# kfjahnke/envutil

Hardware: AMD Instinct MI355X
Metric: Mpix/s reprojected (16K lat/lon->cubemap, b-spline-3) (higher is better)
Workload: dtype f32

## Files before the change

envutil_amd/csrc/eu_api_render.hip:

```cpp

#include "eu_context.h"
#include "eu_setup_math.h"
#include "eu_encode.h"
#include "eu_rgbe_dev.h"

using namespace eu_host;

namespace {

int band_shift_of(int band_rows)
{
  int sh = 0;
  while ((1 << sh) < band_rows) sh++;
  return sh;
}

int build_inv_planar(const eu_target *t, eu_inv_planar *q)
{
  memset(q, 0, sizeof *q);
  const eu_facet *f = t->single;
  if (!f || !eu::has_2d_tf(*f)) return EU_OK;
  q->shear = f->shear_g != 0.0 || f->shear_t != 0.0;
  q->shift = f->h != 0.0 || f->v != 0.0;
  q->lcp = f->a != 0.0 || f->b != 0.0 || f->c != 0.0;
// ... 151 lines not shown
    if (k + 1 < EU_REJ_N) m = std::min(m, raw[k + 1]);
    tab[EU_REJ_HDR + k] = (float)(m * (1.0 - 2e-3));
  }
  const double W = std::max(std::max(std::fabs((double)d.wex0), std::fabs((double)d.wex1)),
                            std::max(std::fabs((double)d.wex2), std::fabs((double)d.wex3)));
  const double mg = 1e-3 * W;
  tab[0] = (float)u0; tab[1] = (float)(1.0 / du); tab[2] = 1.0f;
  {
    bool mono = true;
    double prev = -1.0;
    const double tmax = std::acos(std::max(-1.0, u0));
    for (int i = 0; i <= 4096 && mono; i++) {
      bool k2 = true;
      const double r = radius(tmax * i / 4096.0, k2);
      mono = k2 && r > prev;
      prev = r;
    }
    if (mono && analytic) {
      tab[2] = 2.0f;
      const double f = 1.0 - 2e-3;
      tab[10] = d.has_lcp ? 1.0f / d.lens_s : 0.0f;
      tab[11] = (float)(f * (d.has_lcp ? d.lens_d : 1.0)); tab[12] = d.has_lcp ? (float)(f * d.lens_c) : 0.0f;
      tab[13] = d.has_lcp ? (float)(f * d.lens_b) : 0.0f; tab[14] = d.has_lcp ? (float)(f * d.lens_a) : 0.0f;
    }
  }
  tab[4] = d.has_shift ? d.lens_h : 0.0f; tab[5] = d.has_shift ? d.lens_v : 0.0f;
  tab[6] = (float)(d.wex0 - mg); tab[7] = (float)(d.wex1 + mg); tab[8] = (float)(d.wex2 - mg); tab[9] = (float)(d.wex3 + mg);
  return true;
}

int build_multi(const eu_target *t, eu_source *const *srcs, int nsrc, float *out_dev,
                size_t row_stride_bytes, const eu_switches &sw, eu_multi_params *p, int *degree)
{
  { int rc0 = check_target(t); if (rc0) return rc0; }
  const eu_source *s0 = srcs[0];
  for (int f = 0; f < nsrc; f++) {
    if (!srcs[f]) return fail(EU_ERR_HANDLE, "null source");
    if (srcs[f]->degree != s0->degree) return fail(EU_ERR_ARGUMENT, "facets must share the spline degree");
  }
  const bool twine = t->ntaps > 0;
  std::vector<unsigned char> key = plan_key_of(t, srcs, nsrc, true);
  auto &mp = cur().mplan;
  HIPCHK(cur().tables.host_wait());
  if (key != mp.key) {
    eu::mat3 r_cam = eu::make_r3(t->roll, t->pitch, t->yaw, false);
    std::vector<float> rows;
    eu::stepper_tables tb;
    for (int f = 0; f < nsrc; f++) {
      eu::mat3 r_fct = eu::make_r3(srcs[f]->fct.roll, srcs[f]->fct.pitch, srcs[f]->fct.yaw, true);
      eu::mat3 basis = eu::rotate(r_cam, r_fct);
      if (!eu::build_stepper_tables(*t, basis, true, twine, tb))
        return fail(EU_ERR_UNSUPPORTED, "no stepper for this target projection");
      rows.insert(rows.end(), tb.row.begin(), tb.row.end());
    }
    { int rcu = upload_plan(mp, t, tb, rows, key); if (rcu) return rcu; }
  }
  std::vector<eu_src_dev> sd((size_t)nsrc);
  for (int f = 0; f < nsrc; f++) sd[f] = srcs[f]->sd;
  HIPCHK(mp.src.reserve((size_t)nsrc));
  HIPCHK(hipMemcpyAsync(mp.src.p, sd.data(), sizeof(eu_src_dev) * (size_t)nsrc, hipMemcpyHostToDevice, cur().stream));
  bool any_rej = false;
  std::vector<float> rej;
  if (sw.rej) {
    rej.resize((size_t)nsrc * EU_REJ_STRIDE);
    for (int f = 0; f < nsrc; f++) any_rej |= build_reject_table(sd[f], rej.data() + (size_t)f * EU_REJ_STRIDE, sw.rej == 2);
  }
  if (any_rej) {
    HIPCHK(mp.rej.reserve(rej.size()));
    HIPCHK(hipMemcpyAsync(mp.rej.p, rej.data(), rej.size() * sizeof(float), hipMemcpyHostToDevice, cur().stream));
  }
  std::vector<eu_generic> gv((size_t)nsrc);
  bool any_generic = false;
  for (int f = 0; f < nsrc; f++) {
    memset(&gv[f], 0, sizeof(eu_generic));
    if (!eu::has_translation(srcs[f]->fct) && !eu::generic_target(*t)) continue;
    if (!eu::make_generic(*t, srcs[f]->fct, gv[f]))
      return fail(EU_ERR_UNSUPPORTED, "generic stepper (translation, --single): no planar-to-ray functor for this target projection");
    any_generic = true;
  }
  if (any_generic) {
    HIPCHK(mp.gen.reserve((size_t)nsrc));
    HIPCHK(hipMemcpyAsync(mp.gen.p, gv.data(), sizeof(eu_generic) * (size_t)nsrc, hipMemcpyHostToDevice, cur().stream));
  }
  HIPCHK(hipStreamSynchronize(cur().stream));
  eu_inv_planar inv;
  { int rci = build_inv_planar(t, &inv); if (rci) return rci; }
  memset(p, 0, sizeof *p);
  p->gen = any_generic ? mp.gen.p : nullptr;
  p->rej = any_rej ? mp.rej.p : nullptr;
  p->inv = inv;
  fill_frame(t, p);
  p->form = mp.form; p->norm_mode = mp.norm; p->twine = twine; p->ntaps = t->ntaps;
  fill_synopsis(t, srcs, nsrc, p);
  p->col = mp.col.p; p->row = mp.row.p; p->taps = mp.taps.p; p->srcs = mp.src.p;
  p->out = out_dev; p->out_stride = (long long)(row_stride_bytes / sizeof(float));
  *degree = s0->degree;
  return EU_OK;
}

void refresh_seg_flags(const eu_render_params *p)
{
  eu_src_dev cmp = p->src;
  cmp.base = nullptr;
  if (cur().plan.seg_valid && !memcmp(&cmp, &cur().plan.seg_sd, sizeof cmp)) return;
  cur().plan.seg_sd = cmp;
  cur().plan.seg_valid = true;
  const int W = p->width, H = p->height;
  const int nseg = (H + EU_SEG_ROWS - 1) / EU_SEG_ROWS;
  cur().plan.seg_flags.assign((size_t)nseg, 0);
  const eu_src_dev &s = p->src;
  if (s.prj != EU_SPHERICAL || W < 64 || cur().plan.h_col.size() < (size_t)2 * W || cur().plan.h_row.size() < (size_t)H * EU_ROW_FLOATS)
    return;
  const double kx = (double)s.total_w / s.ext_w, ky = (double)s.total_h / s.ext_h;
  auto ray = [&](int x, int y, double *r) {
    const float *rt = &cur().plan.h_row[(size_t)y * EU_ROW_FLOATS];
    const float c0 = cur().plan.h_col[(size_t)x], c1 = cur().plan.h_col[(size_t)W + x];
    for (int i = 0; i < 3; i++)
      r[i] = p->form == EU_FORM_BCA ? (double)rt[3 + i] * c0 + (double)rt[6 + i] * c1 + rt[i]
                                    : (double)rt[3 + i] * c0 + rt[i];
  };
  for (int k = 0; k < nseg; k++) {
    const int yc = std::min(k * EU_SEG_ROWS + EU_SEG_ROWS / 2, H - 1);
    int across = 0;
    for (int j = 0; j < 16; j++) {
      const int xc = std::min((int)((j + 0.5) * W / 16), W - 2);
      double a[3], b[3];
      ray(xc, yc, a);
      ray(xc + 1, yc, b);
      const double lon0 = std::atan2(a[0], a[2]), lon1 = std::atan2(b[0], b[2]);
      const double lat0 = std::atan2(a[1], std::hypot(a[0], a[2])), lat1 = std::atan2(b[1], std::hypot(b[0], b[2]));
      double dlon = std::fabs(lon1 - lon0);
      if (dlon > M_PI) dlon = 2.0 * M_PI - dlon;
      if (std::fabs(lat1 - lat0) * ky > 0.5 * dlon * kx) across++;
    }
    cur().plan.seg_flags[(size_t)k] = across > 8;
  }
}

int launch_staged(const eu_render_params *p, const eu_switches &sw, hipStream_t st, int *launches)
{
  const unsigned long long ntiles = eu_staged_tiles(p->width, p->row_begin, p->row_end);
  if (ntiles > EU4_WL_MAX_TILES) return -2;
  const size_t need = eu_render4_worklist_ints((size_t)ntiles);
  if (cur().staged.wl.cap < need) {
    if (cur().staged.wl_pair.host_wait() != hipSuccess || cur().staged.wl.reserve(need) != hipSuccess) return -1;
    if (hipMemsetAsync(cur().staged.wl.p, 0, eu_render4_worklist_header_ints() * sizeof(int), st) != hipSuccess) {
      cur().staged.wl.cap = 0;
      return -1;
    }
  }
  eu_render_params q = *p;
  q.wl = cur().staged.wl.p;
  if (cur().staged.wl_pair.order_after(st) != hipSuccess) return -1;
  const int rc = eu_launch_render4(&q, &sw, cur().plan.h_row.data(), cur().plan.h_row.size(), cur().plan.plan_gen, st, launches);
  if (rc || !*launches) return rc;
  return cur().staged.wl_pair.note(st) != hipSuccess ? -1 : 0;
}

int launch_packed_runs(const eu_render_params *p, const eu_switches &sw, hipStream_t st, int *launches)
{
  refresh_seg_flags(p);
  const std::vector<eu_run> runs = eu_split_runs(cur().plan.seg_flags.data(), (int)cur().plan.seg_flags.size(), *p, sw.hybrid == 2);
  if (runs.empty()) { *launches = 1; return eu_launch_render2(p, &sw, st); }
  for (const eu_run &r : runs) {
    eu_render_params q = *p;
    q.row_begin = r.row_begin; q.row_end = r.row_end;
    q.out = p->out + (long long)(r.row_begin - p->row_begin) * p->out_stride;
    q.layout = r.layout;
    ++*launches;
    const int rc = eu_launch_render2(&q, &sw, st);
    if (rc) return rc;
  }
  return 0;
}

int launch_render(const eu_render_params *p, const eu_switches &sw, hipStream_t st)
{
  eu_path path = eu_select_path(*p, sw);
  int rc = 0, n = 0;
  if (path == EU_PATH_STAGED) {
    rc = launch_staged(p, sw, st, &n);
    if (!rc && !n) path = eu_select_path(*p, sw, false);
  }
  switch (path) {
    case EU_PATH_STAGED: break;
    case EU_PATH_PACKED_RUNS: rc = launch_packed_runs(p, sw, st, &n); break;
    case EU_PATH_PACKED: n = 1; rc = eu_launch_render2(p, &sw, st); break;
    case EU_PATH_GENERAL: n = 1; rc = eu_launch_render(p, st); break;
    case EU_PATH_GENERAL_DIRECT: {
      eu_render_params q = *p;
      q.direct = 1;
      n = 1;
      rc = eu_launch_render(&q, st);
    }
  }
  cur().launches += n;
  return rc;
}

int order_encoders(hipStream_t st)
{
  if (st == cur().stream) cur().enc.own = true;
  else if (cur().enc.own) { HIPCHK(hipStreamSynchronize(cur().stream)); cur().enc.own = false; }
  HIPCHK(cur().tables.order_after(st));
  HIPCHK(cur().enc.readers.order_after(st));
  return EU_OK;
}

}

namespace eu_host __attribute__((visibility("hidden"))) {

int render_on_device(const eu_target *trg, eu_source *const *srcs, int nsrc, float *out_dev, size_t stride_bytes,
                     const eu_switches &sw, hipStream_t st, const eu_encode *enc, bool rgbe)
{
  int rc;
  const bool multi = nsrc > 1;
  const bool screen = trg->out_format == EU_OUT_SRGBA8;
  eu_target tf = *trg;
  float *fout = out_dev;
  size_t fstride = stride_bytes;
  const size_t rows = (size_t)(trg->row_end - trg->row_begin);
  if (screen || enc || rgbe) {
    if (screen && !cur().lut) return fail(EU_ERR_NO_DEVICE, "sRGB table missing: library not initialised");
    if (screen && (rc = order_encoders(st))) return rc;
    tf.out_format = EU_OUT_FLOAT;
    fstride = (size_t)frame_w(trg) * trg->nchannels * sizeof(float);
    if (cur().out.scr.cap < rows * frame_w(trg) * trg->nchannels) HIPCHK(cur().tables.host_wait());
    HIPCHK(cur().out.scr.reserve(rows * frame_w(trg) * trg->nchannels));
    fout = cur().out.scr.p;
  }
  if (multi) {
    eu_multi_params mp;
    int mdeg = 0;
    if ((rc = build_multi(&tf, srcs, nsrc, fout, fstride, sw, &mp, &mdeg))) return rc;
    if (eu_launch_render_multi(&mp, mdeg, st)) return fail(EU_ERR_NO_DEVICE, "kernel launch failed");
  } else {
    eu_render_params p;
    if ((rc = build_params(&tf, srcs, nsrc, fout, fstride, sw, &p))) return rc;
    if (launch_render(&p, sw, st)) return fail(EU_ERR_NO_DEVICE, "kernel launch failed");
  }
  if (screen &&
      eu_launch_to_screen(fout, (long long)(fstride / sizeof(float)), (unsigned *)out_dev,
                          (long long)(stride_bytes / sizeof(unsigned)), frame_w(trg), (int)rows,
                          trg->nchannels, cur().lut, st))
    return fail(EU_ERR_NO_DEVICE, "kernel launch failed");
  if (enc && rows) {
    eu_encode_params ep {};
    ep.src = fout; ep.src_stride_bytes = fstride;
    ep.dst = out_dev; ep.dst_stride_bytes = stride_bytes;
    ep.tables = cur().enc.steps.dev.p;
    ep.w = frame_w(trg); ep.h = (int)rows; ep.nch = trg->nchannels;
    ep.bits = enc->bits; ep.big_endian = enc->big_endian;
    if (eu_launch_encode(&ep, st)) return fail(EU_ERR_NO_DEVICE, "kernel launch failed");
  }
  if (rgbe && rows) {
    eu_rgbe_encode_params ep {};
    ep.src = fout; ep.src_stride_bytes = fstride;
    ep.dst = reinterpret_cast<uint32_t *>(out_dev); ep.dst_stride_bytes = stride_bytes;
    ep.w = frame_w(trg); ep.h = (int)rows;
    if (eu_launch_rgbe_encode(&ep, st)) return fail(EU_ERR_NO_DEVICE, "kernel launch failed");
  }
  return EU_OK;
}

}

extern "C" {

static int check_steps(const float *s, int bits, const char *who, const char *which)
{
  const int n = 1 << bits;
  const std::string head = std::string(who) + ": " + which + " steps: ";
  if (std::isnan(s[1])) return fail(EU_ERR_ARGUMENT, head + "entry 1 is NaN, a table has at least one code above 0");
  int m = 1;
  for (; m + 1 < n && !std::isnan(s[m + 1]); m++)
    if (s[m + 1] < s[m]) return fail(EU_ERR_ARGUMENT, head + "entry " + std::to_string(m + 1) + " is smaller than the one before it");
  for (int k = m + 1; k < n; k++)
    if (!std::isnan(s[k]))
      return fail(EU_ERR_ARGUMENT, head + "entry " + std::to_string(k) + " is a number behind the NaN at entry " + std::to_string(m + 1));
  return EU_OK;
}

static int check_encode(const char *who, const eu_encode *enc, int width, int nch, const void *out, size_t out_row_stride_bytes)
{
  const std::string head = std::string(who) + ": ";
  if (!enc || !out) return fail(EU_ERR_ARGUMENT, head + "null argument");
  if (enc->bits != 8 && enc->bits != 16) return fail(EU_ERR_ARGUMENT, head + "bits must be 8 or 16");
  if (!enc->colour_steps) return fail(EU_ERR_ARGUMENT, head + "null colour steps");
  if (nch < 1 || nch > 4) return fail(EU_ERR_ARGUMENT, head + "channels must be 1..4");
  if (width < 0 || (size_t)width * nch > (size_t(1) << 28)) return fail(EU_ERR_ARGUMENT, head + "rows of 0 .. 2^28 samples");
  if (out_row_stride_bytes < (size_t)width * nch * (enc->bits / 8)) return fail(EU_ERR_ARGUMENT, head + "row stride smaller than a row");
  if (enc->bits == 16 && (reinterpret_cast<uintptr_t>(out) % 2 || out_row_stride_bytes % 2))
    return fail(EU_ERR_ARGUMENT, head + "16-bit samples lie at even addresses: out and its row stride are multiples of 2");
  int rc;
  if ((rc = check_steps(enc->colour_steps, enc->bits, who, "colour"))) return rc;
  if (enc->alpha_steps && (rc = check_steps(enc->alpha_steps, enc->bits, who, "alpha"))) return rc;
  return EU_OK;
}

static int upload_steps(const eu_encode *enc, hipStream_t st)
{
  { int rc = order_encoders(st); if (rc) return rc; }
  const size_t n = size_t(1) << enc->bits;
  const float *alpha = enc->alpha_steps ? enc->alpha_steps : enc->colour_steps;
  held_table &steps = cur().enc.steps;
  if (steps.holds(enc->colour_steps, n, alpha, n)) return EU_OK;
// ... 285 lines not shown
```

envutil_amd/csrc/eu_launch.h:

```cpp
#ifndef EU_LAUNCH_H
#define EU_LAUNCH_H
#include <hip/hip_runtime.h>
#include <cstddef>
#include "eu_device.h"
#include "eu_select.h"
#include "eu_worklist.h"

#define EU_REJ_N 1024
#define EU_REJ_HDR 16
#define EU_REJ_STRIDE (EU_REJ_HDR + EU_REJ_N)

struct eu_multi_params {
  int width, height, row_begin, row_end;
  int form, norm_mode, twine, ntaps, nch, nfct, plus;
  const float *col;
  const float *row;
  const float *taps;
  const eu_src_dev *srcs;
  float *out;
  long long out_stride;
  int tiles_x, tiles_y;
  int band_shift, band_count, band_index;
  int hdr, hdr_low, hdr_high;
  const eu_generic *gen;
  eu_inv_planar inv;
  const float *rej;
};

struct eu_alpha_params;

template <class T> struct eu_dev_buf {
  T *p = nullptr;
  size_t cap = 0;
  hipError_t reserve(size_t n)
  {
    if (cap >= n) return hipSuccess;
    if (p) (void)hipFree(p);
    p = nullptr; cap = 0;
    const hipError_t e = hipMalloc((void **)&p, n * sizeof(T));
    if (e == hipSuccess) cap = n; else p = nullptr;
    return e;
  }
};

struct eu_readers {
  hipEvent_t ev = nullptr;
  bool recorded = false;
  hipError_t note(hipStream_t st)
  {
    hipError_t e = ev ? order_after(st) : hipEventCreateWithFlags(&ev, hipEventDisableTiming);
    if (e == hipSuccess) e = hipEventRecord(ev, st);
    if (e == hipSuccess) recorded = true;
    return e;
  }
  hipError_t host_wait() const { return recorded ? hipEventSynchronize(ev) : hipSuccess; }
  hipError_t order_after(hipStream_t st) const { return recorded ? hipStreamWaitEvent(st, ev, 0) : hipSuccess; }
};

extern "C" {
int eu_launch_render(const eu_render_params *p, void *stream);
int eu_launch_render2(const eu_render_params *p, const eu_switches *sw, void *stream);
int eu_launch_render4(const eu_render_params *p, const eu_switches *sw, const float *h_row, size_t h_row_floats,
                      unsigned long long plan_gen, void *stream, int *launches);
int eu_launch_render_rays(const eu_rays_params *p, int path, void *stream);
int eu_launch_view_tables(const eu_view_dev *views, int nviews, int prj, int width, int height, int twine, float *col,
                          float *row, void *stream);
int eu_launch_render_views(const eu_render_params *p, const eu_view_strides *vs, int nviews, int path,
                           const eu_switches *sw, void *stream);
int eu_launch_render_layers(const eu_render_params *p, const eu_layers_params *lp, int path, const eu_switches *sw,
                            void *stream);
int eu_launch_render_multi(const eu_multi_params *p, int degree, void *stream);
int eu_launch_render_multi_nch1(const eu_multi_params *p, int degree, void *stream);
int eu_launch_render_multi_nch2(const eu_multi_params *p, int degree, void *stream);
int eu_launch_render_multi_nch3(const eu_multi_params *p, int degree, void *stream);
int eu_launch_render_multi_nch4(const eu_multi_params *p, int degree, void *stream);
int eu_launch_render_views_multi(const eu_multi_params *p, const eu_view_strides *vs, int nviews, int degree, void *stream);
int eu_launch_render_views_multi_nch1(const eu_multi_params *p, const eu_view_strides *vs, int nviews, int degree, void *stream);
int eu_launch_render_views_multi_nch2(const eu_multi_params *p, const eu_view_strides *vs, int nviews, int degree, void *stream);
int eu_launch_render_views_multi_nch3(const eu_multi_params *p, const eu_view_strides *vs, int nviews, int degree, void *stream);
int eu_launch_render_views_multi_nch4(const eu_multi_params *p, const eu_view_strides *vs, int nviews, int degree, void *stream);
int eu_launch_to_screen(const float *in, long long in_stride, unsigned *out, long long out_stride, int w, int rows,
                        int nch, const float *lut, void *stream);
int eu_launch_prefilter(float *container, const eu_container *g, int nch, int bc0, int bc1, int prefilter_degree,
                        int spherical, int iir_stream, void *stream);
int eu_launch_cubemap_build(const float *faces_dev, float *ir_dev, int nch, long face_px, long section_px,
                            long left_frame, long right_frame, double refc_md, double model_to_px,
                            int prefilter_degree, int iir_stream, void *stream);
int eu_launch_facet_alpha(const eu_alpha_params *p, void *stream);
int eu_launch_diag(const eu_render_params *p, unsigned long long *stamps_dev, void *stream);
int eu_launch_diag_coords(const eu_src_dev *s, const float *rays_dev, long n, int variant, float *out_dev,
                          void *stream);
int eu_launch_selftest(unsigned long long seed, int blocks, int iters, unsigned long long *bad_dev, void *stream);
int eu_verify_const_div(float c, float limit, void *stream);
int eu_current_slot(void);
}

#endif
```

envutil_amd/csrc/eu_render4.hip:

```cpp
#include <cstdio>
#include <cstring>
#include <vector>
#include <algorithm>
#include "eu_packed_dev.h"
#include "eu_launch.h"

#define EU4_TW 16
#define EU4_TH 8
#define EU4_WAVES 4
#ifndef EU4_WAVES0
#define EU4_WAVES0 1
#define EU4_TEXELS 384
#define EU4_OCC0 4
#endif
#define EU4_UNIT_ROWS 4
#define EU4_COL_FLOATS 8
#define EU4_MAX_PLANS 16

__device__ __forceinline__ void eu4_box_reduce(int &mn0, int &mn1, int &mx0, int &mx1)
{
#define EU4_RED(ctrl)                                        \
  "v_min_i32_dpp %0, %0, %0 " ctrl "\n\t"                    \
  "v_min_i32_dpp %1, %1, %1 " ctrl "\n\t"                    \
  "v_max_i32_dpp %2, %2, %2 " ctrl "\n\t"                    \
  "v_max_i32_dpp %3, %3, %3 " ctrl "\n\t"
  asm("s_nop 1\n\t"
      EU4_RED("row_shr:1 row_mask:0xf bank_mask:0xf")
      EU4_RED("row_shr:2 row_mask:0xf bank_mask:0xf")
      EU4_RED("row_shr:4 row_mask:0xf bank_mask:0xf")
      EU4_RED("row_shr:8 row_mask:0xf bank_mask:0xf")
      EU4_RED("row_bcast:15 row_mask:0xa bank_mask:0xf")
      EU4_RED("row_bcast:31 row_mask:0xc bank_mask:0xf")
      "s_nop 0"
      : "+v"(mn0), "+v"(mn1), "+v"(mx0), "+v"(mx1));
#undef EU4_RED
  mn0 = __builtin_amdgcn_readlane(mn0, 63); mn1 = __builtin_amdgcn_readlane(mn1, 63);
  mx0 = __builtin_amdgcn_readlane(mx0, 63); mx1 = __builtin_amdgcn_readlane(mx1, 63);
}

typedef __attribute__((address_space(3))) void *eu4_lds_void;
typedef const __attribute__((address_space(1))) void *eu4_gbl_void;

typedef float eu4_f4 __attribute__((ext_vector_type(4)));

__device__ __forceinline__ void eu4_dma_row(unsigned dst, unsigned voff, const char *sb)
{
  unsigned keep;
  asm volatile("s_mov_b32 %0, m0\n\t"
               "s_mov_b32 m0, %1\n\t"
               "s_nop 0\n\t"
               "global_load_lds_dwordx4 %2, %3\n\t"
               "s_mov_b32 m0, %0"
               : "=&s"(keep) : "s"(dst), "v"(voff), "s"(sb) : "memory");
}

struct eu4_plan {
  const float *atab_g;
  const int *tileplan;
  const float *coltab;
  int tiles16;
  const int *l2_rows;
  int l2_off[9];
  int l2_half;
  unsigned long long l2_magic;
  const int *l1_ent;
  int l1_off[9];
  int l1_ecols;
  unsigned long long l1_magic;
  const int *xtab;
  const int *boxtab;
#ifdef EU5_STAMPS
  unsigned long long *stamps;
#endif
};

#ifdef EU5_STAMPS
#define EU5_STAMP(k) do { asm volatile("" ::: "memory"); st_[k] = __builtin_amdgcn_s_memtime(); asm volatile("" ::: "memory"); } while (0)
#define EU5_STAMP32(k) do { asm volatile("" ::: "memory"); st_[k] = (unsigned)__builtin_amdgcn_s_memtime(); asm volatile("" ::: "memory"); } while (0)
#else
#define EU5_STAMP(k) do { } while (0)
#define EU5_STAMP32(k) do { } while (0)
#endif

template <int NCH, int DEG, int PRJ>
__device__ __forceinline__ void eu4_tile(const eu_render_params &p, const eu4_plan &w, const float *atab,
                                         float *wtile, int tile_y, int x0, int lane)
{
  constexpr int TEX = 4;
  constexpr int order = DEG + 1;
  const eu_src_dev &s = p.src;
  const int lx = lane & 7, ly = lane >> 3;
  const int y = p.row_begin + tile_y * EU4_TH + ly;
  const bool yin = y < p.row_end;
  const int yc = yin ? y : p.row_end - 1;
  const float *rt = p.row + (long long)eu_frame_row(yc, p.band_shift, p.band_count, p.band_index) * EU_ROW_FLOATS;
  const int xa = x0 + 2 * lx, xb = xa + 1;
  const bool va = yin && xa < p.width, vb = yin && xb < p.width;
  const int xac = xa < p.width ? xa : p.width - 1, xbc = xb < p.width ? xb : p.width - 1;

  eu_f2 tx, ty, gy;
  eu_i2 hit, ok = { -1, -1 };
  int ixa, ixb;
  float wxa[order], wxb[order];
  eu_ray2 r;
  {
    const float A0 = rt[0], A1 = rt[1], A2 = rt[2], B0 = rt[3], B1 = rt[4], B2 = rt[5];
    const eu_f2 c0 = { p.col[xac], p.col[xbc] };
    if (p.form == EU_FORM_BCA) {
      const float C0 = rt[6], C1 = rt[7], C2 = rt[8];
      const float *colB = p.col + p.width;
      const eu_f2 c1 = { colB[xac], colB[xbc] };
      r.x = B0 * c0 + C0 * c1 + A0;
      r.y = B1 * c0 + C1 * c1 + A1;
      r.z = B2 * c0 + C2 * c1 + A2;
    } else {
      r.x = B0 * c0 + A0;
      r.y = B1 * c0 + A1;
      r.z = B2 * c0 + A2;
    }
    if (p.norm_mode == EU_NORM_DIV) {
      eu_f2 sqn = r.x * r.x; sqn = sqn + r.y * r.y; sqn = sqn + r.z * r.z;
      const eu_f2 n = { sqrtf(sqn.x), sqrtf(sqn.y) };
      r.x = r.x / n; r.y = r.y / n; r.z = r.z / n;
    }
  }
  asm volatile("s_waitcnt vmcnt(0)" ::: "memory");
  eu_f2 sx, sy;
  hit = eu_coord2_ok<PRJ>(s, r, sx, sy, atab, ok);
  const eu_f2 gx = eu_gate2_ok(sx, s.gate0, s.lower0, s.upper0, ok);
  gy = eu_gate2_ok(sy, s.gate1, s.lower1, s.upper1, ok);
  eu_f2 fx;
  if constexpr (DEG & 1) fx = (eu_f2){ floorf(gx.x), floorf(gx.y) };
  else fx = (eu_f2){ roundf(gx.x), roundf(gx.y) };
  tx = gx - fx;
  ixa = (int)fx.x; ixb = (int)fx.y;
  hit = hit & (eu_i2){ va ? -1 : 0, vb ? -1 : 0 };
  eu_f2 fy;
  if constexpr (DEG & 1) fy = (eu_f2){ floorf(gy.x), floorf(gy.y) };
  else fy = (eu_f2){ roundf(gy.x), roundf(gy.y) };
  ty = gy - fy;
  const int iya = (int)fy.x, iyb = (int)fy.y;

  int mnx = INT_MAX, mny = INT_MAX, mxx = INT_MIN, mxy = INT_MIN;
  if (hit.x) { mnx = ixa; mxx = ixa; mny = iya; mxy = iya; }
  if (hit.y) { mnx = min(mnx, ixb); mxx = max(mxx, ixb); mny = min(mny, iyb); mxy = max(mxy, iyb); }
  eu4_box_reduce(mnx, mny, mxx, mxy);
  const bool any = mnx != INT_MAX;
  const long long bw = (long long)mxx - mnx + order, bh = (long long)mxy - mny + order;
  const bool fits = bw <= 64 && bh <= EU4_TEXELS && bw * bh <= EU4_TEXELS;
  const bool clean = __ballot((hit.x && !ok.x) || (hit.y && !ok.y)) == 0ull;
  float *const orow = p.out + (long long)(yc - p.row_begin) * p.out_stride;
  if (any && !(fits && clean)) {
    if (lane == 0) {
      const int id = tile_y * w.tiles16 + x0 / EU4_TW;
      const int sh = eu4_shard_of(id);
      const int slot = atomicAdd(p.wl + EU4_WL_SHARD(sh), 1);
      p.wl[EU4_WL_ENTRIES + (size_t)slot * EU4_SHARDS + sh] = id;
    }
    return;
  }
  float qa[NCH], qb[NCH];
  if (any) {
    const int ibw = (int)bw, ibh = (int)bh;
    const unsigned lds_tile = (unsigned)(unsigned long long)(eu4_lds_void)wtile;
    if (lane < ibw) {
      const int bx0 = mnx - DEG / 2, by0 = mny - DEG / 2;
      const unsigned voff = (unsigned)(lane * NCH) * 4u;
      const char *sb = (const char *)(s.base + ((long long)by0 * s.es1 + (long long)bx0 * NCH));
      const long long step = s.es1 * 4;
      unsigned dst = lds_tile;
      const unsigned dstep = (unsigned)ibw * (TEX * 4u);
#pragma unroll 1
      for (int it = 0; it < ibh; it++) { eu4_dma_row(dst, voff, sb); sb += step; dst += dstep; }
    }
    eu_f2 wx[order], wy[order];
    float wya[order], wyb[order];
    if constexpr (DEG >= 2) {
      eu_weights2<DEG>(s.wm, ty, wy);
      eu_weights2<DEG>(s.wm, tx, wx);
    }
#pragma unroll
    for (int i = 0; i < order; i++) {
      if constexpr (DEG >= 2) {
        wya[i] = wy[i].x; wyb[i] = wy[i].y;
        wxa[i] = wx[i].x; wxb[i] = wx[i].y;
      } else {
        wya[i] = wyb[i] = 0.0f;
        wxa[i] = wxb[i] = 0.0f;
      }
    }
    const int oa = hit.x ? ((iya - mny) * ibw + (ixa - mnx)) * TEX : 0;
    const int ob = hit.y ? ((iyb - mny) * ibw + (ixb - mnx)) * TEX : 0;
    asm volatile("s_waitcnt vmcnt(0)" ::: "memory");
    eu_lptr lt = (eu_lptr)wtile;
    eu_accumulate1<NCH, DEG, TEX, int, eu_lptr>(lt + oa, ibw * TEX, wxa, wya, tx.x, ty.x, qa);
    eu_accumulate1<NCH, DEG, TEX, int, eu_lptr>(lt + ob, ibw * TEX, wxb, wyb, tx.y, ty.y, qb);
  } else {
#pragma unroll
    for (int c = 0; c < NCH; c++) { qa[c] = 0.0f; qb[c] = 0.0f; }
  }
  constexpr int ncol = (NCH == 2 || NCH == 4) ? NCH - 1 : NCH;
  const bool bright = s.brighten != 1.0f;
#pragma unroll
  for (int c = 0; c < NCH; c++) {
    float a = qa[c], bb = qb[c];
    if (bright && c < ncol) { a = a * s.brighten; bb = bb * s.brighten; }
    qa[c] = hit.x ? a : 0.0f;
    qb[c] = hit.y ? bb : 0.0f;
  }
  if (va) eu_put<NCH>(orow, xa, qa);
  if (vb) eu_put<NCH>(orow, xb, qb);
}

template <int NCH, int DEG, int PRJ>
__global__ __launch_bounds__(64 * EU4_WAVES0, EU4_OCC0) void eu_render4s_kernel(const eu_render_params p, const eu4_plan w)
{
  __shared__ __attribute__((aligned(16))) float tile_all[EU4_WAVES0 * EU4_TEXELS * 4];
  __shared__ __attribute__((aligned(16))) float atab[768];
  const int lane = threadIdx.x & 63;
  const int wave = __builtin_amdgcn_readfirstlane(threadIdx.x >> 6);
  float *const tile = tile_all + wave * (EU4_TEXELS * 4);
  if (PRJ != EU_CUBEMAP && wave == 0) {
    static_assert(EU_ATAN_TAB_FLOATS * 4 <= 3 * 1024, "three pieces");
#pragma unroll
    for (int i = 0; i < 3; i++)
      __builtin_amdgcn_global_load_lds((eu4_gbl_void)(w.atab_g + i * 256 + lane * 4),
                                       (eu4_lds_void)(atab + i * 256), 16, 0, 0);
  }
  const int tile_x = (int)(blockIdx.x >> 3) * EU4_WAVES0 + wave;
  const int tile_y = ((int)blockIdx.z * 8 + (int)(blockIdx.x & 7)) * EU4_UNIT_ROWS + (int)blockIdx.y;
  if (tile_y >= p.tiles_y) return;
  if constexpr (EU4_WAVES0 > 1) {
    asm volatile("s_waitcnt vmcnt(0)" ::: "memory");
    __syncthreads();
  }
  if (tile_x >= w.tiles16) return;
  eu4_tile<NCH, DEG, PRJ>(p, w, atab, tile, tile_y, tile_x * EU4_TW, lane);
}

template <int NCH, int DEG, int PRJ>
__device__ __forceinline__ void eu4_direct_tile(const eu_render_params &p, const float *atab, int tile_y, int x0, int lane)
{
  const eu_src_dev &s = p.src;
  const int lx = lane & 7, ly = lane >> 3;
  const int y = p.row_begin + tile_y * EU4_TH + ly;
  const bool yin = y < p.row_end;
  const int yc = yin ? y : p.row_end - 1;
  const float *rt = p.row + (long long)eu_frame_row(yc, p.band_shift, p.band_count, p.band_index) * EU_ROW_FLOATS;
  const int xa = x0 + 2 * lx, xb = xa + 1;
  const bool va = yin && xa < p.width, vb = yin && xb < p.width;
  const int xac = xa < p.width ? xa : p.width - 1, xbc = xb < p.width ? xb : p.width - 1;
  eu_ray2 ry;
  {
    const float A0 = rt[0], A1 = rt[1], A2 = rt[2], B0 = rt[3], B1 = rt[4], B2 = rt[5];
    const eu_f2 c0 = { p.col[xac], p.col[xbc] };
    if (p.form == EU_FORM_BCA) {
      const float C0 = rt[6], C1 = rt[7], C2 = rt[8];
      const float *colB = p.col + p.width;
      const eu_f2 c1 = { colB[xac], colB[xbc] };
      ry.x = B0 * c0 + C0 * c1 + A0;
      ry.y = B1 * c0 + C1 * c1 + A1;
      ry.z = B2 * c0 + C2 * c1 + A2;
    } else {
      ry.x = B0 * c0 + A0;
      ry.y = B1 * c0 + A1;
      ry.z = B2 * c0 + A2;
    }
    if (p.norm_mode == EU_NORM_DIV) {
      eu_f2 sqn = ry.x * ry.x; sqn = sqn + ry.y * ry.y; sqn = sqn + ry.z * ry.z;
      const eu_f2 n = { sqrtf(sqn.x), sqrtf(sqn.y) };
      ry.x = ry.x / n; ry.y = ry.y / n; ry.z = ry.z / n;
    }
  }
  eu_f2 sx, sy;
  eu_i2 hit = eu_coord2<PRJ>(s, ry, sx, sy, atab);
  hit = hit & (eu_i2){ va ? -1 : 0, vb ? -1 : 0 };
  float pxa[NCH], pxb[NCH];
  eu_eval2<NCH, DEG>(s, sx, sy, hit, pxa, pxb);
  float *const orow = p.out + (long long)(yc - p.row_begin) * p.out_stride;
  if (va) eu_put<NCH>(orow, xa, pxa);
  if (vb) eu_put<NCH>(orow, xb, pxb);
}

#include "eu_share_groups.h"
#include "eu_render5.h"

template <int DEG>
__global__ __launch_bounds__(256) void eu_colplan_kernel(const eu_render_params p, float *ct,
                                                         float A0, float A2, float B0, float B2)
{
  __shared__ __attribute__((aligned(16))) float atab[EU_ATAN_TAB_FLOATS];
  if (threadIdx.x < EU_ATAN_TAB_ENTRIES) eu_atan_tab_entry(threadIdx.x, atab + 8 * threadIdx.x);
  __syncthreads();
  constexpr int order = DEG + 1;
  const eu_src_dev &s = p.src;
  const int xa = 2 * (blockIdx.x * 256 + threadIdx.x), xb = xa + 1;
  if (xa >= p.width) return;
  const int xbc = xb < p.width ? xb : p.width - 1;
  const eu_f2 c0 = { p.col[xa], p.col[xbc] };
  const eu_f2 rx = B0 * c0 + A0, rz = B2 * c0 + A2;
  eu_i2 ok = { -1, -1 };
  const eu_f2 q2 = rx * rx + rz * rz;
  const eu_f2 qs = eu_sqrt2_ok(q2, ok);
  const eu_f2 lon = eu_atan2f_2_tab_ok(rx, rz, atab, 0, ok);
  eu_f2 i0 = { (float)((double)lon.x - s.tex_x0), (float)((double)lon.y - s.tex_x0) };
  if (s.cdiv_ok) i0 = eu_div2_const(i0, s.ext_w, s.rcp_ext_w);
  else i0 = i0 / s.ext_w;
  i0 = i0 * s.total_w; i0 = i0 - .5f;
  const eu_f2 sx = i0 - s.win_x_off;
  const eu_f2 gx = eu_gate2_ok(sx, s.gate0, s.lower0, s.upper0, ok);
  eu_f2 fx;
  if constexpr (DEG & 1) fx = (eu_f2){ floorf(gx.x), floorf(gx.y) };
  else fx = (eu_f2){ roundf(gx.x), roundf(gx.y) };
  const eu_f2 tx = gx - fx;
  eu_f2 wx[4];
#pragma unroll
  for (int i = 0; i < 4; i++) wx[i] = (eu_f2){ 0.0f, 0.0f };
  if constexpr (DEG >= 2) eu_weights2<DEG>(s.wm, tx, wx);
  float e[2][EU4_COL_FLOATS];
  e[0][0] = __int_as_float(ok.x ? (int)fx.x : INT_MIN);
  e[1][0] = __int_as_float(ok.y ? (int)fx.y : INT_MIN);
  e[0][1] = tx.x; e[1][1] = tx.y;
#pragma unroll
  for (int i = 0; i < 4; i++) { e[0][2 + i] = i < order ? wx[i].x : 0.0f; e[1][2 + i] = i < order ? wx[i].y : 0.0f; }
  e[0][6] = qs.x; e[1][6] = qs.y;
  e[0][7] = lon.x; e[1][7] = lon.y;
  float *o = ct + (size_t)xa * EU4_COL_FLOATS;
#pragma unroll
  for (int i = 0; i < EU4_COL_FLOATS; i++) o[i] = e[0][i];
  if (xb < p.width) {
#pragma unroll
    for (int i = 0; i < EU4_COL_FLOATS; i++) o[EU4_COL_FLOATS + i] = e[1][i];
  }
}

template <int NCH, int DEG, int PRJ>
__global__ __launch_bounds__(256, 4) void eu_render4d_kernel(const eu_render_params p, const eu4_plan w)
{
  __shared__ __attribute__((aligned(16))) float atab[EU_ATAN_TAB_FLOATS];
  if constexpr (PRJ != EU_CUBEMAP) {
    if (threadIdx.x < EU_ATAN_TAB_ENTRIES) eu_atan_tab_entry(threadIdx.x, atab + 8 * threadIdx.x);
  }
  const int lane = threadIdx.x & 63;
  const int wave = __builtin_amdgcn_readfirstlane(threadIdx.x >> 6);
  const int gid = blockIdx.x * EU4_WAVES + wave;
  const int sh = gid & (EU4_SHARDS - 1);
  const int nwork = __builtin_amdgcn_readfirstlane(
    __hip_atomic_load(p.wl + EU4_WL_SHARD(sh), __ATOMIC_RELAXED, __HIP_MEMORY_SCOPE_AGENT));
  __syncthreads();
#pragma unroll 1
  for (int k = gid / EU4_SHARDS; k < nwork; k += (int)(gridDim.x * EU4_WAVES / EU4_SHARDS)) {
    const int id = __builtin_amdgcn_readfirstlane(p.wl[EU4_WL_ENTRIES + (size_t)k * EU4_SHARDS + sh]);
    const int tile_y = id / w.tiles16;
    const int x0 = (id - tile_y * w.tiles16) * EU4_TW;
    eu4_direct_tile<NCH, DEG, PRJ>(p, atab, tile_y, x0, lane);
  }
  __shared__ int last, listed;
  __syncthreads();
  if (threadIdx.x == 0) { listed = 0; last = atomicAdd(p.wl + EU4_WL_DONE1, 1) == (int)gridDim.x - 1; }
  __syncthreads();
  if (last) {
    int mine = 0;
    for (int i = threadIdx.x; i < EU4_SHARDS; i += 256)
      mine += __hip_atomic_load(p.wl + EU4_WL_SHARD(i), __ATOMIC_RELAXED, __HIP_MEMORY_SCOPE_AGENT);
    atomicAdd(&listed, mine);
    for (int i = threadIdx.x; i <= EU4_SHARDS + 8; i += 256)
      __hip_atomic_store(p.wl + 16 * i, 0, __ATOMIC_RELAXED, __HIP_MEMORY_SCOPE_AGENT);
    __syncthreads();
    if (threadIdx.x == 0) __hip_atomic_store(p.wl + EU4_WL_LISTED, listed, __ATOMIC_RELAXED, __HIP_MEMORY_SCOPE_AGENT);
  }
}

static long long eu4_followers_plan = 0, eu4_followers_last = 0;
extern "C" unsigned long long eu_hip_share_follower_tiles(void) { return (unsigned long long)eu4_followers_last; }
static int eu4_boxtab_last = 0;
static long long eu4_boxtab_tiles_last = 0;
extern "C" int eu_hip_boxtab_used(void) { return eu4_boxtab_last; }
extern "C" unsigned long long eu_hip_boxtab_tiles(void) { return (unsigned long long)eu4_boxtab_tiles_last; }

#ifndef EU4_DIRECT_WGS
#define EU4_DIRECT_WGS 2048
#endif

template <int NCH, int DEG, int PRJ>
static int launch4_ndp(const eu_render_params &p, const eu4_plan &w, hipStream_t st)
{
  if constexpr (PRJ == EU_SPHERICAL) {
    static const int cus = [] {
      int dev = 0, n = 0;
      if (hipGetDevice(&dev) != hipSuccess) return 0;
      if (hipDeviceGetAttribute(&n, hipDeviceAttributeMultiprocessorCount, dev) != hipSuccess) return 0;
      return n;
    }();
    const bool fast = eu_staged_fast_profile(p);
    const bool bt = fast && w.boxtab != nullptr && p.out_stride < (1ll << 25);
    int per_cu = 0;
    if (bt) {
      static const int occ = [] { int n = 0; return hipOccupancyMaxActiveBlocksPerMultiprocessor(&n, eu_render5_kernel<NCH, DEG, PRJ, true, true>, 64 * EU5_WAVES, 0) == hipSuccess ? n : 0; }();
      per_cu = occ;
    } else if (fast) {
      static const int occ = [] { int n = 0; return hipOccupancyMaxActiveBlocksPerMultiprocessor(&n, eu_render5_kernel<NCH, DEG, PRJ, true>, 64 * EU5_WAVES, 0) == hipSuccess ? n : 0; }();
      per_cu = occ;
    } else {
      static const int occ = [] { int n = 0; return hipOccupancyMaxActiveBlocksPerMultiprocessor(&n, eu_render5_kernel<NCH, DEG, PRJ, false>, 64 * EU5_WAVES, 0) == hipSuccess ? n : 0; }();
      per_cu = occ;
    }
    const int wgs = (cus / 8) * 8 * per_cu;
    if (wgs <= 0) return -1;
    if (fast) eu4_followers_last = eu4_followers_plan;
    eu4_boxtab_last = bt;
    if (bt) hipLaunchKernelGGL((eu_render5_kernel<NCH, DEG, PRJ, true, true>), dim3((unsigned)wgs), dim3(64 * EU5_WAVES), 0, st, p, w);
    else if (fast) hipLaunchKernelGGL((eu_render5_kernel<NCH, DEG, PRJ, true>), dim3((unsigned)wgs), dim3(64 * EU5_WAVES), 0, st, p, w);
    else hipLaunchKernelGGL((eu_render5_kernel<NCH, DEG, PRJ, false>), dim3((unsigned)wgs), dim3(64 * EU5_WAVES), 0, st, p, w);
  } else {
    const int units = (p.tiles_y + EU4_UNIT_ROWS - 1) / EU4_UNIT_ROWS;
    dim3 grid((unsigned)(8 * ((w.tiles16 + EU4_WAVES0 - 1) / EU4_WAVES0)), (unsigned)EU4_UNIT_ROWS, (unsigned)((units + 7) / 8));
    hipLaunchKernelGGL((eu_render4s_kernel<NCH, DEG, PRJ>), grid, dim3(64 * EU4_WAVES0), 0, st, p, w);
  }
  if (hipGetLastError() != hipSuccess) return -1;
  hipLaunchKernelGGL((eu_render4d_kernel<NCH, DEG, PRJ>), dim3(EU4_DIRECT_WGS), dim3(256), 0, st, p, w);
  if (hipGetLastError() != hipSuccess) {
    (void)hipMemsetAsync(p.wl, 0, EU4_WL_ENTRIES * sizeof(int), st);
    return -1;
  }
  return 0;
}

template <int NCH, int DEG>
static int launch4_nd(const eu_render_params &p, const eu4_plan &w, hipStream_t st)
{
  switch (p.src.prj) {
    case EU_SPHERICAL: return launch4_ndp<NCH, DEG, EU_SPHERICAL>(p, w, st);
    case EU_CUBEMAP: return launch4_ndp<NCH, DEG, EU_CUBEMAP>(p, w, st);
    case EU_BIATAN6: return launch4_ndp<NCH, DEG, EU_BIATAN6>(p, w, st);
  }
  return -2;
}

template <int NCH>
static int launch4_n(const eu_render_params &p, const eu4_plan &w, hipStream_t st)
{
  switch (p.src.degree) {
    case 1: return launch4_nd<NCH, 1>(p, w, st);
    case 2: return launch4_nd<NCH, 2>(p, w, st);
    case 3: return launch4_nd<NCH, 3>(p, w, st);
  }
  return -2;
}

static_assert(EU_STAGED_TILE_ROWS == EU4_TH && EU_STAGED_MAX_TILES_Y == 65535 * 8 * EU4_UNIT_ROWS, "eu_select.h: eu_staged_covers");
namespace {
struct plan_cache {
  std::vector<unsigned char> key;
  eu_dev_buf<int> tileplan, l2_rows, l1_ent, xtab, boxtab;
  bool has_boxtab = false;
  long long boxtab_tiles = 0;
  eu_dev_buf<float> coltab;
  float *atab = nullptr;
  int planned_rows = 0;
  int l2_off[9] = {};
  int l1_off[9] = {};
  int l1_ecols = 1;
  long long follower_tiles = 0;
} g4s[EU_MAX_SLOTS];
#define g4 (g4s[eu_current_slot()])

bool ensure_atab()
{
  if (g4.atab) return true;
  std::vector<float> tab(768, 0.0f);
  for (int i = 0; i < EU_ATAN_TAB_ENTRIES; i++) eu_atan_tab_entry(i, tab.data() + 8 * i);
  if (hipMalloc((void **)&g4.atab, tab.size() * sizeof(float)) != hipSuccess) return false;
  return hipMemcpy(g4.atab, tab.data(), tab.size() * sizeof(float), hipMemcpyHostToDevice) == hipSuccess;
}

template <int DEG>
void launch_colplan(const eu_render_params &p, float *ct, const float *k, hipStream_t st)
{
  hipLaunchKernelGGL((eu_colplan_kernel<DEG>), dim3((unsigned)((p.width + 511) / 512)), dim3(256), 0, st, p, ct,
                     k[0], k[1], k[2], k[3]);
}

std::vector<unsigned char> eu4_plan_key(const eu_render_params &p, unsigned long long plan_gen, const eu_switches &sw)
{
  std::vector<unsigned char> key(sizeof(unsigned long long) + sizeof(eu_src_dev) + 11 * sizeof(int));
  unsigned char *q = key.data();
  memcpy(q, &plan_gen, sizeof plan_gen); q += sizeof plan_gen;
  eu_src_dev sd = p.src; sd.base = nullptr;
  memcpy(q, &sd, sizeof sd); q += sizeof sd;
  const int v[11] = { p.width, p.row_begin, p.row_end, p.band_shift, p.band_count, p.band_index, p.form, p.norm_mode, sw.share,
                      sw.boxtab, sw.boxtab_max_kb };
  memcpy(q, v, sizeof v);
  return key;
}

bool upload(eu_dev_buf<int> &buf, const std::vector<int> &v, size_t spare)
{
  if (buf.reserve(v.size() + spare) != hipSuccess) return false;
  return v.empty() || hipMemcpy(buf.p, v.data(), v.size() * sizeof(int), hipMemcpyHostToDevice) == hipSuccess;
}

template <int DEG>
void launch_boxplan(const eu_render_params &p, const float *atab_g, const int *l2_rows, int tiles16, int ntiles, int *tab, hipStream_t st)
{
  hipLaunchKernelGGL((eu5_boxplan_kernel<DEG>), dim3((unsigned)((ntiles + 3) / 4)), dim3(256), 0, st, p, atab_g, l2_rows, tiles16,
                     ntiles, tab);
}

int eu4_build_plans(const eu_render_params &p, int tiles16, const eu_switches &sw, const float *h_row,
                    size_t h_row_floats, hipStream_t st)
{
  std::vector<int> tp((size_t)p.tiles_y, -1);
  std::vector<float> plans;
  const bool can = p.form == EU_FORM_BA && p.norm_mode == EU_NORM_NONE && h_row;
  if (can && sw.colplan) {
    for (int ty = 0; ty < p.tiles_y; ty++) {
      float k[4] = { 0, 0, 0, 0 };
      bool same = true;
      for (int ly = 0; ly < EU4_TH && same; ly++) {
        const int y = std::min(p.row_begin + ty * EU4_TH + ly, p.row_end - 1);
        const size_t fr = (size_t)eu_frame_row(y, p.band_shift, p.band_count, p.band_index) * EU_ROW_FLOATS;
        if (fr + 6 > h_row_floats) { same = false; break; }
        const float c[4] = { h_row[fr + 0], h_row[fr + 2], h_row[fr + 3], h_row[fr + 5] };
        if (ly == 0) memcpy(k, c, sizeof k);
        else same = memcmp(k, c, sizeof k) == 0;
      }
      if (!same) continue;
      int id = -1;
      for (size_t j = 0; j < plans.size() / 4 && id < 0; j++)
        if (memcmp(&plans[4 * j], k, sizeof k) == 0) id = (int)j;
      if (id < 0 && plans.size() / 4 < EU4_MAX_PLANS) {
        id = (int)(plans.size() / 4);
        plans.insert(plans.end(), k, k + 4);
      }
      tp[(size_t)ty] = id;
    }
  }
  const int nplans = (int)(plans.size() / 4);
  if (hipStreamSynchronize(st) != hipSuccess) return -1;
  if (g4.tileplan.reserve(tp.size()) != hipSuccess) return -1;
  if (g4.coltab.reserve(std::max<size_t>(1, nplans) * (size_t)p.width * EU4_COL_FLOATS) != hipSuccess) return -1;
  if (hipMemcpy(g4.tileplan.p, tp.data(), tp.size() * sizeof(int), hipMemcpyHostToDevice) != hipSuccess) return -1;
  g4.planned_rows = 0;
  for (int v : tp) g4.planned_rows += v >= 0;
  auto paired = [&](int m) { return 2 * m + 1 < p.tiles_y && tp[(size_t)2 * m] >= 0 && tp[(size_t)2 * m] == tp[(size_t)2 * m + 1]; };
  {
    std::vector<int> rows[8], all;
    for (int r = 0; r < p.tiles_y; r++)
      if (!paired(r >> 1)) rows[(r / EU5_UNIT_ROWS) & 7].push_back(r);
    for (int x = 0; x < 8; x++) { g4.l2_off[x] = (int)all.size(); all.insert(all.end(), rows[x].begin(), rows[x].end()); }
    g4.l2_off[8] = (int)all.size();
    if (!upload(g4.l2_rows, all, 1)) return -1;
  }
  g4.has_boxtab = false; g4.boxtab_tiles = 0;
  if (sw.boxtab && eu_staged_fast_profile(p)) {
    const long long ntiles = (long long)g4.l2_off[8] * tiles16;
    const long long bytes = ntiles * (EU5_BT_RECS * 16);
    if (bytes <= (long long)sw.boxtab_max_kb * 1024) {
      if (g4.boxtab.reserve((size_t)std::max<long long>(1, ntiles) * (EU5_BT_RECS * 4)) != hipSuccess) return -1;
      if (ntiles > 0) {
        switch (p.src.degree) {
          case 1: launch_boxplan<1>(p, g4.atab, g4.l2_rows.p, tiles16, (int)ntiles, g4.boxtab.p, st); break;
          case 2: launch_boxplan<2>(p, g4.atab, g4.l2_rows.p, tiles16, (int)ntiles, g4.boxtab.p, st); break;
          default: launch_boxplan<3>(p, g4.atab, g4.l2_rows.p, tiles16, (int)ntiles, g4.boxtab.p, st); break;
        }
        if (hipGetLastError() != hipSuccess) return -1;
      }
      g4.has_boxtab = true; g4.boxtab_tiles = ntiles;
    }
  }
  for (int j = 0; j < nplans; j++) {
    float *ct = g4.coltab.p + j * (size_t)p.width * EU4_COL_FLOATS;
    switch (p.src.degree) {
      case 1: launch_colplan<1>(p, ct, &plans[4 * j], st); break;
      case 2: launch_colplan<2>(p, ct, &plans[4 * j], st); break;
      default: launch_colplan<3>(p, ct, &plans[4 * j], st); break;
    }
    if (hipGetLastError() != hipSuccess) return -1;
  }
  std::vector<float> h_ct((size_t)nplans * p.width * EU4_COL_FLOATS);
  if (nplans) {
    if (hipStreamSynchronize(st) != hipSuccess) return -1;
    if (hipMemcpy(h_ct.data(), g4.coltab.p, h_ct.size() * sizeof(float), hipMemcpyDeviceToHost) != hipSuccess) return -1;
  }
  std::vector<int> cm, cp;
  for (int m = 0; 2 * m + 1 < p.tiles_y; m++)
    if (paired(m)) { cm.push_back(m); cp.push_back(tp[(size_t)2 * m]); }
  eu_share_input in;
  in.width = p.width; in.tiles16 = tiles16; in.row_begin = p.row_begin; in.row_end = p.row_end;
  in.band_mode = p.band_count > 1;
  in.ncand = (int)cm.size(); in.cand_m = cm.data(); in.cand_plan = cp.data();
  in.h_row = h_row; in.h_row_floats = h_row_floats; in.row_floats = EU_ROW_FLOATS;
  in.coltab = nplans ? h_ct.data() : nullptr; in.col_floats = EU4_COL_FLOATS; in.nplans = nplans;
  in.mode = sw.share; in.unit_drows = EU5_UNIT_ROWS / 2;
  eu_share_result gr;
  eu_share_build(in, gr);
  if (!upload(g4.l1_ent, gr.entries, 2)) return -1;
  if (g4.xtab.reserve(gr.xtab.size()) != hipSuccess) return -1;
  if (hipMemcpy(g4.xtab.p, gr.xtab.data(), gr.xtab.size() * sizeof(int), hipMemcpyHostToDevice) != hipSuccess) return -1;
  for (int x = 0; x < 9; x++) g4.l1_off[x] = gr.off[x];
  g4.l1_ecols = gr.ecols;
  g4.follower_tiles = gr.follower_tiles;
  return 0;
}

void eu4_fill_plan(eu4_plan &w)
{
  w.tileplan = g4.tileplan.p;
  w.coltab = g4.coltab.p;
  w.l2_rows = g4.l2_rows.p;
  for (int x = 0; x < 9; x++) w.l2_off[x] = g4.l2_off[x];
  w.l2_half = (w.tiles16 + 1) / 2;
  w.l2_magic = (1ull << 40) / (unsigned long long)w.l2_half + 1;
  w.l1_ent = g4.l1_ent.p;
  for (int x = 0; x < 9; x++) w.l1_off[x] = g4.l1_off[x];
  w.l1_ecols = g4.l1_ecols;
  w.l1_magic = (1ull << 40) / (unsigned long long)w.l1_ecols + 1;
  w.xtab = g4.xtab.p;
  w.boxtab = g4.has_boxtab ? g4.boxtab.p : nullptr;
}

int launch4(const eu_render_params &p, const eu4_plan &w, hipStream_t st)
{
  switch (p.nch) {
    case 3: return launch4_n<3>(p, w, st);
    case 4: return launch4_n<4>(p, w, st);
  }
  return -2;
}

#ifdef EU5_STAMPS
int launch4_stamped(const eu_render_params &p, eu4_plan &w, hipStream_t st)
{
  static unsigned long long *d_st = nullptr; static size_t st_cap = 0; static int dumps = 0;
  const size_t ntile_st = (size_t)w.tiles16 * p.tiles_y * 8;
  const size_t nst = ntile_st + 8192 * 4;
  if (st_cap < nst) { if (d_st) (void)hipFree(d_st); if (hipMalloc((void **)&d_st, nst * 8) != hipSuccess) return -1; st_cap = nst; }
  (void)hipMemsetAsync(d_st, 0, nst * 8, st);
  w.stamps = d_st;
  const int rc_ = launch4(p, w, st);
  if (rc_ == 0 && dumps < 2 && nst >= 8 * 4096) {
    dumps++;
    std::vector<unsigned long long> h(nst);
    (void)hipStreamSynchronize(st);
    (void)hipMemcpy(h.data(), d_st, nst * 8, hipMemcpyDeviceToHost);
    double acc[32][8] = {}; size_t cnt[32] = {};
    for (size_t t = 0; t < ntile_st / 8; t++) {
      const unsigned long long *q = &h[t * 8];
      if (!q[0] || !q[7]) continue;
      const int cls = (int)(q[1] & 31);
      cnt[cls]++;
      acc[cls][0] += (double)(q[2] - q[0]); acc[cls][1] += (double)(q[3] - q[2]);
      if (q[4]) { acc[cls][2] += (double)(q[4] - q[3]); acc[cls][3] += (double)(q[5] - q[4]); acc[cls][4] += (double)(q[6] - q[5]); }
      acc[cls][5] += (double)(q[7] - q[6]); acc[cls][6] += (double)(q[7] - q[0]);
    }
    {
      double mn = 1e30, mx = 0, sum = 0, l1 = 0, first = 1e30, last = 0; size_t nw = 0;
      for (size_t k = 0; k < 8192; k++) {
        const unsigned long long *q = &h[ntile_st + k * 4];
        if (!q[3]) continue;
        const double d = (double)(q[2] - q[0]);
        mn = std::min(mn, d); mx = std::max(mx, d); sum += d; l1 += (double)(q[1] - q[0]); nw++;
        first = std::min(first, (double)q[0]); last = std::max(last, (double)q[2]);
      }
      if (nw) fprintf(stderr, "eu5 waves: %zu, cycles per wave min %.0f avg %.0f max %.0f, first loop avg %.0f, first start .. last end %.0f\n",
                      nw, mn, sum / nw, mx, l1 / nw, last - first);
    }
    for (int c = 0; c < 32; c++) if (cnt[c])
      fprintf(stderr, "eu5 stamps: hoist %d npass %2d tiles %8zu | coords %7.0f box %6.0f dma-issue+weights %6.0f dma-wait %6.0f taps(all passes) %6.0f store %5.0f | tile %7.0f (100 MHz ticks? s_memtime)\n",
              c >> 4, (c & 15) - 1, cnt[c], acc[c][0] / cnt[c], acc[c][1] / cnt[c], acc[c][2] / cnt[c], acc[c][3] / cnt[c], acc[c][4] / cnt[c], acc[c][5] / cnt[c], acc[c][6] / cnt[c]);
  }
  return rc_;
}
#endif
}

extern "C" int eu_launch_render4(const eu_render_params *pp, const eu_switches *sw, const float *h_row, size_t h_row_floats,
                                 unsigned long long plan_gen, void *stream, int *launches)
{
  eu_render_params p = *pp;
  eu4_followers_last = 0;
  eu4_boxtab_last = 0; eu4_boxtab_tiles_last = 0;
  *launches = 2;
  if (!eu_staged_covers(p) || !p.wl) return -2;
  p.tiles_y = (p.row_end - p.row_begin + EU4_TH - 1) / EU4_TH;
  eu4_plan w;
  w.tiles16 = (p.width + EU4_TW - 1) / EU4_TW;
  if (w.tiles16 <= 0 || p.tiles_y <= 0) return 0;
  hipStream_t st = (hipStream_t)stream;
  if (!ensure_atab()) return -1;
  w.atab_g = g4.atab;
  if (p.src.prj == EU_SPHERICAL) {
    std::vector<unsigned char> key = eu4_plan_key(p, plan_gen, *sw);
    if (key != g4.key) {
      if (eu4_build_plans(p, w.tiles16, *sw, h_row, h_row_floats, st)) return -1;
      g4.key.swap(key);
    }
    if (sw->r4 != 1 && !eu_staged_worth(p.src.degree, g4.planned_rows, p.tiles_y)) { *launches = 0; return 0; }
  }
  eu4_fill_plan(w);
  eu4_followers_plan = g4.follower_tiles;
  eu4_boxtab_tiles_last = w.boxtab ? g4.boxtab_tiles : 0;
#ifdef EU5_STAMPS
  return launch4_stamped(p, w, st);
#else
  return launch4(p, w, st);
#endif
}
```

envutil_amd/csrc/eu_render5.h:

```cpp
#define EU5_WAVES 4
#ifndef EU5_TEXELS
#define EU5_TEXELS 576
#endif
#ifndef EU5_OCC
#define EU5_OCC 4
#endif
#ifndef EU5_UNIT_ROWS
#define EU5_UNIT_ROWS 4
#endif

typedef const __attribute__((address_space(3))) eu4_f4 *eu5_l4ptr;

template <int NCH, int DEG>
__device__ __forceinline__ void eu5_taps(eu_lptr lt, int a, int b, int pitch, const eu_f2 *wx, const eu_f2 *wy,
                                         eu_f2 tx, eu_f2 ty, eu_f2 &rga, eu_f2 &bxa, eu_f2 &rgb, eu_f2 &bxb)
{
  constexpr int order = DEG + 1;
  if constexpr (DEG == 1) {
    const eu_f2 wl0 = 1.0f - tx, wr0 = tx, wl1 = 1.0f - ty, wr1 = ty;
    const eu4_f4 a00 = *(eu5_l4ptr)(lt + a), a01 = *(eu5_l4ptr)(lt + a + 4);
    const eu4_f4 a10 = *(eu5_l4ptr)(lt + a + pitch), a11 = *(eu5_l4ptr)(lt + a + pitch + 4);
    const eu4_f4 b00 = *(eu5_l4ptr)(lt + b), b01 = *(eu5_l4ptr)(lt + b + 4);
    const eu4_f4 b10 = *(eu5_l4ptr)(lt + b + pitch), b11 = *(eu5_l4ptr)(lt + b + pitch + 4);
    {
      const eu_f2 l0 = { wl0.x, wl0.x }, r0 = { wr0.x, wr0.x }, l1 = { wl1.x, wl1.x }, r1 = { wr1.x, wr1.x };
      eu_f2 s = a00.xy * l0; s = s + a01.xy * r0; s = s * l1;
      eu_f2 u = a10.xy * l0; u = u + a11.xy * r0; rga = s + u * r1;
      s = a00.zw * l0; s = s + a01.zw * r0; s = s * l1;
      u = a10.zw * l0; u = u + a11.zw * r0; bxa = s + u * r1;
    }
    {
      const eu_f2 l0 = { wl0.y, wl0.y }, r0 = { wr0.y, wr0.y }, l1 = { wl1.y, wl1.y }, r1 = { wr1.y, wr1.y };
      eu_f2 s = b00.xy * l0; s = s + b01.xy * r0; s = s * l1;
      eu_f2 u = b10.xy * l0; u = u + b11.xy * r0; rgb = s + u * r1;
      s = b00.zw * l0; s = s + b01.zw * r0; s = s * l1;
      u = b10.zw * l0; u = u + b11.zw * r0; bxb = s + u * r1;
    }
  } else {
#pragma unroll
    for (int j = 0; j < order; j++) {
      eu4_f4 ta[order], tb[order];
#pragma unroll
      for (int i = 0; i < order; i++) {
        ta[i] = *(eu5_l4ptr)(lt + a + j * pitch + 4 * i);
        tb[i] = *(eu5_l4ptr)(lt + b + j * pitch + 4 * i);
      }
      const eu_f2 w0a = { wx[0].x, wx[0].x }, w0b = { wx[0].y, wx[0].y };
      eu_f2 ra = ta[0].xy * w0a, qa = ta[0].zw * w0a, rb = tb[0].xy * w0b, qb = tb[0].zw * w0b;
#pragma unroll
      for (int i = 1; i < order; i++) {
        const eu_f2 wa = { wx[i].x, wx[i].x }, wb = { wx[i].y, wx[i].y };
        ra = EU_MAD2(wa, ta[i].xy, ra); qa = EU_MAD2(wa, ta[i].zw, qa);
        rb = EU_MAD2(wb, tb[i].xy, rb); qb = EU_MAD2(wb, tb[i].zw, qb);
      }
      const eu_f2 ya = { wy[j].x, wy[j].x }, yb = { wy[j].y, wy[j].y };
      if (j == 0) { rga = ra * ya; bxa = qa * ya; rgb = rb * yb; bxb = qb * yb; }
      else { rga = EU_MAD2(ra, ya, rga); bxa = EU_MAD2(qa, ya, bxa); rgb = EU_MAD2(rb, yb, rgb); bxb = EU_MAD2(qb, yb, bxb); }
    }
  }
}

__device__ __forceinline__ void eu5_box_reduce(int &q0, int &q1, int &q2, int &q3, int &h0, int &h1, int &h2, int &h3)
{
#define EU5_RED(ctrl)                                        \
  "v_min_i32_dpp %0, %0, %0 " ctrl "\n\t"                    \
  "v_min_i32_dpp %1, %1, %1 " ctrl "\n\t"                    \
  "v_max_i32_dpp %2, %2, %2 " ctrl "\n\t"                    \
  "v_max_i32_dpp %3, %3, %3 " ctrl "\n\t"
  asm("s_nop 1\n\t"
      EU5_RED("row_shr:1 row_mask:0xf bank_mask:0xf")
      EU5_RED("row_shr:2 row_mask:0xf bank_mask:0xf")
      EU5_RED("row_shr:4 row_mask:0xf bank_mask:0xf")
      EU5_RED("row_shr:8 row_mask:0xf bank_mask:0xf")
      "v_mov_b32 %4, %0\n\tv_mov_b32 %5, %1\n\tv_mov_b32 %6, %2\n\tv_mov_b32 %7, %3\n\t"
      "v_min_i32_dpp %4, %0, %4 row_bcast:15 row_mask:0xa bank_mask:0xf\n\t"
      "v_min_i32_dpp %5, %1, %5 row_bcast:15 row_mask:0xa bank_mask:0xf\n\t"
      "v_max_i32_dpp %6, %2, %6 row_bcast:15 row_mask:0xa bank_mask:0xf\n\t"
      "v_max_i32_dpp %7, %3, %7 row_bcast:15 row_mask:0xa bank_mask:0xf\n\t"
      "s_nop 0"
      : "+v"(q0), "+v"(q1), "+v"(q2), "+v"(q3), "=&v"(h0), "=&v"(h1), "=&v"(h2), "=&v"(h3));
#undef EU5_RED
}

struct eu5_box { int mnx, mny, mxx, mxy; };

struct eu5_divtab_t { unsigned v[65]; };
static constexpr eu5_divtab_t eu5_make_divtab()
{
  eu5_divtab_t t = {};
  t.v[0] = 0;
  for (unsigned w = 1; w <= 64; w++) t.v[w] = ((65536u + w - 1) / w) | ((64u / w) << 24);
  return t;
}
__constant__ const eu5_divtab_t eu5_divtab = eu5_make_divtab();

__device__ __forceinline__ eu5_box eu5_box_at(int a, int b, int c, int d, int lane)
{
  eu5_box r;
  r.mnx = __builtin_amdgcn_readlane(a, lane); r.mny = __builtin_amdgcn_readlane(b, lane);
  r.mxx = __builtin_amdgcn_readlane(c, lane); r.mxy = __builtin_amdgcn_readlane(d, lane);
  return r;
}
__device__ __forceinline__ eu5_box eu5_box_join(const eu5_box &a, const eu5_box &b)
{
  eu5_box r = { min(a.mnx, b.mnx), min(a.mny, b.mny), max(a.mxx, b.mxx), max(a.mxy, b.mxy) };
  return r;
}
template <int ORDER>
__device__ __forceinline__ int eu5_box_fits(const eu5_box &b)
{
  if (b.mnx == INT_MAX) return -1;
  const unsigned bw = (unsigned)b.mxx - (unsigned)b.mnx + ORDER, bh = (unsigned)b.mxy - (unsigned)b.mny + ORDER;
  return bw <= 64u && bh <= (unsigned)EU5_TEXELS && bw * bh <= (unsigned)EU5_TEXELS;
}

__device__ __forceinline__ eu_f2 eu5_gate2(eu_f2 c, int kind, float lower, float upper)
{
  if (kind == 0) {
    eu_f2 r = c;
    r = eu_sel2(c < lower, (eu_f2){ lower, lower }, r);
    r = eu_sel2(c > upper, (eu_f2){ upper, upper }, r);
    return r;
  }
  eu_f2 cc = c - lower;
  if (kind == 1) cc = eu_abs2(cc);
  return cc + lower;
}

__device__ __forceinline__ int eu5_out_of_range3(float a, float b, float c)
{
  const float hi = __builtin_fmaxf(__builtin_fmaxf(__builtin_fabsf(a), __builtin_fabsf(b)), __builtin_fabsf(c));
  const float lo = __builtin_fminf(__builtin_fminf(__builtin_fabsf(a), __builtin_fabsf(b)), __builtin_fabsf(c));
  return (hi <= 0x1p40f && lo >= 0x1p-40f) ? 0 : -1;
}

struct eu5_tab8 { eu_f2 c0; float A0, A1, A2, B0, B1, B2; };

template <bool FAST>
__device__ __forceinline__ void eu5_load8(const eu_render_params &p, int tile_y, int x0, int lane, eu5_tab8 &T)
{
  const int pr = lane & 3, rw = (lane >> 2) & 7, hf = lane >> 5;
  const int y = p.row_begin + tile_y * EU4_TH + rw;
  const int yc = y < p.row_end ? y : p.row_end - 1;
  const float *rt = p.row + (long long)(FAST ? yc : eu_frame_row(yc, p.band_shift, p.band_count, p.band_index)) * EU_ROW_FLOATS;
  const int xa = x0 + 8 * hf + 2 * pr, xb = xa + 1;
  const int xac = xa < p.width ? xa : p.width - 1, xbc = xb < p.width ? xb : p.width - 1;
  T.A0 = rt[0]; T.A1 = rt[1]; T.A2 = rt[2]; T.B0 = rt[3]; T.B1 = rt[4]; T.B2 = rt[5];
  T.c0 = (eu_f2){ p.col[xac], p.col[xbc] };
}

struct eu5_co8 {
  eu_f2 tx, ty;
  int ixa, ixb, iya, iyb;
  eu_i2 ok;
};

template <int DEG>
__device__ __forceinline__ void eu5_coords8(const eu_src_dev &s, const float *atab, const eu5_tab8 &T, eu5_co8 &c)
{
  eu_i2 big0 = { 0, 0 }, big1 = { 0, 0 };
  const eu_f2 c0 = T.c0;
  const eu_f2 rx = T.B0 * c0 + T.A0, ry = T.B1 * c0 + T.A1, rz = T.B2 * c0 + T.A2;
  const eu_i2 ok = { ~eu5_out_of_range3(rx.x, ry.x, rz.x), ~eu5_out_of_range3(rx.y, ry.y, rz.y) };
  const eu_f2 q2 = rx * rx + rz * rz;
  const eu_f2 qs = eu_sqrt2_safe(q2);
  const eu_f2 lat = eu_atan2f_2_lean(ry, qs, atab, 1, big0);
  const eu_f2 lon = eu_atan2f_2_lean(rx, rz, atab, 0, big1);
  c.ok = ok & ~(big0 | big1);
  eu_f2 i0 = { (float)((double)lon.x - s.tex_x0), (float)((double)lon.y - s.tex_x0) };
  if (s.cdiv_ok) i0 = eu_div2_const(i0, s.ext_w, s.rcp_ext_w);
  else i0 = eu_div2_rr(i0, s.ext_w, eu_rcp_refined(s.ext_w));
  i0 = i0 * s.total_w; i0 = i0 - .5f;
  const eu_f2 sx = i0 - s.win_x_off;
  const eu_f2 gx = eu5_gate2(sx, s.gate0, s.lower0, s.upper0);
  eu_f2 fx;
  if constexpr (DEG & 1) fx = (eu_f2){ floorf(gx.x), floorf(gx.y) };
  else fx = (eu_f2){ roundf(gx.x), roundf(gx.y) };
  c.tx = gx - fx;
  c.ixa = (int)fx.x; c.ixb = (int)fx.y;
  eu_f2 i1 = { (float)((double)lat.x - s.tex_y0), (float)((double)lat.y - s.tex_y0) };
  if (s.cdiv_ok) i1 = eu_div2_const(i1, s.ext_h, s.rcp_ext_h);
  else i1 = eu_div2_rr(i1, s.ext_h, eu_rcp_refined(s.ext_h));
  i1 = i1 * s.total_h; i1 = i1 - .5f;
  const eu_f2 sy = i1 - s.win_y_off;
  c.ty = eu5_gate2(sy, s.gate1, s.lower1, s.upper1);
}

template <int DEG>
__device__ __forceinline__ void eu5_split_y(eu5_co8 &c)
{
  const eu_f2 gy = c.ty;
  eu_f2 fy;
  if constexpr (DEG & 1) fy = (eu_f2){ floorf(gy.x), floorf(gy.y) };
  else fy = (eu_f2){ roundf(gy.x), roundf(gy.y) };
  c.ty = gy - fy;
  c.iya = (int)fy.x; c.iyb = (int)fy.y;
}

struct eu5_boxes {
  int q0, q1, q2, q3, h0, h1, h2, h3;
  eu5_box full;
  int npass;
  bool clean;
};

template <int DEG, bool GATES>
__device__ __forceinline__ void eu5_box_stage(int gate0, int gate1, float upper0, float upper1, eu_i2 hit, eu_i2 ok,
                                              int ixa, int ixb, int iya, int iyb, eu5_boxes &b)
{
  constexpr int order = DEG + 1;
  int q0 = INT_MAX, q1 = INT_MAX, q2 = INT_MIN, q3 = INT_MIN, h0, h1, h2, h3;
  if (hit.x) { q0 = ixa; q2 = ixa; q1 = iya; q3 = iya; }
  if (hit.y) { q0 = min(q0, ixb); q2 = max(q2, ixb); q1 = min(q1, iyb); q3 = max(q3, iyb); }
  eu5_box_reduce(q0, q1, q2, q3, h0, h1, h2, h3);
  const eu5_box full = eu5_box_join(eu5_box_at(h0, h1, h2, h3, 31), eu5_box_at(h0, h1, h2, h3, 63));
  bool clean = __ballot((hit.x && !ok.x) || (hit.y && !ok.y)) == 0ull;
  if constexpr (GATES) {
    const int cw = (int)(upper0 + 0.5f), ch = (int)(upper1 + 0.5f);
    if (full.mnx != INT_MAX) {
      if (gate0 == 2 && full.mnx < 0) clean = false;
      if (gate0 != 0 && full.mxx >= cw - 1) clean = false;
      if (gate1 == 2 && full.mny < 0) clean = false;
      if (gate1 != 0 && full.mxy >= ch - 1) clean = false;
    }
  }
  int npass = 1;
  const int f = eu5_box_fits<order>(full);
  if (f < 0) npass = 0;
  else if (f == 0) {
    npass = 2;
    if (eu5_box_fits<order>(eu5_box_at(h0, h1, h2, h3, 31)) == 0 || eu5_box_fits<order>(eu5_box_at(h0, h1, h2, h3, 63)) == 0) {
      npass = 4;
      if (eu5_box_fits<order>(eu5_box_at(q0, q1, q2, q3, 15)) == 0 || eu5_box_fits<order>(eu5_box_at(q0, q1, q2, q3, 31)) == 0 ||
          eu5_box_fits<order>(eu5_box_at(q0, q1, q2, q3, 47)) == 0 || eu5_box_fits<order>(eu5_box_at(q0, q1, q2, q3, 63)) == 0)
        npass = -1;
    }
  }
  b.q0 = q0; b.q1 = q1; b.q2 = q2; b.q3 = q3; b.h0 = h0; b.h1 = h1; b.h2 = h2; b.h3 = h3;
  b.full = full; b.npass = npass; b.clean = clean;
}

template <int NCH, int DEG, int PRJ, bool HOIST, bool FAST, bool PRE = false>
__device__ __forceinline__ void eu5_tile(const eu_render_params &p, const eu4_plan &w, const float *atab,
                                         float *wtile, const float *ct, int tile_y, int x0, int lane,
                                         const eu5_tab8 *T = nullptr, bool have_n = false, int ty_n = 0, int x0_n = 0,
                                         eu5_tab8 *Tn = nullptr)
{
  static_assert(!PRE || (!HOIST && FAST), "the prefetching form exists for plain FAST tiles");
  constexpr int TEX = 4;
  constexpr int order = DEG + 1;
  const eu_src_dev &s = p.src;
#ifdef EU5_STAMPS
  unsigned long long st_[8] = { 0, 0, 0, 0, 0, 0, 0, 0 };
#endif
  EU5_STAMP(0);
  const int pr = lane & 3, rw = (lane >> 2) & 7, hf = lane >> 5;
  const int y = p.row_begin + tile_y * EU4_TH + rw;
  const bool yin = y < p.row_end;
  const int yc = yin ? y : p.row_end - 1;
  const float *rt = p.row + (long long)(FAST ? yc : eu_frame_row(yc, p.band_shift, p.band_count, p.band_index)) * EU_ROW_FLOATS;
  const int xa = x0 + 8 * hf + 2 * pr, xb = xa + 1;
  const bool va = yin && xa < p.width, vb = yin && xb < p.width;
  const int xac = xa < p.width ? xa : p.width - 1, xbc = xb < p.width ? xb : p.width - 1;

  eu_f2 tx, ty, gy;
  eu_i2 hit, ok = { -1, -1 };
  int ixa, ixb;
  eu_f2 wx[order], wy[order];
  constexpr bool LEAN = FAST && PRJ == EU_SPHERICAL;
  if constexpr (LEAN) {
    hit = (eu_i2){ -1, -1 };
    eu_i2 big0 = { 0, 0 }, big1 = { 0, 0 };
    eu_f2 lat;
    if constexpr (HOIST) {
      const float4 *ea = (const float4 *)(ct + (size_t)xac * EU4_COL_FLOATS);
      const float4 *eb = (const float4 *)(ct + (size_t)xbc * EU4_COL_FLOATS);
      const float4 a0 = ea[0], a1 = ea[1], b0 = eb[0], b1 = eb[1];
      const float A1 = rt[1], B1 = rt[4];
      const eu_f2 c0 = { p.col[xac], p.col[xbc] };
      const eu_f2 ryy = B1 * c0 + A1;
      ixa = __float_as_int(a0.x); ixb = __float_as_int(b0.x);
      tx = (eu_f2){ a0.y, b0.y };
      if constexpr (DEG >= 2) {
        wx[0] = (eu_f2){ a0.z, b0.z }; wx[1] = (eu_f2){ a0.w, b0.w }; wx[2] = (eu_f2){ a1.x, b1.x };
        if constexpr (DEG == 3) wx[3] = (eu_f2){ a1.y, b1.y };
      }
      const eu_f2 qs = { a1.z, b1.z };
      ok = (eu_i2){ (ixa != INT_MIN ? -1 : 0) & ~eu5_out_of_range3(ryy.x, qs.x, qs.x),
                    (ixb != INT_MIN ? -1 : 0) & ~eu5_out_of_range3(ryy.y, qs.y, qs.y) };
      lat = eu_atan2f_2_lean(ryy, qs, atab, 1, big0);
    } else {
      float A0, A1, A2, B0, B1, B2;
      eu_f2 c0;
      if constexpr (PRE) { A0 = T->A0; A1 = T->A1; A2 = T->A2; B0 = T->B0; B1 = T->B1; B2 = T->B2; c0 = T->c0; }
      else {
        A0 = rt[0]; A1 = rt[1]; A2 = rt[2]; B0 = rt[3]; B1 = rt[4]; B2 = rt[5];
        c0 = (eu_f2){ p.col[xac], p.col[xbc] };
      }
      const eu_f2 rx = B0 * c0 + A0, ry = B1 * c0 + A1, rz = B2 * c0 + A2;
      ok = (eu_i2){ ~eu5_out_of_range3(rx.x, ry.x, rz.x), ~eu5_out_of_range3(rx.y, ry.y, rz.y) };
      const eu_f2 q2 = rx * rx + rz * rz;
      const eu_f2 qs = eu_sqrt2_safe(q2);
      lat = eu_atan2f_2_lean(ry, qs, atab, 1, big0);
      const eu_f2 lon = eu_atan2f_2_lean(rx, rz, atab, 0, big1);
      eu_f2 i0 = { (float)((double)lon.x - s.tex_x0), (float)((double)lon.y - s.tex_x0) };
      if (s.cdiv_ok) i0 = eu_div2_const(i0, s.ext_w, s.rcp_ext_w);
      else i0 = eu_div2_rr(i0, s.ext_w, eu_rcp_refined(s.ext_w));
      i0 = i0 * s.total_w; i0 = i0 - .5f;
      const eu_f2 sx = i0 - s.win_x_off;
      const eu_f2 gx = eu5_gate2(sx, s.gate0, s.lower0, s.upper0);
      eu_f2 fx;
      if constexpr (DEG & 1) fx = (eu_f2){ floorf(gx.x), floorf(gx.y) };
      else fx = (eu_f2){ roundf(gx.x), roundf(gx.y) };
      tx = gx - fx;
      ixa = (int)fx.x; ixb = (int)fx.y;
    }
    ok = ok & ~(big0 | big1);
    eu_f2 i1 = { (float)((double)lat.x - s.tex_y0), (float)((double)lat.y - s.tex_y0) };
    if (s.cdiv_ok) i1 = eu_div2_const(i1, s.ext_h, s.rcp_ext_h);
    else i1 = eu_div2_rr(i1, s.ext_h, eu_rcp_refined(s.ext_h));
    i1 = i1 * s.total_h; i1 = i1 - .5f;
    const eu_f2 sy = i1 - s.win_y_off;
    gy = eu5_gate2(sy, s.gate1, s.lower1, s.upper1);
  } else if constexpr (HOIST) {
    const float4 *ea = (const float4 *)(ct + (size_t)xac * EU4_COL_FLOATS);
    const float4 *eb = (const float4 *)(ct + (size_t)xbc * EU4_COL_FLOATS);
    const float4 a0 = ea[0], a1 = ea[1], b0 = eb[0], b1 = eb[1];
    const float A1 = rt[1], B1 = rt[4];
    const eu_f2 c0 = { p.col[xac], p.col[xbc] };
    const eu_f2 ryy = B1 * c0 + A1;
    ixa = __float_as_int(a0.x); ixb = __float_as_int(b0.x);
    ok = ok & (eu_i2){ ixa != INT_MIN ? -1 : 0, ixb != INT_MIN ? -1 : 0 };
    tx = (eu_f2){ a0.y, b0.y };
    if constexpr (DEG >= 2) {
      wx[0] = (eu_f2){ a0.z, b0.z }; wx[1] = (eu_f2){ a0.w, b0.w }; wx[2] = (eu_f2){ a1.x, b1.x };
      if constexpr (DEG == 3) wx[3] = (eu_f2){ a1.y, b1.y };
    }
    const eu_f2 qs = { a1.z, b1.z };
// ... 65 lines not shown
  const eu5_box full = eu5_box_join(eu5_box_at(h0, h1, h2, h3, 31), eu5_box_at(h0, h1, h2, h3, 63));
  bool clean = __ballot((hit.x && !ok.x) || (hit.y && !ok.y)) == 0ull;
  if constexpr (LEAN) {
    const int cw = (int)(s.upper0 + 0.5f), ch = (int)(s.upper1 + 0.5f);
    if (full.mnx != INT_MAX) {
      if (s.gate0 == 2 && full.mnx < 0) clean = false;
      if (s.gate0 != 0 && full.mxx >= cw - 1) clean = false;
      if (s.gate1 == 2 && full.mny < 0) clean = false;
      if (s.gate1 != 0 && full.mxy >= ch - 1) clean = false;
    }
  }
  int npass = 1;
  const int f = eu5_box_fits<order>(full);
  if (f < 0) npass = 0;
  else if (f == 0) {
    npass = 2;
    if (eu5_box_fits<order>(eu5_box_at(h0, h1, h2, h3, 31)) == 0 || eu5_box_fits<order>(eu5_box_at(h0, h1, h2, h3, 63)) == 0) {
      npass = 4;
      if (eu5_box_fits<order>(eu5_box_at(q0, q1, q2, q3, 15)) == 0 || eu5_box_fits<order>(eu5_box_at(q0, q1, q2, q3, 31)) == 0 ||
          eu5_box_fits<order>(eu5_box_at(q0, q1, q2, q3, 47)) == 0 || eu5_box_fits<order>(eu5_box_at(q0, q1, q2, q3, 63)) == 0)
        npass = -1;
    }
  }
  EU5_STAMP(3);
  float *const orow = p.out + (long long)(yc - p.row_begin) * p.out_stride;
  if (npass < 0 || (npass > 0 && !clean)) {
    if (lane == 0) {
      const int id = tile_y * w.tiles16 + x0 / EU4_TW;
      const int sh = eu4_shard_of(id);
      const int slot = atomicAdd(p.wl + EU4_WL_SHARD(sh), 1);
      p.wl[EU4_WL_ENTRIES + (size_t)slot * EU4_SHARDS + sh] = id;
    }
    if constexpr (PRE) { if (have_n) eu5_load8<FAST>(p, ty_n, x0_n, lane, *Tn); }
    return;
  }
  eu_f2 rga = { 0.0f, 0.0f }, bxa = { 0.0f, 0.0f }, rgb = { 0.0f, 0.0f }, bxb = { 0.0f, 0.0f };
  if (npass > 0) {
    const unsigned lds_tile = (unsigned)(unsigned long long)(eu4_lds_void)wtile;
    const int grp = npass == 1 ? 0 : npass == 2 ? hf : (lane >> 4);
#pragma unroll 1
    for (int pi = 0; pi < npass; pi++) {
      eu5_box bx = full;
      if (npass > 1) {
        const int ln = npass == 2 ? 31 + 32 * pi : 15 + 16 * pi;
        const eu5_box bh = eu5_box_at(h0, h1, h2, h3, ln), bq = eu5_box_at(q0, q1, q2, q3, ln);
        bx = npass == 2 ? bh : bq;
      }
      if (bx.mnx == INT_MAX) continue;
      const int ibw = bx.mxx - bx.mnx + order, ibh = bx.mxy - bx.mny + order;
      {
        const unsigned tv = eu5_divtab.v[ibw];
        const int k = (int)(tv >> 24);
        const unsigned r = ((unsigned)lane * (tv & 0x1ffffu)) >> 16, c = (unsigned)lane - r * (unsigned)ibw;
        const int bx0 = bx.mnx - DEG / 2, by0 = bx.mny - DEG / 2;
        const unsigned pitchb = (unsigned)(s.es1 * 4);
        const unsigned voff = r * pitchb + c * (NCH * 4u);
        const char *sb = (const char *)(s.base + ((long long)by0 * s.es1 + (long long)bx0 * NCH));
        const unsigned long long step = (unsigned long long)k * pitchb;
        unsigned dst = lds_tile;
        const unsigned dstep = (unsigned)(k * ibw) * (TEX * 4u);
        int left = ibh;
        if ((int)r < k) {
#pragma unroll 1
          for (; left >= k; left -= k) { eu4_dma_row(dst, voff, sb); sb += step; dst += dstep; }
        }
        left = ibh % k;
        if ((int)r < left) {
          const int full = ibh / k;
          eu4_dma_row(lds_tile + (unsigned)full * dstep, voff,
                      (const char *)(s.base + ((long long)by0 * s.es1 + (long long)bx0 * NCH)) + (unsigned long long)full * step);
        }
      }
      if (pi == 0) {
        if constexpr (DEG >= 2) {
          eu_weights2<DEG>(s.wm, ty, wy);
          if constexpr (!HOIST) eu_weights2<DEG>(s.wm, tx, wx);
        }
      }
      const bool mine = grp == pi;
      const int oa = (mine && hit.x) ? ((iya - bx.mny) * ibw + (ixa - bx.mnx)) * TEX : 0;
      const int ob = (mine && hit.y) ? ((iyb - bx.mny) * ibw + (ixb - bx.mnx)) * TEX : 0;
      if (pi == 0) EU5_STAMP(4);
      asm volatile("s_waitcnt vmcnt(0)" ::: "memory");
      if (pi == 0) EU5_STAMP(5);
      if (mine) eu5_taps<NCH, DEG>((eu_lptr)wtile, oa, ob, ibw * TEX, wx, wy, tx, ty, rga, bxa, rgb, bxb);
    }
  }
#ifdef EU5_STAMPS
  asm volatile("" : : "v"(rga), "v"(bxa), "v"(rgb), "v"(bxb));
#endif
  EU5_STAMP(6);
  float qa[4] = { rga.x, rga.y, bxa.x, bxa.y }, qb[4] = { rgb.x, rgb.y, bxb.x, bxb.y };
  constexpr int ncol = (NCH == 2 || NCH == 4) ? NCH - 1 : NCH;
  const bool bright = !FAST && s.brighten != 1.0f;
#pragma unroll
  for (int c = 0; c < NCH; c++) {
    float a = qa[c], bb = qb[c];
    if (bright && c < ncol) { a = a * s.brighten; bb = bb * s.brighten; }
    qa[c] = hit.x ? a : 0.0f;
    qb[c] = hit.y ? bb : 0.0f;
  }
  if constexpr (PRE) {
    if (have_n) eu5_load8<FAST>(p, ty_n, x0_n, lane, *Tn);
    __builtin_amdgcn_sched_barrier(0);
  }
  if (va) eu_put<NCH>(orow, xa, qa);
  if (vb) eu_put<NCH>(orow, xb, qb);
  EU5_STAMP(7);
#ifdef EU5_STAMPS
  if (lane == 0 && w.stamps) {
    unsigned long long *o = w.stamps + ((size_t)tile_y * w.tiles16 + x0 / EU4_TW) * 8;
    st_[1] = (unsigned long long)(npass + 1) | (HOIST ? 16ull : 0ull);
#pragma unroll
    for (int k = 0; k < 8; k++) o[k] = st_[k];
  }
#endif
}



template <int NCH, int DEG>
__device__ __forceinline__ void eu5_stage(const eu_src_dev &s, const eu5_box &bx, unsigned lds_tile, int lane)
{
  constexpr int order = DEG + 1;
  const int ibw = bx.mxx - bx.mnx + order, ibh = bx.mxy - bx.mny + order;
  const unsigned tv = eu5_divtab.v[ibw];
  const int k = (int)(tv >> 24);
  const unsigned r = ((unsigned)lane * (tv & 0x1ffffu)) >> 16, c = (unsigned)lane - r * (unsigned)ibw;
  const int bx0 = bx.mnx - DEG / 2, by0 = bx.mny - DEG / 2;
  const unsigned pitchb = (unsigned)(s.es1 * 4);
  const unsigned voff = r * pitchb + c * (NCH * 4u);
  const char *const sb0 = (const char *)(s.base + ((long long)by0 * s.es1 + (long long)bx0 * NCH));
  const unsigned long long step = (unsigned long long)k * pitchb;
  const unsigned dstep = (unsigned)(k * ibw) * 16u;
  if ((int)r < k) {
    const char *sb = sb0;
    unsigned dst = lds_tile;
#pragma unroll 1
    for (int left = ibh; left >= k; left -= k) { eu4_dma_row(dst, voff, sb); sb += step; dst += dstep; }
  }
  if ((int)r < ibh % k) {
    const int full = ibh / k;
    eu4_dma_row(lds_tile + (unsigned)full * dstep, voff, sb0 + (unsigned long long)full * step);
  }
}

#define EU5_BT_RECS 4
#define EU5_BT_WORK 8
#define EU5_WAIT_VM0 0x0F70
typedef unsigned eu5_u3 __attribute__((ext_vector_type(3)));
typedef unsigned eu5_u4 __attribute__((ext_vector_type(4)));
typedef int eu5_i4 __attribute__((ext_vector_type(4)));
typedef const __attribute__((address_space(4))) eu5_i4 *eu5_crec;

__device__ __forceinline__ int eu5_bt_pack(const eu5_box &b, int w3, int c)
{
  if (c == 2) return b.mnx == INT_MAX ? -1 : (int)(((unsigned)b.mxx - (unsigned)b.mnx) | (((unsigned)b.mxy - (unsigned)b.mny) << 16));
  return c == 0 ? b.mnx : c == 1 ? b.mny : w3;
}

template <int DEG>
__global__ __launch_bounds__(256) void eu5_boxplan_kernel(const eu_render_params p, const float *atab_g, const int *l2_rows,
                                                          int tiles16, int ntiles, int *tab)
{
  __shared__ __attribute__((aligned(16))) float atab[768];
  const int lane = threadIdx.x & 63;
  const int wave = __builtin_amdgcn_readfirstlane(threadIdx.x >> 6);
  if (wave == 0) {
#pragma unroll
    for (int i = 0; i < 3; i++)
      __builtin_amdgcn_global_load_lds((eu4_gbl_void)(atab_g + i * 256 + lane * 4), (eu4_lds_void)(atab + i * 256), 16, 0, 0);
    asm volatile("s_waitcnt vmcnt(0)" ::: "memory");
  }
  __syncthreads();
  const int g = (int)blockIdx.x * 4 + wave;
  if (g >= ntiles) return;
  const int slot = g / tiles16, tcol = g - slot * tiles16;
  const int tile_y = __builtin_amdgcn_readfirstlane(l2_rows[slot]);
  const int x0 = tcol * EU4_TW;
  const eu_src_dev &s = p.src;
  const int pr = lane & 3, rw = (lane >> 2) & 7, hf = lane >> 5;
  const int y = p.row_begin + tile_y * EU4_TH + rw;
  const bool yin = y < p.row_end;
  const int xa = x0 + 8 * hf + 2 * pr, xb = xa + 1;
  const bool va = yin && xa < p.width, vb = yin && xb < p.width;
  eu5_tab8 T;
  eu5_load8<true>(p, tile_y, x0, lane, T);
  eu5_co8 c;
  eu5_coords8<DEG>(s, atab, T, c);
  eu5_split_y<DEG>(c);
  const eu_i2 hit = { va ? -1 : 0, vb ? -1 : 0 };
  eu5_boxes B;
  eu5_box_stage<DEG, true>(s.gate0, s.gate1, s.upper0, s.upper1, hit, c.ok, c.ixa, c.ixb, c.iya, c.iyb, B);
  const int cls = (B.npass < 0 || (B.npass > 0 && !B.clean)) ? EU5_BT_WORK : B.npass;
  eu5_box r[EU5_BT_RECS] = { B.full, B.full, B.full, B.full };
  if (B.npass == 2) { r[0] = eu5_box_at(B.h0, B.h1, B.h2, B.h3, 31); r[1] = eu5_box_at(B.h0, B.h1, B.h2, B.h3, 63); }
  if (B.npass == 4) {
#pragma unroll
    for (int k = 0; k < 4; k++) r[k] = eu5_box_at(B.q0, B.q1, B.q2, B.q3, 15 + 16 * k);
  }
  int v = 0;
#pragma unroll
  for (int k = 0; k < EU5_BT_RECS; k++) {
#pragma unroll
    for (int i = 0; i < 4; i++)
      if (lane == 4 * k + i) v = eu5_bt_pack(r[k], k == 0 ? cls : 0, i);
  }
  if (lane < 4 * EU5_BT_RECS) tab[(size_t)g * (4 * EU5_BT_RECS) + lane] = v;
}

template <int NCH, int DEG>
__device__ __forceinline__ void eu5_tile_bt(const eu_render_params &p, const eu4_plan &w, const float *atab, float *wtile,
                                            int tile_y, int x0, int lane, const eu5_tab8 &T, eu5_i4 R, eu5_crec rec,
                                            bool have_n, int ty_n, int x0_n, eu5_tab8 &Tn)
{
  constexpr int order = DEG + 1;
  const eu_src_dev &s = p.src;
#ifdef EU5_STAMPS
  unsigned long long st_[8] = { 0, 0, 0, 0, 0, 0, 0, 0 };
#endif
  EU5_STAMP(0);
  const int cls = R.w;
  if (cls & EU5_BT_WORK) {
    if (lane == 0) {
      const int id = tile_y * w.tiles16 + x0 / EU4_TW;
      const int sh = eu4_shard_of(id);
      const int slot = atomicAdd(p.wl + EU4_WL_SHARD(sh), 1);
      p.wl[EU4_WL_ENTRIES + (size_t)slot * EU4_SHARDS + sh] = id;
    }
    if (have_n) eu5_load8<true>(p, ty_n, x0_n, lane, Tn);
    __builtin_amdgcn_s_waitcnt(EU5_WAIT_VM0);
    return;
  }
  const int npass = cls & 7;
  const unsigned lds_tile = (unsigned)(unsigned long long)(eu4_lds_void)wtile;
  eu5_tab8 Tl = T;
  asm volatile("" : "+v"(Tl.c0), "+v"(Tl.A0), "+v"(Tl.A1), "+v"(Tl.A2), "+v"(Tl.B0), "+v"(Tl.B1), "+v"(Tl.B2));
  eu5_box bx = { R.x, R.y, R.x + (R.z & 0xffff), R.y + (R.z >> 16) };
  bool some = npass > 0 && R.z >= 0;
  if (some) eu5_stage<NCH, DEG>(s, bx, lds_tile, lane);
  const int pr = lane & 3, rw = (lane >> 2) & 7, hf = lane >> 5;
  const int y = p.row_begin + tile_y * EU4_TH + rw;
  const bool yin = y < p.row_end;
  const int xa = x0 + 8 * hf + 2 * pr, xb = xa + 1;
  const bool va = yin && xa < p.width, vb = yin && xb < p.width;
  eu_f2 rga = { 0.0f, 0.0f }, bxa = { 0.0f, 0.0f }, rgb = { 0.0f, 0.0f }, bxb = { 0.0f, 0.0f };
  if (npass > 0) {
    eu5_co8 c;
    eu5_coords8<DEG>(s, atab, Tl, c);
    eu5_split_y<DEG>(c);
#ifdef EU5_STAMPS
    asm volatile("" : : "v"(c.iya), "v"(c.iyb), "v"(c.ixa), "v"(c.ixb));
#endif
    EU5_STAMP(2);
#ifdef EU5_STAMPS
    st_[3] = st_[2];
#endif
    eu_f2 wx[order], wy[order];
    if constexpr (DEG >= 2) {
      eu_weights2<DEG>(s.wm, c.ty, wy);
      eu_weights2<DEG>(s.wm, c.tx, wx);
    }
    const int grp = npass == 1 ? 0 : npass == 2 ? hf : (lane >> 4);
#pragma unroll 1
    for (int pi = 0; pi < npass; pi++) {
      eu5_i4 Rn = { 0, 0, -1, 0 };
      if (pi + 1 < npass) Rn = rec[pi + 1];
      if (some) {
        if (pi > 0) eu5_stage<NCH, DEG>(s, bx, lds_tile, lane);
        const int ibw = bx.mxx - bx.mnx + order;
        const bool mine = grp == pi;
        const int oa = (mine && va) ? ((c.iya - bx.mny) * ibw + (c.ixa - bx.mnx)) * 4 : 0;
        const int ob = (mine && vb) ? ((c.iyb - bx.mny) * ibw + (c.ixb - bx.mnx)) * 4 : 0;
        if (pi == 0) EU5_STAMP(4);
        asm volatile("s_waitcnt vmcnt(0)" ::: "memory");
        if (pi == 0) EU5_STAMP(5);
        if (mine) eu5_taps<NCH, DEG>((eu_lptr)wtile, oa, ob, ibw * 4, wx, wy, c.tx, c.ty, rga, bxa, rgb, bxb);
      }
      bx = (eu5_box){ Rn.x, Rn.y, Rn.x + (Rn.z & 0xffff), Rn.y + (Rn.z >> 16) };
      some = Rn.z >= 0;
    }
  }
#ifdef EU5_STAMPS
  asm volatile("" : : "v"(rga), "v"(bxa), "v"(rgb), "v"(bxb));
#endif
  EU5_STAMP(6);
  float qa[4] = { rga.x, rga.y, bxa.x, bxa.y }, qb[4] = { rgb.x, rgb.y, bxb.x, bxb.y };
  if (have_n) eu5_load8<true>(p, ty_n, x0_n, lane, Tn);
  __builtin_amdgcn_sched_barrier(0);
  {
    float *const base = p.out + (long long)(tile_y * EU4_TH) * p.out_stride + (long long)x0 * NCH;
    const __amdgpu_buffer_rsrc_t rs = __builtin_amdgcn_make_buffer_rsrc(base, 0, 0x80000000u, 0x00027000);
    const unsigned off = ((unsigned)rw * (unsigned)p.out_stride + (unsigned)((8 * hf + 2 * pr) * NCH)) * 4u;
    const unsigned oa = va ? off : 0xfffff000u, ob = vb ? oa + NCH * 4u : 0xfffff000u;
    if constexpr (NCH == 3) {
      __builtin_amdgcn_raw_buffer_store_b96((eu5_u3){ __float_as_uint(qa[0]), __float_as_uint(qa[1]), __float_as_uint(qa[2]) }, rs, (int)oa, 0, 0);
      __builtin_amdgcn_raw_buffer_store_b96((eu5_u3){ __float_as_uint(qb[0]), __float_as_uint(qb[1]), __float_as_uint(qb[2]) }, rs, (int)ob, 0, 0);
    } else {
      __builtin_amdgcn_raw_buffer_store_b128((eu5_u4){ __float_as_uint(qa[0]), __float_as_uint(qa[1]), __float_as_uint(qa[2]), __float_as_uint(qa[3]) }, rs, (int)oa, 0, 0);
      __builtin_amdgcn_raw_buffer_store_b128((eu5_u4){ __float_as_uint(qb[0]), __float_as_uint(qb[1]), __float_as_uint(qb[2]), __float_as_uint(qb[3]) }, rs, (int)ob, 0, 0);
    }
  }
  EU5_STAMP(7);
#ifdef EU5_STAMPS
  if (lane == 0 && w.stamps) {
    unsigned long long *o = w.stamps + ((size_t)tile_y * w.tiles16 + x0 / EU4_TW) * 8;
    st_[1] = (unsigned long long)(npass + 1);
#pragma unroll
    for (int k = 0; k < 8; k++) o[k] = st_[k];
  }
#endif
}

struct eu5_tab16 {
  eu4_f4 a0, a1, b0, b1;
  eu_f2 c0;
  float A1A, B1A, A1B, B1B;
};

__device__ __forceinline__ void eu5_load16(const eu_render_params &p, const float *ct, int tile_y, int x0, int lane, eu5_tab16 &T)
{
  const int pr = lane & 3, rw = (lane >> 2) & 7, hf = lane >> 5;
  const int yA = p.row_begin + tile_y * EU4_TH + rw, yB = yA + EU4_TH;
  const int ycA = yA < p.row_end ? yA : p.row_end - 1, ycB = yB < p.row_end ? yB : p.row_end - 1;
  const float *rtA = p.row + (long long)ycA * EU_ROW_FLOATS, *rtB = p.row + (long long)ycB * EU_ROW_FLOATS;
  const int xa = x0 + 8 * hf + 2 * pr, xb = xa + 1;
  const int xac = xa < p.width ? xa : p.width - 1, xbc = xb < p.width ? xb : p.width - 1;
  const eu4_f4 *ea = (const eu4_f4 *)(ct + (size_t)xac * EU4_COL_FLOATS);
  const eu4_f4 *eb = (const eu4_f4 *)(ct + (size_t)xbc * EU4_COL_FLOATS);
  T.a0 = ea[0]; T.a1 = ea[1]; T.b0 = eb[0]; T.b1 = eb[1];
  T.A1A = rtA[1]; T.B1A = rtA[4]; T.A1B = rtB[1]; T.B1B = rtB[4];
  T.c0 = (eu_f2){ p.col[xac], p.col[xbc] };
}

typedef const __attribute__((address_space(4))) int *eu5_cint;

__device__ __forceinline__ void eu5_load_cols(const float *ct, int xa, int xb, eu5_tab16 &T)
{
  const eu4_f4 *ea = (const eu4_f4 *)(ct + (size_t)xa * EU4_COL_FLOATS);
  const eu4_f4 *eb = (const eu4_f4 *)(ct + (size_t)xb * EU4_COL_FLOATS);
  T.a0 = ea[0]; T.a1 = ea[1]; T.b0 = eb[0]; T.b1 = eb[1];
}

__device__ __forceinline__ void eu5_y_reduce(int &mn, int &mx)
{
#define EU5_RED2(ctrl)                                       \
  "v_min_i32_dpp %0, %0, %0 " ctrl "\n\t"                    \
  "v_max_i32_dpp %1, %1, %1 " ctrl "\n\t"                    \
  "s_nop 1\n\t"
  asm("s_nop 1\n\t"
      EU5_RED2("row_shr:1 row_mask:0xf bank_mask:0xf")
      EU5_RED2("row_shr:2 row_mask:0xf bank_mask:0xf")
      EU5_RED2("row_shr:4 row_mask:0xf bank_mask:0xf")
      EU5_RED2("row_shr:8 row_mask:0xf bank_mask:0xf")
      EU5_RED2("row_bcast:15 row_mask:0xa bank_mask:0xf")
      EU5_RED2("row_bcast:31 row_mask:0xc bank_mask:0xf")
      : "+v"(mn), "+v"(mx));
#undef EU5_RED2
  mn = __builtin_amdgcn_readlane(mn, 63); mx = __builtin_amdgcn_readlane(mx, 63);
}

template <int NCH, int DEG>
__device__ __forceinline__ void eu5_group16(const eu_render_params &p, const eu4_plan &w, const float *atab, float *wtile,
                                            eu5_tab16 &T, eu5_cint ent, int n, int m0, int plan0, int tcol, int lane0,
                                            bool have_n, int m_n, int plan_n, int tcol_n)
{
  constexpr int order = DEG + 1;
  const eu_src_dev &s = p.src;
#ifdef EU5_STAMPS
  unsigned st_[8] = { 0, 0, 0, 0, 0, 0, 0, 0 };
#endif
  EU5_STAMP32(0);
  const eu5_cint xt = (eu5_cint)w.xtab;
  int xmn = xt[2 * (plan0 * w.tiles16 + tcol)], xmx = xt[2 * (plan0 * w.tiles16 + tcol) + 1];
  int iyAa, iyAb, iyBa, iyBb, bad, mny = INT_MAX, mxy = INT_MIN;
  eu_f2 tyA, tyB;
  bool off;
  {
    int lane = lane0;
    asm volatile("" : "+v"(lane));
    const int pr = lane & 3, rw = (lane >> 2) & 7, hf = lane >> 5;
    const int yA = p.row_begin + 2 * m0 * EU4_TH + rw, yB = yA + EU4_TH;
    const bool yinA = yA < p.row_end, yinB = yB < p.row_end;
    const int xa = tcol * EU4_TW + 8 * hf + 2 * pr, xb = xa + 1;
    const bool vxa = xa < p.width, vxb = xb < p.width;
    const eu_f2 c0 = T.c0;
    const eu_f2 ryA = T.B1A * c0 + T.A1A, ryB = T.B1B * c0 + T.A1B;
    const eu_f2 qs = { T.a1.z, T.b1.z };
    eu_i2 bigA = { 0, 0 }, bigB = { 0, 0 };
    bad = eu5_out_of_range3(ryA.x, qs.x, ryB.x) | eu5_out_of_range3(ryA.y, qs.y, ryB.y);
    const eu_f2 latA = eu_atan2f_2_lean(ryA, qs, atab, 1, bigA);
    const eu_f2 latB = eu_atan2f_2_lean(ryB, qs, atab, 1, bigB);
    bad |= bigA.x | bigA.y | bigB.x | bigB.y;
    const float rr = s.cdiv_ok ? 0.0f : __int_as_float(__builtin_amdgcn_readfirstlane(__float_as_int(eu_rcp_refined(s.ext_h))));
    eu_f2 iA = { (float)((double)latA.x - s.tex_y0), (float)((double)latA.y - s.tex_y0) };
    eu_f2 iB = { (float)((double)latB.x - s.tex_y0), (float)((double)latB.y - s.tex_y0) };
    if (s.cdiv_ok) { iA = eu_div2_const(iA, s.ext_h, s.rcp_ext_h); iB = eu_div2_const(iB, s.ext_h, s.rcp_ext_h); }
    else { iA = eu_div2_rr(iA, s.ext_h, rr); iB = eu_div2_rr(iB, s.ext_h, rr); }
    iA = iA * s.total_h; iA = iA - .5f; iB = iB * s.total_h; iB = iB - .5f;
    const eu_f2 gyA = eu5_gate2(iA - s.win_y_off, s.gate1, s.lower1, s.upper1);
    const eu_f2 gyB = eu5_gate2(iB - s.win_y_off, s.gate1, s.lower1, s.upper1);
    eu_f2 fyA, fyB;
    if constexpr (DEG & 1) { fyA = (eu_f2){ floorf(gyA.x), floorf(gyA.y) }; fyB = (eu_f2){ floorf(gyB.x), floorf(gyB.y) }; }
    else { fyA = (eu_f2){ roundf(gyA.x), roundf(gyA.y) }; fyB = (eu_f2){ roundf(gyB.x), roundf(gyB.y) }; }
    tyA = gyA - fyA; tyB = gyB - fyB;
    iyAa = (int)fyA.x; iyAb = (int)fyA.y; iyBa = (int)fyB.x; iyBb = (int)fyB.y;
#ifdef EU5_STAMPS
    asm volatile("" : : "v"(iyAa), "v"(iyAb), "v"(iyBa), "v"(iyBb));
#endif
    EU5_STAMP32(2);
    const bool hAa = yinA && vxa, hAb = yinA && vxb, hBa = yinB && vxa, hBb = yinB && vxb;
    int q1 = INT_MAX, q3 = INT_MIN;
    if (hAa) { q1 = iyAa; q3 = iyAa; }
    if (hAb) { q1 = min(q1, iyAb); q3 = max(q3, iyAb); }
    if (hBa) { q1 = min(q1, iyBa); q3 = max(q3, iyBa); }
    if (hBb) { q1 = min(q1, iyBb); q3 = max(q3, iyBb); }
    eu5_y_reduce(q1, q3);
    mny = q1; mxy = q3;
    off = __ballot(bad != 0 && (hAa || hAb || hBa || hBb)) != 0ull;
  }
  EU5_STAMP32(3);
  int mk = m0, pk = plan0;
#pragma unroll 1
  for (int k = 0; k < n; k++) {
    int lane = lane0;
    asm volatile("" : "+v"(lane));
    const int pr = lane & 3, rw = (lane >> 2) & 7, hf = lane >> 5;
    const bool mir = (pk & EU_SHARE_MIRROR) != 0;
    const int tc = mir ? w.tiles16 - 1 - tcol : tcol;
    int mk_n = 0, pk_n = 0;
    if (k + 1 < n) { mk_n = ent[2 * k + 4]; pk_n = ent[2 * k + 5]; }
#ifdef EU5_STAMPS
    if (k > 0) { EU5_STAMP32(0); st_[2] = st_[0]; st_[3] = st_[0]; }
#endif
    eu5_box bx = { xmn, mny, xmx, mxy };
    bool fast = !off && xmn != INT_MAX && mny != INT_MAX;
    if (fast) {
      const int cw = __builtin_amdgcn_readfirstlane((int)(s.upper0 + 0.5f)), ch = __builtin_amdgcn_readfirstlane((int)(s.upper1 + 0.5f));
      if (s.gate0 == 2 && bx.mnx < 0) fast = false;
      if (s.gate0 != 0 && bx.mxx >= cw - 1) fast = false;
      if (s.gate1 == 2 && bx.mny < 0) fast = false;
      if (s.gate1 != 0 && bx.mxy >= ch - 1) fast = false;
      if (eu5_box_fits<order>(bx) != 1) fast = false;
    }
    const int xl = 8 * hf + 2 * pr;
    const int xa = mir ? p.width - 1 - (tcol * EU4_TW + xl) : tc * EU4_TW + xl, xb = mir ? xa - 1 : xa + 1;
    const int yA = p.row_begin + 2 * mk * EU4_TH + rw, yB = yA + EU4_TH;
    const bool yinA = yA < p.row_end, yinB = yB < p.row_end;
    const int ycA = yinA ? yA : p.row_end - 1, ycB = yinB ? yB : p.row_end - 1;
    const bool vxa = xa < p.width, vxb = xb < p.width;
    const bool hAa = yinA && vxa, hAb = yinA && vxb, hBa = yinB && vxa, hBb = yinB && vxb;
    eu_f2 rga = { 0.0f, 0.0f }, bxa = { 0.0f, 0.0f }, rgb = { 0.0f, 0.0f }, bxb = { 0.0f, 0.0f };
    if (fast) eu5_stage<NCH, DEG>(s, bx, (unsigned)(unsigned long long)(eu4_lds_void)wtile, lane);
    const bool mir_n = (pk_n & EU_SHARE_MIRROR) != 0;
    const int plan_k = pk_n & (EU_SHARE_MIRROR - 1);
    const int tc_k = mir_n ? w.tiles16 - 1 - tcol : tcol;
    int xmn_n = INT_MAX, xmx_n = INT_MIN;
    if (k + 1 < n) { xmn_n = xt[2 * (plan_k * w.tiles16 + tc_k)]; xmx_n = xt[2 * (plan_k * w.tiles16 + tc_k) + 1]; }
    if (fast) {
      eu_f2 wx[order], wyA[order], wyB[order];
      const int ixa = __float_as_int(T.a0.x), ixb = __float_as_int(T.b0.x);
      const eu_f2 tx = { T.a0.y, T.b0.y };
      if constexpr (DEG >= 2) {
        wx[0] = (eu_f2){ T.a0.z, T.b0.z }; wx[1] = (eu_f2){ T.a0.w, T.b0.w }; wx[2] = (eu_f2){ T.a1.x, T.b1.x };
        if constexpr (DEG == 3) wx[3] = (eu_f2){ T.a1.y, T.b1.y };
        eu_weights2<DEG>(s.wm, tyA, wyA); eu_weights2<DEG>(s.wm, tyB, wyB);
      }
      const int ibw = bx.mxx - bx.mnx + order;
      const int oAa = hAa ? ((iyAa - bx.mny) * ibw + (ixa - bx.mnx)) * 4 : 0, oAb = hAb ? ((iyAb - bx.mny) * ibw + (ixb - bx.mnx)) * 4 : 0;
      const int oBa = hBa ? ((iyBa - bx.mny) * ibw + (ixa - bx.mnx)) * 4 : 0, oBb = hBb ? ((iyBb - bx.mny) * ibw + (ixb - bx.mnx)) * 4 : 0;
      asm volatile("s_waitcnt vmcnt(0)" ::: "memory");
      __builtin_amdgcn_sched_barrier(0);
      eu5_taps<NCH, DEG>((eu_lptr)wtile, oAa, oAb, ibw * 4, wx, wyA, tx, tyA, rga, bxa, rgb, bxb);
      asm volatile("" : "+v"(rga), "+v"(bxa), "+v"(rgb), "+v"(bxb));
      {
        float qa[4] = { rga.x, rga.y, bxa.x, bxa.y }, qb[4] = { rgb.x, rgb.y, bxb.x, bxb.y };
        float *const orow = p.out + (long long)(ycA - p.row_begin) * p.out_stride;
        if (hAa) eu_put<NCH>(orow, xa, qa);
        if (hAb) eu_put<NCH>(orow, xb, qb);
      }
      __builtin_amdgcn_sched_barrier(0);
      eu5_taps<NCH, DEG>((eu_lptr)wtile, oBa, oBb, ibw * 4, wx, wyB, tx, tyB, rga, bxa, rgb, bxb);
      asm volatile("" : "+v"(rga), "+v"(bxa), "+v"(rgb), "+v"(bxb));
    } else if (mny != INT_MAX) {
      if (lane < 2) {
        const int id = (2 * mk + lane) * w.tiles16 + tc;
        const int sh = eu4_shard_of(id);
        const int slot = atomicAdd(p.wl + EU4_WL_SHARD(sh), 1);
        p.wl[EU4_WL_ENTRIES + (size_t)slot * EU4_SHARDS + sh] = id;
      }
    }
    if (k + 1 < n) {
      const int xa_n = mir_n ? p.width - 1 - (tcol * EU4_TW + xl) : tcol * EU4_TW + xl, xb_n = mir_n ? xa_n - 1 : xa_n + 1;
      const int xac = xa_n < p.width ? xa_n : p.width - 1, xbc = xb_n < p.width ? xb_n : p.width - 1;
      eu5_load_cols(w.coltab + (size_t)plan_k * p.width * EU4_COL_FLOATS, xac, xbc, T);
    } else if (have_n) {
      eu5_load16(p, w.coltab + (size_t)plan_n * p.width * EU4_COL_FLOATS, 2 * m_n, tcol_n * EU4_TW, lane, T);
    }
    __builtin_amdgcn_sched_barrier(0);
    if (fast) {
      float qa[4] = { rga.x, rga.y, bxa.x, bxa.y }, qb[4] = { rgb.x, rgb.y, bxb.x, bxb.y };
      float *const orow = p.out + (long long)(ycB - p.row_begin) * p.out_stride;
      if (hBa) eu_put<NCH>(orow, xa, qa);
      if (hBb) eu_put<NCH>(orow, xb, qb);
    }
    EU5_STAMP32(7);
#ifdef EU5_STAMPS
    if (fast && lane == 0 && w.stamps) {
      unsigned long long *o = w.stamps + ((size_t)(2 * mk) * w.tiles16 + tc) * 8;
      st_[1] = (k == 0 ? 6ull : 7ull) | 16ull;
#pragma unroll
      for (int q = 0; q < 8; q++) o[q] = q == 1 ? st_[1] : (q == 4 || q == 5) ? 0ull : (unsigned long long)st_[q == 6 ? 7 : q] | (1ull << 32);
    }
#endif
    mk = mk_n; pk = pk_n; xmn = xmn_n; xmx = xmx_n;
  }
}

template <int UNIT>
struct eu5_iter {
  int ul, ry, rx;
  int du, dy, dx;
  int xcd, units, tiles16;
  __device__ __forceinline__ void start(int t0, int K)
  {
    const int per_unit = UNIT * tiles16;
    ul = t0 / per_unit;
    ry = (t0 - ul * per_unit) / tiles16;
    rx = t0 - ul * per_unit - ry * tiles16;
    du = K / per_unit; dy = (K - du * per_unit) / tiles16; dx = K - du * per_unit - dy * tiles16;
  }
  __device__ __forceinline__ void step()
  {
    rx += dx; ry += dy; ul += du;
    if (rx >= tiles16) { rx -= tiles16; ry++; }
    if (ry >= UNIT) { ry -= UNIT; ul++; }
  }
  __device__ __forceinline__ bool done() const { return ul * 8 + xcd >= units; }
  __device__ __forceinline__ int row() const { return (ul * 8 + xcd) * UNIT + ry; }
  __device__ __forceinline__ int col() const
  {
    const unsigned h = ((unsigned)row() * 0x9E3779B1u) >> 16;
    int c = rx + (int)((h * (unsigned)tiles16) >> 16);
    if (c >= tiles16) c -= tiles16;
    return c;
  }
};

__device__ __forceinline__ int eu5_pair_plan(const int *tileplan, int tiles_y, int m)
{
  if (2 * m + 1 >= tiles_y) return -1;
  const eu5_cint tp = (eu5_cint)tileplan;
  const int a = tp[2 * m], b = tp[2 * m + 1];
  return a == b ? a : -1;
}

template <int NCH, int DEG, int PRJ, bool FAST, bool BOXTAB = false>
__global__ __launch_bounds__(64 * EU5_WAVES, EU5_OCC) void eu_render5_kernel(const eu_render_params p, const eu4_plan w)
{
  __shared__ __attribute__((aligned(16))) float tile_all[EU5_WAVES * EU5_TEXELS * 4];
  __shared__ __attribute__((aligned(16))) float atab[768];
  const int lane0 = threadIdx.x & 63;
  const int wave = __builtin_amdgcn_readfirstlane(threadIdx.x >> 6);
  float *const tile = tile_all + wave * (EU5_TEXELS * 4);
  if (PRJ != EU_CUBEMAP && wave == 0) {
#pragma unroll
    for (int i = 0; i < 3; i++)
      __builtin_amdgcn_global_load_lds((eu4_gbl_void)(w.atab_g + i * 256 + lane0 * 4),
                                       (eu4_lds_void)(atab + i * 256), 16, 0, 0);
    asm volatile("s_waitcnt vmcnt(0)" ::: "memory");
  }
  __syncthreads();
#ifdef EU5_STAMPS
  const unsigned long long ws0 = __builtin_amdgcn_s_memtime();
  unsigned long long ws1 = ws0;
#endif
  const int xcd = (int)(blockIdx.x & 7);
  const int K = (int)(gridDim.x >> 3) * EU5_WAVES;
  const int t0 = (int)(blockIdx.x >> 3) * EU5_WAVES + wave;
  constexpr bool PAIRS = FAST && PRJ == EU_SPHERICAL;
  if constexpr (PAIRS) {
    const int n1 = (w.l1_off[xcd + 1] - w.l1_off[xcd]) * w.l1_ecols;
    const eu5_cint ents = (eu5_cint)w.l1_ent + EU_SHARE_ENTRY_INTS * w.l1_off[xcd];
    int pos1 = t0;
    auto seek = [&](eu5_cint &e, int &n, int &m, int &plan, int &tcol) -> bool {
      if (pos1 >= n1) return false;
      const int r = (int)(((unsigned long long)(unsigned)pos1 * w.l1_magic) >> 40);
      e = ents + EU_SHARE_ENTRY_INTS * r;
      n = e[0]; m = e[2]; plan = e[3];
      const unsigned h = ((unsigned)m * 0x9E3779B1u) >> 16;
      int c = pos1 - r * w.l1_ecols + (int)((h * (unsigned)w.l1_ecols) >> 16);
      if (c >= w.l1_ecols) c -= w.l1_ecols;
      tcol = e[1] + c;
      pos1 += K;
      return true;
    };
    eu5_cint e_a = ents, e_n = ents;
    int n_a = 0, m_a = 0, col_a = 0, plan_a = 0, n_n = 0, m_n = 0, col_n = 0, plan_n = 0;
    bool have_a = seek(e_a, n_a, m_a, plan_a, col_a);
    eu5_tab16 T;
    if (have_a) eu5_load16(p, w.coltab + (size_t)plan_a * p.width * EU4_COL_FLOATS, 2 * m_a, col_a * EU4_TW, lane0, T);
#pragma unroll 1
    while (have_a) {
      const bool have_n = seek(e_n, n_n, m_n, plan_n, col_n);
      eu5_group16<NCH, DEG>(p, w, atab, tile, T, e_a, n_a, m_a, plan_a, col_a, lane0, have_n, m_n, have_n ? plan_n : 0, col_n);
      e_a = e_n; n_a = n_n; m_a = m_n; plan_a = plan_n; col_a = col_n; have_a = have_n;
    }
  }
#ifdef EU5_STAMPS
  ws1 = __builtin_amdgcn_s_memtime();
#endif
  eu5_iter<EU5_UNIT_ROWS> it;
  it.xcd = xcd; it.tiles16 = w.tiles16;
  it.units = (p.tiles_y + EU5_UNIT_ROWS - 1) / EU5_UNIT_ROWS;
  it.start(t0, K);
  if constexpr (PAIRS) {
    int *const queue = p.wl + EU4_WL_DYN(xcd);
    const int nbatch = (w.l2_off[xcd + 1] - w.l2_off[xcd]) * w.l2_half;
    const eu5_cint rows2 = (eu5_cint)w.l2_rows + w.l2_off[xcd];
    auto take = [&]() -> int {
      int v = 0;
      if (lane0 == 0) v = atomicAdd(queue, 1);
      return v;
    };
    if constexpr (BOXTAB) {
      static_assert(FAST && PRJ == EU_SPHERICAL, "the box table is that of the FAST lat/lon second loop");
      const eu5_crec bt = (eu5_crec)w.boxtab;
      auto decode = [&](int j, int &ty, int &tcol, int &ti) -> bool {
        if (j >= nbatch) return false;
        const int r = (int)(((unsigned long long)(unsigned)j * w.l2_magic) >> 40);
        ty = rows2[r]; tcol = 2 * (j - r * w.l2_half);
        ti = ((w.l2_off[xcd] + r) * w.tiles16 + tcol) * EU5_BT_RECS;
        return true;
      };
      int ty_a = 0, col_a = 0, ti_a = 0, ty_n = 0, col_n = 0, ti_n = 0;
      bool have = decode(__builtin_amdgcn_readfirstlane(take()), ty_a, col_a, ti_a);
      eu5_tab8 Ta, Tb;
      eu5_i4 Ra = { 0, 0, -1, 0 }, Rb = { 0, 0, -1, 0 };
      if (have) { Ra = bt[ti_a]; eu5_load8<FAST>(p, ty_a, col_a * EU4_TW, lane0, Ta); }
      __builtin_amdgcn_s_waitcnt(EU5_WAIT_VM0);
#pragma unroll 1
      while (have) {
        const int jn_lane = take();
        const bool second = col_a + 1 < w.tiles16;
        if (second) Rb = bt[ti_a + EU5_BT_RECS];
        {
          int lane = lane0;
          asm volatile("" : "+v"(lane));
          eu5_tile_bt<NCH, DEG>(p, w, atab, tile, ty_a, col_a * EU4_TW, lane, Ta, Ra, bt + ti_a, second, ty_a,
                                (col_a + 1) * EU4_TW, Tb);
        }
        const bool have_n = decode(__builtin_amdgcn_readfirstlane(jn_lane), ty_n, col_n, ti_n);
        if (have_n) Ra = bt[ti_n];
        if (second) {
          int lane = lane0;
          asm volatile("" : "+v"(lane));
          eu5_tile_bt<NCH, DEG>(p, w, atab, tile, ty_a, (col_a + 1) * EU4_TW, lane, Tb, Rb, bt + ti_a + EU5_BT_RECS, have_n,
                                ty_n, col_n * EU4_TW, Ta);
        } else if (have_n) {
          eu5_load8<FAST>(p, ty_n, col_n * EU4_TW, lane0, Ta);
          __builtin_amdgcn_s_waitcnt(EU5_WAIT_VM0);
        }
        ty_a = ty_n; col_a = col_n; ti_a = ti_n; have = have_n;
      }
    } else {
      auto decode = [&](int j, int &ty, int &tcol) -> bool {
        if (j >= nbatch) return false;
        const int r = (int)(((unsigned long long)(unsigned)j * w.l2_magic) >> 40);
        ty = rows2[r]; tcol = 2 * (j - r * w.l2_half);
        return true;
      };
      int ty_a = 0, col_a = 0, ty_n = 0, col_n = 0;
      bool have = decode(__builtin_amdgcn_readfirstlane(take()), ty_a, col_a);
      eu5_tab8 Ta, Tb;
      if (have) eu5_load8<FAST>(p, ty_a, col_a * EU4_TW, lane0, Ta);
  #pragma unroll 1
      while (have) {
        const int jn_lane = take();
        const bool second = col_a + 1 < w.tiles16;
        {
          int lane = lane0;
          asm volatile("" : "+v"(lane));
          eu5_tile<NCH, DEG, PRJ, false, FAST, true>(p, w, atab, tile, nullptr, ty_a, col_a * EU4_TW, lane, &Ta, second, ty_a,
                                                     (col_a + 1) * EU4_TW, &Tb);
        }
        const bool have_n = decode(__builtin_amdgcn_readfirstlane(jn_lane), ty_n, col_n);
        if (second) {
          int lane = lane0;
          asm volatile("" : "+v"(lane));
          eu5_tile<NCH, DEG, PRJ, false, FAST, true>(p, w, atab, tile, nullptr, ty_a, (col_a + 1) * EU4_TW, lane, &Tb, have_n, ty_n,
                                                     col_n * EU4_TW, &Ta);
        } else if (have_n) eu5_load8<FAST>(p, ty_n, col_n * EU4_TW, lane0, Ta);
        ty_a = ty_n; col_a = col_n; have = have_n;
      }
    }
  } else {
    int plan_n = (it.done() || it.row() >= p.tiles_y) ? -2 : (PRJ == EU_SPHERICAL ? ((eu5_cint)w.tileplan)[it.row()] : -1);
#pragma unroll 1
    while (!it.done()) {
      const int tile_y = it.row(), tcol = it.col(), plan = plan_n;
      it.step();
      plan_n = (it.done() || it.row() >= p.tiles_y) ? -2 : (PRJ == EU_SPHERICAL ? ((eu5_cint)w.tileplan)[it.row()] : -1);
      if (plan == -2) continue;
      int lane = lane0;
      asm volatile("" : "+v"(lane));
      if (plan >= 0)
        eu5_tile<NCH, DEG, PRJ, PRJ == EU_SPHERICAL, FAST>(p, w, atab, tile, w.coltab + (size_t)plan * p.width * EU4_COL_FLOATS,
                                                            tile_y, tcol * EU4_TW, lane);
      else
        eu5_tile<NCH, DEG, PRJ, false, FAST>(p, w, atab, tile, nullptr, tile_y, tcol * EU4_TW, lane);
    }
  }
#ifdef EU5_STAMPS
  if (lane0 == 0 && w.stamps) {
    unsigned long long *o = w.stamps + (size_t)w.tiles16 * p.tiles_y * 8 + ((size_t)blockIdx.x * EU5_WAVES + wave) * 4;
    o[0] = ws0; o[1] = ws1; o[2] = __builtin_amdgcn_s_memtime(); o[3] = 1;
  }
#endif
}
```

envutil_amd/csrc/eu_select.h:

```cpp
#ifndef EU_SELECT_H
#define EU_SELECT_H
#include <algorithm>
#include <climits>
#include <cstdlib>
#include <vector>
#include "eu_device.h"
#include "eu_share_groups.h"
#include "eu_worklist.h"

struct eu_switches {
  int force_general;
  int hybrid;
  int r4;
  int colmajor;
  int rej;
  int colplan;
  int share;
  int direct;
  int iir_stream;
  int boxtab;
  int boxtab_max_kb;
  int views_max_kb;
  int layers_max;
};

#define EU_BOXTAB_MAX_KB 65536
#define EU_VIEWS_MAX_KB 65536
#define EU_LAYERS_MAX 4

inline eu_switches eu_read_switches()
{
  auto first = [](const char *name) { const char *e = getenv(name); return e ? e[0] : '\0'; };
  eu_switches s;
  s.force_general = first("EU_HIP_KERNEL") == '1';
  const char hy = first("EU_HIP_HYBRID");
  s.hybrid = hy == '0' ? 0 : hy == '2' ? 2 : 1;
  const char *r4 = getenv("EU_HIP_R4");
  s.r4 = r4 ? atoi(r4) : -1;
  const char *cm = getenv("EU_HIP_COLMAJOR");
  s.colmajor = cm && cm[0] ? atoi(cm) : -1;
  const char rj = first("EU_HIP_REJ");
  s.rej = rj == '1' ? 1 : rj == '2' ? 2 : 0;
  s.colplan = first("EU_HIP_COLPLAN") != '0';
  const char sh = first("EU_HIP_SHARE");
  s.share = sh == '0' ? 0 : sh == 'm' ? EU_SHARE_MIRRORS : sh == 'f' ? EU_SHARE_FACES : EU_SHARE_FACES | EU_SHARE_MIRRORS;
  s.direct = first("EU_HIP_DIRECT") == '1';
  const char *iir = getenv("EU_HIP_IIR_STREAM");
  s.iir_stream = iir ? atoi(iir) : 7;
  s.boxtab = first("EU_HIP_BOXTAB") != '0';
  const char *bm = getenv("EU_HIP_BOXTAB_MAX_KB");
  s.boxtab_max_kb = bm && bm[0] ? std::max(0, std::min(atoi(bm), 16 * 1024 * 1024)) : EU_BOXTAB_MAX_KB;
  const char *vm = getenv("EU_HIP_VIEWS_MAX_KB");
  s.views_max_kb = vm && vm[0] ? std::max(0, std::min(atoi(vm), 16 * 1024 * 1024)) : EU_VIEWS_MAX_KB;
  const char *lm = getenv("EU_HIP_LAYERS_MAX");
  s.layers_max = lm && lm[0] ? std::max(0, atoi(lm)) : EU_LAYERS_MAX;
  return s;
}

inline bool eu_cube_source(int prj) { return prj == EU_CUBEMAP || prj == EU_BIATAN6; }

inline bool eu_packed_covers_source(const eu_src_dev &s, int nch, int nch_out)
{
  if (s.has_lcp || nch_out != nch) return false;
  if (s.prj != EU_SPHERICAL && !eu_cube_source(s.prj)) return false;
  if (s.degree < 1 || s.degree > 3 || s.es0 != nch) return false;
  return nch >= 1 && nch <= 4;
}
inline bool eu_packed_covers(const eu_render_params &p)
{
  if (p.stage != 0 || p.form >= EU_FORM_FISH) return false;
  return eu_packed_covers_source(p.src, p.nch, p.nch_out);
}

#define EU_STAGED_TILE_ROWS 8
#define EU_STAGED_TILE_COLS 16
#define EU_STAGED_MAX_TILES_Y (65535 * 8 * 4)
inline unsigned long long eu_staged_tiles(int width, int row_begin, int row_end)
{
  const long long tx = ((long long)width + EU_STAGED_TILE_COLS - 1) / EU_STAGED_TILE_COLS;
  const long long ty = ((long long)row_end - row_begin + EU_STAGED_TILE_ROWS - 1) / EU_STAGED_TILE_ROWS;
  return tx > 0 && ty > 0 ? (unsigned long long)tx * (unsigned long long)ty : 0ull;
}
inline bool eu_staged_covers(const eu_render_params &p)
{
  if (!eu_packed_covers(p) || p.twine) return false;
  if (p.norm_mode != EU_NORM_NONE && p.norm_mode != EU_NORM_DIV) return false;
  if (p.nch != 3 && p.nch != 4) return false;
  if (p.src.es1 * 4 >= (1ll << 31)) return false;
  if ((p.row_end - p.row_begin + EU_STAGED_TILE_ROWS - 1) / EU_STAGED_TILE_ROWS > EU_STAGED_MAX_TILES_Y) return false;
  return eu_staged_tiles(p.width, p.row_begin, p.row_end) <= EU4_WL_MAX_TILES;
}

inline bool eu_plain_ba(const eu_render_params &p)
{
  return p.form == EU_FORM_BA && p.norm_mode == EU_NORM_NONE && p.band_count <= 1 && p.src.brighten == 1.0f &&
         p.src.always_hit;
}

inline bool eu_staged_default(const eu_render_params &p)
{
  return p.src.prj == EU_SPHERICAL && p.src.degree >= 2 && !p.twine && eu_plain_ba(p);
}

inline bool eu_staged_fast_profile(const eu_render_params &p)
{
  auto mag_ok = [](double v) { const double a = v < 0 ? -v : v; return a == 0.0 || (a >= 0x1p-20 && a <= 0x1p20); };
  return eu_plain_ba(p) && mag_ok(p.src.tex_x0) && mag_ok(p.src.tex_y0) && p.src.ext_w >= 0x1p-20f &&
         p.src.ext_w <= 0x1p20f && p.src.ext_h >= 0x1p-20f && p.src.ext_h <= 0x1p20f && p.tab_finite;
}

inline bool eu_staged_worth(int degree, int planned_rows, int tiles_y)
{
  return degree >= 2 && planned_rows * 2 >= tiles_y;
}

enum eu_path { EU_PATH_GENERAL, EU_PATH_GENERAL_DIRECT, EU_PATH_PACKED, EU_PATH_PACKED_RUNS, EU_PATH_STAGED };

inline eu_path eu_select_path(const eu_render_params &p, const eu_switches &sw, bool staged_allowed = true)
{
  if (p.src.mask_paint) return EU_PATH_GENERAL_DIRECT;
  if (sw.force_general) return EU_PATH_GENERAL;
  const bool want_staged = sw.r4 == 1 || (sw.r4 != 0 && p.src.degree >= 2 && (eu_cube_source(p.src.prj) || eu_staged_default(p)));
  if (staged_allowed && want_staged && eu_staged_covers(p)) return EU_PATH_STAGED;
  if (!eu_packed_covers(p)) return EU_PATH_GENERAL;
  const bool worth = sw.hybrid == 2 || p.src.degree >= 2;
  if (sw.hybrid && worth && !p.twine && p.norm_mode == EU_NORM_NONE && p.src.prj == EU_SPHERICAL) return EU_PATH_PACKED_RUNS;
  return EU_PATH_PACKED;
}

enum eu_ray_path { EU_RAYS_GENERAL, EU_RAYS_PACKED };

inline eu_ray_path eu_select_ray_path(const eu_rays_params &p, const eu_switches &sw)
{
  if (p.src.mask_paint || sw.force_general) return EU_RAYS_GENERAL;
  return eu_packed_covers_source(p.src, p.nch, p.nch_out) ? EU_RAYS_PACKED : EU_RAYS_GENERAL;
}

enum eu_view_path { EU_VIEWS_GENERAL, EU_VIEWS_PACKED };

inline eu_view_path eu_select_view_path(const eu_render_params &p, const eu_switches &sw)
{
  if (p.src.mask_paint || sw.force_general) return EU_VIEWS_GENERAL;
  return eu_packed_covers(p) ? EU_VIEWS_PACKED : EU_VIEWS_GENERAL;
}

#define EU_VIEWS_MAX_GRID_Y 65535
inline int eu_views_per_chunk(int width, int height, int max_kb, int nfct = 1)
{
  const unsigned long long nf = (unsigned long long)std::max(nfct, 1);
  const unsigned long long per = nf * ((unsigned long long)6 * width + (unsigned long long)EU_ROW_FLOATS * height) * sizeof(float);
  const unsigned long long n = per ? (unsigned long long)max_kb * 1024ull / per : EU_VIEWS_MAX_GRID_Y;
  return (int)std::max<unsigned long long>(1, std::min<unsigned long long>(n, EU_VIEWS_MAX_GRID_Y / nf));
}

enum eu_layer_path { EU_LAYERS_GENERAL, EU_LAYERS_PACKED };

inline eu_layer_path eu_select_layer_path(const eu_render_params &p, const eu_switches &sw)
{
  if (p.src.mask_paint || sw.force_general) return EU_LAYERS_GENERAL;
  return eu_packed_covers(p) ? EU_LAYERS_PACKED : EU_LAYERS_GENERAL;
}

#ifndef EU_LAYERS_GROUP
#define EU_LAYERS_GROUP 1
#endif

constexpr int eu_layers_per_launch(int nlayers, int layers_max)
{
  return layers_max > 0 && layers_max < nlayers ? layers_max : nlayers;
}
constexpr int eu_layers_launches(int nlayers, int layers_max)
{
  return eu_layers_per_launch(nlayers, layers_max) > 0
             ? (nlayers + eu_layers_per_launch(nlayers, layers_max) - 1) / eu_layers_per_launch(nlayers, layers_max) : 0;
}
constexpr int eu_layers_groups(int n, int group = EU_LAYERS_GROUP) { return n > 0 ? (n + group - 1) / group : 0; }
constexpr int eu_layers_in_group(int n, int g, int group = EU_LAYERS_GROUP)
{
  return n - g * group <= 0 ? 0 : n - g * group < group ? n - g * group : group;
}

#define EU_SEG_ROWS 512

struct eu_run { int row_begin, row_end, layout; };

inline std::vector<eu_run> eu_split_runs(const unsigned char *flags, int nflags, const eu_render_params &p, bool any)
{
  std::vector<eu_run> runs;
  bool mixed = false;
  for (int k = 0; k < nflags; k++) mixed = mixed || flags[k];
  if (!mixed) return runs;
  auto flag_of = [&](int r) {
    const int fy = eu_frame_row(std::min(r, p.row_end - 1), p.band_shift, p.band_count, p.band_index);
    return (int)flags[std::min(fy / EU_SEG_ROWS, nflags - 1)];
  };
  auto run_end = [&](int a, int fl) {
    int b = std::min((a / 64 + 1) * 64, p.row_end);
    while (b < p.row_end && flag_of(b) == fl) b = std::min(b + 64, p.row_end);
// ... 17 lines not shown
```

envutil_amd/csrc/eu_share_groups.h:

```cpp
#ifndef EU_SHARE_GROUPS_H
#define EU_SHARE_GROUPS_H
#include <climits>
#include <cstddef>
#include <cstring>
#include <vector>

#define EU_SHARE_MAX_MEMBERS 8
#define EU_SHARE_ENTRY_INTS (2 + 2 * EU_SHARE_MAX_MEMBERS)
#define EU_SHARE_MIRROR (1 << 30)
#define EU_SHARE_FACES 1
#define EU_SHARE_MIRRORS 2

struct eu_share_input {
  int width, tiles16;
  int row_begin, row_end;
  int band_mode;
  int ncand;
  const int *cand_m, *cand_plan;
  const float *h_row;
  size_t h_row_floats;
  int row_floats;
  const float *coltab;
  int col_floats, nplans;
  int mode;
  int unit_drows;
};

struct eu_share_result {
  std::vector<int> entries;
  int off[9];
  int ecols;
  long long follower_tiles;
  std::vector<int> xtab;
};

namespace eu_share_detail {
inline bool is_zero_bits(float v) { unsigned u; memcpy(&u, &v, 4); return (u & 0x7fffffffu) == 0; }
inline int ix_of(const eu_share_input &in, int plan, int x)
{
  int v; memcpy(&v, in.coltab + ((size_t)plan * in.width + x) * in.col_floats, 4); return v;
}
inline unsigned qs_of(const eu_share_input &in, int plan, int x)
{
  unsigned v; memcpy(&v, in.coltab + ((size_t)plan * in.width + x) * in.col_floats + 6, 4); return v;
}
}

inline void eu_share_build(const eu_share_input &in, eu_share_result &out)
{
  using namespace eu_share_detail;
  const int W = in.width, T = in.tiles16, np = in.nplans;
  out.xtab.assign((size_t)(np > 0 ? np : 1) * T * 2, 0);
  std::vector<char> plan_clean((size_t)(np > 0 ? np : 1), 1);
  for (int pl = 0; pl < np; pl++)
    for (int t = 0; t < T; t++) {
      int mn = INT_MAX, mx = INT_MIN;
      bool okc = true;
      for (int x = 16 * t; x < 16 * t + 16 && x < W; x++) {
        const int ix = ix_of(in, pl, x);
        if (ix == INT_MIN) okc = false;
        mn = ix < mn ? ix : mn; mx = ix > mx ? ix : mx;
      }
      if (!okc) { mn = INT_MAX; mx = INT_MIN; plan_clean[(size_t)pl] = 0; }
      out.xtab[((size_t)pl * T + t) * 2] = mn; out.xtab[((size_t)pl * T + t) * 2 + 1] = mx;
    }
  const bool share_ok = in.mode != 0 && !in.band_mode && in.h_row && in.coltab;
  const bool half = share_ok && (in.mode & EU_SHARE_MIRRORS) && W % 16 == 0 && T % 2 == 0;
  out.ecols = half ? T / 2 : T;
  out.follower_tiles = 0;
  const int n = in.ncand;
  std::vector<char> can((size_t)n, 0), done((size_t)n, 0);
  std::vector<float> a1((size_t)n * 16, 0.0f);
  for (int i = 0; share_ok && i < n; i++) {
    const int y0 = in.row_begin + 16 * in.cand_m[i];
    const int pl = in.cand_plan[i];
    if (y0 + 16 > in.row_end || pl < 0 || pl >= np || !plan_clean[(size_t)pl]) continue;
    bool ok = true;
    for (int r = 0; r < 16 && ok; r++) {
      const size_t fr = (size_t)(y0 + r) * in.row_floats;
      if (fr + 6 > in.h_row_floats) { ok = false; break; }
      const float A1 = in.h_row[fr + 1], B1 = in.h_row[fr + 4];
      ok = is_zero_bits(B1) && !is_zero_bits(A1);
      a1[(size_t)i * 16 + r] = A1;
    }
    can[(size_t)i] = ok;
  }
  std::vector<char> memo((size_t)(np > 0 ? np : 1) * (np > 0 ? np : 1) * 2, 0);
  auto qs_eq = [&](int pa, int pb, int mirror) -> bool {
    char &m = memo[((size_t)pa * np + pb) * 2 + mirror];
    if (!m) {
      m = 1;
      for (int x = 0; x < W; x++)
        if (qs_of(in, pa, x) != qs_of(in, pb, mirror ? W - 1 - x : x)) { m = 2; break; }
    }
    return m == 1;
  };
  std::vector<int> lists[8];
  auto emit = [&](int xcd, int colbase, const std::vector<int> &mem) {
    std::vector<int> &l = lists[xcd];
    const size_t at = l.size();
    l.resize(at + EU_SHARE_ENTRY_INTS, 0);
    l[at] = (int)mem.size() / 2; l[at + 1] = colbase;
    for (size_t k = 0; k < mem.size(); k++) l[at + 2 + k] = mem[k];
    out.follower_tiles += (long long)(mem.size() / 2 - 1) * out.ecols;
  };
  for (int i = 0; i < n; i++) {
    if (done[(size_t)i]) continue;
    done[(size_t)i] = 1;
    const int pi = in.cand_plan[i];
    const bool mirrored = half && can[(size_t)i] && qs_eq(pi, pi, 1);
    std::vector<int> faces(1, i);
    const int max_faces = mirrored ? EU_SHARE_MAX_MEMBERS / 2 : EU_SHARE_MAX_MEMBERS;
    if (can[(size_t)i] && (in.mode & EU_SHARE_FACES))
      for (int j = i + 1; j < n && (int)faces.size() < max_faces; j++) {
        if (done[(size_t)j] || !can[(size_t)j]) continue;
        if (memcmp(&a1[(size_t)i * 16], &a1[(size_t)j * 16], 16 * sizeof(float)) != 0) continue;
        const int pj = in.cand_plan[j];
        if (!qs_eq(pi, pj, 0)) continue;
        if (mirrored && !qs_eq(pi, pj, 1)) continue;
        done[(size_t)j] = 1;
        faces.push_back(j);
      }
    std::vector<int> mem;
    for (int f : faces) {
      mem.push_back(in.cand_m[f]); mem.push_back(in.cand_plan[f]);
      if (mirrored) { mem.push_back(in.cand_m[f]); mem.push_back(in.cand_plan[f] | EU_SHARE_MIRROR); }
    }
    const int xcd = (in.cand_m[i] / (in.unit_drows > 0 ? in.unit_drows : 1)) & 7;
    emit(xcd, 0, mem);
    if (half && !mirrored) emit(xcd, T / 2, mem);
  }
  out.entries.clear();
  for (int x = 0; x < 8; x++) {
    out.off[x] = (int)(out.entries.size() / EU_SHARE_ENTRY_INTS);
    out.entries.insert(out.entries.end(), lists[x].begin(), lists[x].end());
  }
  out.off[8] = (int)(out.entries.size() / EU_SHARE_ENTRY_INTS);
}
#endif
```

include/eu_hip.h:

```cpp
#ifndef EU_HIP_H
#define EU_HIP_H

#include <stddef.h>
#include <stdint.h>

#ifdef __cplusplus
extern "C" {
#endif

typedef enum {
  EU_SPHERICAL = 0, EU_CYLINDRICAL, EU_RECTILINEAR, EU_STEREOGRAPHIC,
  EU_FISHEYE, EU_CUBEMAP, EU_BIATAN6, EU_PRJ_NONE
} eu_projection;

typedef enum {
  EU_BC_MIRROR = 0, EU_BC_PERIODIC, EU_BC_REFLECT, EU_BC_NATURAL,
  EU_BC_CONSTANT, EU_BC_ZEROPAD, EU_BC_GUESS
} eu_bc;

typedef enum {
  EU_OK = 0,
  EU_ERR_NO_DEVICE = -1,
  EU_ERR_ARGUMENT = -2,
  EU_ERR_UNSUPPORTED = -3,
  EU_ERR_MEMORY = -4,
  EU_ERR_HANDLE = -5
} eu_status;

#define EU_MAX_DEGREE 9
#define EU_MAX_TAPS 1024
#define EU_MAX_FACETS 64

typedef struct eu_facet {
  int32_t projection;
  int32_t nchannels;
  double  hfov;
  int32_t width, height;
  int32_t window_width, window_height, window_x_offset, window_y_offset;
  double  yaw, pitch, roll;
  double  brighten;
  double  step;
  int32_t has_lcp;
  double  a, b, c, h, v, s, shear_g, shear_t;
  double  tr_x, tr_y, tr_z, tp_y, tp_p, tp_r;
  int32_t mask_paint;
} eu_facet;

typedef struct eu_source eu_source;

typedef struct eu_container {
  int64_t shape[2];
  int64_t left[2], right[2];
  int64_t core[2];
} eu_container;

typedef struct eu_target {
  int32_t projection;
  int32_t width, height;
  double  x0, x1, y0, y1;
  double  yaw, pitch, roll;
  int32_t nchannels;
  int32_t ntaps;
  const float *taps;
  int32_t row_begin, row_end;
  int32_t stage;
  int32_t crop_x0, crop_y0, crop_w, crop_h;
  int32_t out_format;
  int32_t band_rows, band_count, band_index;
  int32_t synopsis;
  const eu_facet *single;
} eu_target;

int  eu_hip_layout_segments(const eu_target *trg, eu_source *const *srcs, int nsrc,
                            unsigned char *flags, int max_flags, int *seg_rows);

unsigned long long eu_hip_launch_count(void);

unsigned long long eu_hip_share_follower_tiles(void);

unsigned long long eu_hip_listed_tiles(void);

int  eu_hip_band_rows(int height, int band_rows, int band_count, int band_index);

enum { EU_OUT_FLOAT = 0, EU_OUT_SRGBA8 = 1 };
enum { EU_SYN_PANORAMA = 0, EU_SYN_HDR_MERGE = 1 };

int  eu_hip_device_count(void);
int  eu_hip_init(int device);
const char *eu_hip_last_error(void);

#define EU_MAX_SLOTS 16
int  eu_hip_init_devices(const int *devices, int ndevices);
int  eu_hip_device_slots(void);
int  eu_hip_render_devices(const eu_target *trg, eu_source *const *srcs, int nsrc, float *out,
                           size_t out_row_stride_bytes, int out_on_device);
int  eu_hip_device_strips(const eu_target *trg, eu_source *const *srcs, int nsrc, int *begin, int *end);

int  eu_hip_get_extent(int projection, int width, int height, double hfov,
                       double *x0x1y0y1);
double eu_hip_get_step(int projection, int width, int height, double hfov);
int  eu_hip_make_spread(int w, int h, float d, float sigma, float threshold,
                        float *taps, int max_taps);
typedef struct eu_mask_polygon { int n; const float *x; const float *y; } eu_mask_polygon;
int  eu_hip_facet_alpha(float *pixels, int width, int height, int nchannels,
                        const eu_mask_polygon *polygons, int npolygons, int crop_kind,
                        int crop_x0, int crop_x1, int crop_y0, int crop_y1, float *alpha_out);
int  eu_hip_facet_alpha_rows(int width, int height, const eu_mask_polygon *polygons, int npolygons,
                             int crop_kind, int crop_x0, int crop_x1, int crop_y0, int crop_y1,
                             int32_t *keep, int32_t *row_start, int32_t *spans, int max_spans);
typedef struct eu_facet_edit {
  const eu_mask_polygon *polygons; int32_t npolygons;
  int32_t crop_kind, crop_x0, crop_x1, crop_y0, crop_y1;
  int32_t pixel_channels;
  int32_t pixels_on_device;
} eu_facet_edit;
int  eu_hip_facet_alpha_dev(void *pixels_dev, int width, int height, int nchannels,
                            const eu_facet_edit *edit, float *alpha_out_dev, void *stream);
int  eu_hip_cubemap_metrics(int face_px, double face_fov, int support_min,
                            int tile_px, int64_t *section_px,
                            int64_t *left_frame_px, double *refc_md,
                            double *model_to_px);
int  eu_hip_container_geometry(int degree, int bc0, int bc1, int64_t w,
                               int64_t h, eu_container *out);

int  eu_hip_source_load(const eu_facet *fct, const float *pixels,
                        int spline_degree, int prefilter_degree,
                        int support_min, int tile_size, eu_source **out);
int  eu_hip_source_load_edited(const eu_facet *fct, const void *pixels, const eu_facet_edit *edit,
                               int spline_degree, int prefilter_degree, int support_min,
                               int tile_size, eu_source **out);
typedef struct eu_samples {
  const void *data;
  int32_t bits;
  int32_t big_endian;
  int32_t pixel_channels;
  int32_t on_device;
  const float *colour_table;
  const float *alpha_table;
} eu_samples;
int  eu_hip_source_load_samples(const eu_facet *fct, const eu_samples *smp, const eu_facet_edit *edit,
                                int spline_degree, int prefilter_degree, int support_min, int tile_size,
                                eu_source **out);
typedef struct eu_rgbe {
  const void *data;
  int32_t on_device;
  const float *colour_table;
} eu_rgbe;
int  eu_hip_source_load_rgbe(const eu_facet *fct, const eu_rgbe *px, const eu_facet_edit *edit, int spline_degree,
                             int prefilter_degree, int support_min, int tile_size, eu_source **out);
int  eu_hip_source_adopt(const eu_facet *fct, const float *container,
                         int spline_degree, int bc0, int bc1,
                         int support_min, int tile_size, eu_source **out);
int  eu_hip_source_alloc(const eu_facet *fct, int spline_degree,
                         int support_min, int tile_size, eu_source **out);
int  eu_hip_source_update_facet(eu_source *src, const eu_facet *fct);
int  eu_hip_source_device_ptr(const eu_source *src, void **dev_ptr,
                              size_t *nfloats);
int  eu_hip_source_download(const eu_source *src, float *container,
                            size_t nfloats);
int  eu_hip_source_info(const eu_source *src, eu_container *geom, int *nch);
int  eu_hip_source_release(eu_source *src);

int  eu_hip_render(const eu_target *trg, eu_source *const *srcs, int nsrc,
                   float *out, size_t out_row_stride_bytes, int out_on_device,
                   void *stream);
int  eu_hip_sync(void);

int  eu_hip_render_timed(const eu_target *trg, eu_source *const *srcs, int nsrc,
                         float *out_dev, size_t out_row_stride_bytes,
                         int iters, float *mean_ms);

typedef struct eu_rays {
  int32_t width, height;
  int32_t ninputs;
  int32_t nchannels;
  int32_t ntaps; const float *taps;
  const float *rays; size_t ray_row_stride_bytes; int32_t rays_on_device;
} eu_rays;
int  eu_hip_render_rays(const eu_rays *r, eu_source *src, float *out,
                        size_t out_row_stride_bytes, int out_on_device, void *stream);
int  eu_hip_render_rays_timed(const eu_rays *r, eu_source *src, float *out_dev,
                              size_t out_row_stride_bytes, int iters, float *mean_ms);

typedef struct eu_view {
  double yaw, pitch, roll;
  double x0, x1, y0, y1;
} eu_view;
int  eu_hip_render_views(const eu_target *trg, const eu_view *views, int nviews, eu_source *src, float *out,
                         size_t out_row_stride_bytes, size_t out_view_stride_bytes, int out_on_device, void *stream);
int  eu_hip_render_views_multi(const eu_target *trg, const eu_view *views, int nviews, eu_source *const *srcs, int nsrc,
                               float *out, size_t out_row_stride_bytes, size_t out_view_stride_bytes, int out_on_device,
                               void *stream);
int  eu_hip_view_tables(const eu_target *trg, const eu_view *view, eu_source *src, float *col_dev_built,
                        float *row_dev_built, float *col_host_built, float *row_host_built);

int  eu_hip_render_layers(const eu_target *trg, eu_source *const *layers, int nlayers, float *out,
                          size_t out_row_stride_bytes, size_t out_layer_stride_bytes, int out_on_device, void *stream);
int  eu_hip_layers_group(void);

typedef struct eu_encode {
  int32_t bits;
  int32_t big_endian;
  const float *colour_steps;
  const float *alpha_steps;
} eu_encode;
int  eu_hip_encode_samples(const float *frame, size_t frame_row_stride_bytes, int frame_on_device,
                           int width, int height, int nchannels, const eu_encode *enc,
                           void *out, size_t out_row_stride_bytes, int out_on_device, void *stream);
int  eu_hip_render_samples(const eu_target *trg, eu_source *const *srcs, int nsrc, const eu_encode *enc,
                           void *out, size_t out_row_stride_bytes, int out_on_device, void *stream);

int  eu_hip_encode_rgbe(const float *frame, size_t frame_row_stride_bytes, int frame_on_device, int width, int height,
                        void *out, size_t out_row_stride_bytes, int out_on_device, void *stream);
int  eu_hip_render_rgbe(const eu_target *trg, eu_source *const *srcs, int nsrc, void *out,
                        size_t out_row_stride_bytes, int out_on_device, void *stream);

int  eu_hip_malloc(void **p, size_t bytes);
int  eu_hip_free(void *p);
int  eu_hip_memcpy_d2h(void *dst, const void *src, size_t bytes);
int  eu_hip_memcpy_h2d(void *dst, const void *src, size_t bytes);

#ifdef __cplusplus
}
#endif
#endif
```

Before: 109,200.

## Share box-table second-loop tiles across polar row twins and column mirrors

Adds a host-side grouping pass for the box-table second loop. It finds tile rows whose coordinate frames are vertical flips of each other (twins) and columns that are sign-mirrored, then emits worklist entries in which one leader tile's computed coordinates and weights serve several follower tiles via flip/mirror flags. The kernel's box-table path is rewritten to walk these entries, with prefetch of the next entry's tile. The aim is to avoid recomputing geometry and setup for symmetric tiles of a lat/lon to cubemap reprojection, at the cost of more complex per-tile output scatter and a rebuilt pipelining loop.

After: 113,000 (median of 6 runs). 3.5% higher.

```diff
diff --git a/envutil_amd/csrc/eu_api_render.hip b/envutil_amd/csrc/eu_api_render.hip
--- a/envutil_amd/csrc/eu_api_render.hip
+++ b/envutil_amd/csrc/eu_api_render.hip
@@ -327,7 +327,8 @@
   eu_render_params q = *p;
   q.wl = cur().staged.wl.p;
   if (cur().staged.wl_pair.order_after(st) != hipSuccess) return -1;
-  const int rc = eu_launch_render4(&q, &sw, cur().plan.h_row.data(), cur().plan.h_row.size(), cur().plan.plan_gen, st, launches);
+  const int rc = eu_launch_render4(&q, &sw, cur().plan.h_row.data(), cur().plan.h_row.size(), cur().plan.h_col.data(),
+                                   cur().plan.h_col.size(), cur().plan.plan_gen, st, launches);
   if (rc || !*launches) return rc;
   return cur().staged.wl_pair.note(st) != hipSuccess ? -1 : 0;
 }
diff --git a/envutil_amd/csrc/eu_launch.h b/envutil_amd/csrc/eu_launch.h
--- a/envutil_amd/csrc/eu_launch.h
+++ b/envutil_amd/csrc/eu_launch.h
@@ -61,7 +61,7 @@
 int eu_launch_render(const eu_render_params *p, void *stream);
 int eu_launch_render2(const eu_render_params *p, const eu_switches *sw, void *stream);
 int eu_launch_render4(const eu_render_params *p, const eu_switches *sw, const float *h_row, size_t h_row_floats,
-                      unsigned long long plan_gen, void *stream, int *launches);
+                      const float *h_col, size_t h_col_floats, unsigned long long plan_gen, void *stream, int *launches);
 int eu_launch_render_rays(const eu_rays_params *p, int path, void *stream);
 int eu_launch_view_tables(const eu_view_dev *views, int nviews, int prj, int width, int height, int twine, float *col,
                           float *row, void *stream);
diff --git a/envutil_amd/csrc/eu_polar_groups.h b/envutil_amd/csrc/eu_polar_groups.h
--- /dev/null
+++ b/envutil_amd/csrc/eu_polar_groups.h
@@ -0,0 +1,176 @@
+#ifndef EU_POLAR_GROUPS_H
+#define EU_POLAR_GROUPS_H
+#include <algorithm>
+#include <cstddef>
+#include <cstring>
+#include <map>
+#include <utility>
+#include <vector>
+#include "eu_share_groups.h"
+
+#define EU_POLAR_MAX_MEMBERS 4
+#define EU_POLAR_ENTRY_INTS 12
+#define EU_POLAR_FLIP (1 << 29)
+#define EU_POLAR_MIRROR (1 << 30)
+#define EU_TILE_ROWS 8
+#define EU_PLAN_MAX 16
+#define EU_SECOND_LOOP_UNIT_ROWS 4
+
+struct eu_polar_input {
+  int width, tiles16;
+  int row_begin, row_end;
+  int band_mode;
+  int nrows;
+  const int *rows;
+  const float *h_row;
+  size_t h_row_floats;
+  int row_floats;
+  const float *h_col;
+  size_t h_col_floats;
+  int mode;
+  int unit_rows;
+};
+
+struct eu_polar_result {
+  std::vector<int> entries;
+  int off[9];
+  int ecols;
+  int bcols;
+  long long follower_tiles;
+};
+
+namespace eu_polar_detail {
+inline unsigned bits_of(float v) { unsigned u; memcpy(&u, &v, 4); return u; }
+inline bool is_zero_bits(float v) { return (bits_of(v) & 0x7fffffffu) == 0; }
+}
+
+template <class FrameRow>
+inline void eu_tile_row_plans(const float *h_row, size_t h_row_floats, int row_floats, int row_begin, int row_end,
+                              FrameRow frame_row, std::vector<int> &tileplan, std::vector<float> &plans)
+{
+  const int tiles_y = (row_end - row_begin + EU_TILE_ROWS - 1) / EU_TILE_ROWS;
+  tileplan.assign((size_t)(tiles_y > 0 ? tiles_y : 0), -1);
+  plans.clear();
+  for (int ty = 0; h_row && ty < tiles_y; ty++) {
+    float k[4] = { 0, 0, 0, 0 };
+    bool same = true;
+    for (int ly = 0; ly < EU_TILE_ROWS && same; ly++) {
+      const int y = std::min(row_begin + ty * EU_TILE_ROWS + ly, row_end - 1);
+      const size_t fr = (size_t)frame_row(y) * row_floats;
+      if (fr + 6 > h_row_floats) { same = false; break; }
+      const float c[4] = { h_row[fr + 0], h_row[fr + 2], h_row[fr + 3], h_row[fr + 5] };
+      if (ly == 0) memcpy(k, c, sizeof k);
+      else same = memcmp(k, c, sizeof k) == 0;
+    }
+    if (!same) continue;
+    int id = -1;
+    for (size_t j = 0; j < plans.size() / 4 && id < 0; j++)
+      if (memcmp(&plans[4 * j], k, sizeof k) == 0) id = (int)j;
+    if (id < 0 && plans.size() / 4 < EU_PLAN_MAX) {
+      id = (int)(plans.size() / 4);
+      plans.insert(plans.end(), k, k + 4);
+    }
+    tileplan[(size_t)ty] = id;
+  }
+}
+
+inline void eu_second_loop_rows(const std::vector<int> &tileplan, int unit_rows, std::vector<int> &rows, int off[9])
+{
+  const int ty = (int)tileplan.size();
+  auto paired = [&](int m) { return 2 * m + 1 < ty && tileplan[(size_t)2 * m] >= 0 && tileplan[(size_t)2 * m] == tileplan[(size_t)2 * m + 1]; };
+  std::vector<int> per[8];
+  for (int r = 0; r < ty; r++)
+    if (!paired(r >> 1)) per[(r / unit_rows) & 7].push_back(r);
+  rows.clear();
+  for (int x = 0; x < 8; x++) { off[x] = (int)rows.size(); rows.insert(rows.end(), per[x].begin(), per[x].end()); }
+  off[8] = (int)rows.size();
+}
+
+inline void eu_polar_build(const eu_polar_input &in, eu_polar_result &out)
+{
+  using namespace eu_polar_detail;
+  const int W = in.width, T = in.tiles16, n = in.nrows, rf = in.row_floats;
+  const bool share_ok = in.mode != 0 && !in.band_mode && in.h_row && in.h_col;
+  bool colmirror = share_ok && (in.mode & EU_POLAR_MIRRORS) && W > 0 && W % 16 == 0 && T % 2 == 0 && in.h_col_floats >= (size_t)W;
+  for (int x = 0; colmirror && x < W; x++)
+    colmirror = !is_zero_bits(in.h_col[x]) && bits_of(in.h_col[W - 1 - x]) == (bits_of(in.h_col[x]) ^ 0x80000000u);
+  out.ecols = colmirror ? T / 2 : T;
+  out.follower_tiles = 0;
+  std::vector<char> plain((size_t)n, 0), done((size_t)n, 0);
+  auto frame_row = [&](int i, int k) { return in.h_row + (size_t)(in.row_begin + 8 * in.rows[i] + k) * rf; };
+  for (int i = 0; share_ok && i < n; i++) {
+    const long long y0 = (long long)in.row_begin + 8ll * in.rows[i];
+    if (y0 < 0 || y0 + 8 > in.row_end || (size_t)(y0 + 8) * rf > in.h_row_floats) continue;
+    bool ok = true;
+    for (int k = 0; k < 8 && ok; k++) {
+      const float *r = frame_row(i, k);
+      ok = is_zero_bits(r[0]) && is_zero_bits(r[4]) && is_zero_bits(r[5]);
+    }
+    plain[(size_t)i] = ok;
+  }
+  std::map<std::pair<unsigned, unsigned>, std::vector<int>> by_last;
+  const bool twins = share_ok && (in.mode & EU_POLAR_TWINS);
+  for (int i = 0; twins && i < n; i++)
+    if (plain[(size_t)i]) {
+      const float *r = frame_row(i, 7);
+      by_last[std::make_pair(bits_of(r[2]), bits_of(r[1]) & 0x7fffffffu)].push_back(i);
+    }
+  auto twin_of = [&](int i) -> int {
+    if (!twins || !plain[(size_t)i]) return -1;
+    const float *r0 = frame_row(i, 0);
+    auto it = by_last.find(std::make_pair(bits_of(r0[2]), bits_of(r0[1]) & 0x7fffffffu));
+    if (it == by_last.end()) return -1;
+    for (int j : it->second) {
+      if (j == i || done[(size_t)j]) continue;
+      bool ok = true;
+      for (int k = 0; k < 8 && ok; k++) {
+        const float *a = frame_row(i, k), *b = frame_row(j, 7 - k);
+        ok = bits_of(a[2]) == bits_of(b[2]) && bits_of(a[3]) == bits_of(b[3]) && !is_zero_bits(a[1]) &&
+             bits_of(a[1]) == (bits_of(b[1]) ^ 0x80000000u);
+      }
+      if (ok) return j;
+    }
+    return -1;
+  };
+  std::vector<int> order((size_t)n);
+  for (int i = 0; i < n; i++) order[(size_t)i] = i;
+  std::stable_sort(order.begin(), order.end(), [&](int a, int b) { return in.rows[a] < in.rows[b]; });
+  std::vector<int> lists[8];
+  bool all_followed = n > 0;
+  for (int oi = 0; oi < n; oi++) {
+    const int i = order[(size_t)oi];
+    if (done[(size_t)i]) continue;
+    done[(size_t)i] = 1;
+    const int j = twin_of(i);
+    if (j >= 0) done[(size_t)j] = 1;
+    const bool mirrored = colmirror && plain[(size_t)i];
+    int mem[2 * EU_POLAR_MAX_MEMBERS], nm = 0;
+    auto add = [&](int slot, int flags) { mem[2 * nm] = in.rows[slot] | flags; mem[2 * nm + 1] = slot; nm++; };
+    add(i, 0);
+    if (mirrored) add(i, EU_POLAR_MIRROR);
+    if (j >= 0) {
+      add(j, EU_POLAR_FLIP);
+      if (mirrored) add(j, EU_POLAR_FLIP | EU_POLAR_MIRROR);
+    }
+    if (nm < 2) all_followed = false;
+    const int xcd = (in.rows[i] / (in.unit_rows > 0 ? in.unit_rows : 1)) & 7;
+    auto emit = [&](int colbase) {
+      std::vector<int> &l = lists[xcd];
+      const size_t at = l.size();
+      l.resize(at + EU_POLAR_ENTRY_INTS, 0);
+      l[at] = nm; l[at + 1] = colbase;
+      for (int k = 0; k < 2 * nm; k++) l[at + 2 + k] = mem[k];
+      out.follower_tiles += (long long)(nm - 1) * out.ecols;
+    };
+    emit(0);
+    if (colmirror && !mirrored) emit(T / 2);
+  }
+  out.bcols = all_followed ? 1 : 2;
+  out.entries.clear();
+  for (int x = 0; x < 8; x++) {
+    out.off[x] = (int)(out.entries.size() / EU_POLAR_ENTRY_INTS);
+    out.entries.insert(out.entries.end(), lists[x].begin(), lists[x].end());
+  }
+  out.off[8] = (int)(out.entries.size() / EU_POLAR_ENTRY_INTS);
+}
+#endif
diff --git a/envutil_amd/csrc/eu_render4.hip b/envutil_amd/csrc/eu_render4.hip
--- a/envutil_amd/csrc/eu_render4.hip
+++ b/envutil_amd/csrc/eu_render4.hip
@@ -4,6 +4,7 @@
 #include <algorithm>
 #include "eu_packed_dev.h"
 #include "eu_launch.h"
+#include "eu_polar_groups.h"
 
 #define EU4_TW 16
 #define EU4_TH 8
@@ -69,6 +70,10 @@
   unsigned long long l1_magic;
   const int *xtab;
   const int *boxtab;
+  const int *l2p_ent;
+  int l2p_off[9];
+  int l2p_ecols, l2p_bcols, l2p_bpe;
+  unsigned long long l2p_magic;
 #ifdef EU5_STAMPS
   unsigned long long *stamps;
 #endif
@@ -373,6 +378,8 @@
 
 static long long eu4_followers_plan = 0, eu4_followers_last = 0;
 extern "C" unsigned long long eu_hip_share_follower_tiles(void) { return (unsigned long long)eu4_followers_last; }
+static long long eu4_polar_plan = 0, eu4_polar_last = 0;
+extern "C" unsigned long long eu_hip_polar_follower_tiles(void) { return (unsigned long long)eu4_polar_last; }
 static int eu4_boxtab_last = 0;
 static long long eu4_boxtab_tiles_last = 0;
 extern "C" int eu_hip_boxtab_used(void) { return eu4_boxtab_last; }
@@ -409,6 +416,7 @@
     if (wgs <= 0) return -1;
     if (fast) eu4_followers_last = eu4_followers_plan;
     eu4_boxtab_last = bt;
+    if (bt) eu4_polar_last = eu4_polar_plan;
     if (bt) hipLaunchKernelGGL((eu_render5_kernel<NCH, DEG, PRJ, true, true>), dim3((unsigned)wgs), dim3(64 * EU5_WAVES), 0, st, p, w);
     else if (fast) hipLaunchKernelGGL((eu_render5_kernel<NCH, DEG, PRJ, true>), dim3((unsigned)wgs), dim3(64 * EU5_WAVES), 0, st, p, w);
     else hipLaunchKernelGGL((eu_render5_kernel<NCH, DEG, PRJ, false>), dim3((unsigned)wgs), dim3(64 * EU5_WAVES), 0, st, p, w);
@@ -452,7 +460,7 @@
 namespace {
 struct plan_cache {
   std::vector<unsigned char> key;
-  eu_dev_buf<int> tileplan, l2_rows, l1_ent, xtab, boxtab;
+  eu_dev_buf<int> tileplan, l2_rows, l1_ent, xtab, boxtab, l2p_ent;
   bool has_boxtab = false;
   long long boxtab_tiles = 0;
   eu_dev_buf<float> coltab;
@@ -462,6 +470,9 @@
   int l1_off[9] = {};
   int l1_ecols = 1;
   long long follower_tiles = 0;
+  int l2p_off[9] = {};
+  int l2p_ecols = 1, l2p_bcols = 2;
+  long long polar_follower_tiles = 0;
 } g4s[EU_MAX_SLOTS];
 #define g4 (g4s[eu_current_slot()])
 
@@ -483,13 +494,13 @@
 
 std::vector<unsigned char> eu4_plan_key(const eu_render_params &p, unsigned long long plan_gen, const eu_switches &sw)
 {
-  std::vector<unsigned char> key(sizeof(unsigned long long) + sizeof(eu_src_dev) + 11 * sizeof(int));
+  std::vector<unsigned char> key(sizeof(unsigned long long) + sizeof(eu_src_dev) + 12 * sizeof(int));
   unsigned char *q = key.data();
   memcpy(q, &plan_gen, sizeof plan_gen); q += sizeof plan_gen;
   eu_src_dev sd = p.src; sd.base = nullptr;
   memcpy(q, &sd, sizeof sd); q += sizeof sd;
-  const int v[11] = { p.width, p.row_begin, p.row_end, p.band_shift, p.band_count, p.band_index, p.form, p.norm_mode, sw.share,
-                      sw.boxtab, sw.boxtab_max_kb };
+  const int v[12] = { p.width, p.row_begin, p.row_end, p.band_shift, p.band_count, p.band_index, p.form, p.norm_mode, sw.share,
+                      sw.boxtab, sw.boxtab_max_kb, sw.polar_share };
   memcpy(q, v, sizeof v);
   return key;
 }
@@ -508,34 +519,16 @@
 }
 
 int eu4_build_plans(const eu_render_params &p, int tiles16, const eu_switches &sw, const float *h_row,
-                    size_t h_row_floats, hipStream_t st)
-{
+                    size_t h_row_floats, const float *h_col, size_t h_col_floats, hipStream_t st)
+{
+  static_assert(EU_TILE_ROWS == EU4_TH && EU_PLAN_MAX == EU4_MAX_PLANS && EU_SECOND_LOOP_UNIT_ROWS == EU5_UNIT_ROWS,
+                "eu_polar_groups.h: what a host program takes for the launcher's constants");
   std::vector<int> tp((size_t)p.tiles_y, -1);
   std::vector<float> plans;
   const bool can = p.form == EU_FORM_BA && p.norm_mode == EU_NORM_NONE && h_row;
-  if (can && sw.colplan) {
-    for (int ty = 0; ty < p.tiles_y; ty++) {
-      float k[4] = { 0, 0, 0, 0 };
-      bool same = true;
-      for (int ly = 0; ly < EU4_TH && same; ly++) {
-        const int y = std::min(p.row_begin + ty * EU4_TH + ly, p.row_end - 1);
-        const size_t fr = (size_t)eu_frame_row(y, p.band_shift, p.band_count, p.band_index) * EU_ROW_FLOATS;
-        if (fr + 6 > h_row_floats) { same = false; break; }
-        const float c[4] = { h_row[fr + 0], h_row[fr + 2], h_row[fr + 3], h_row[fr + 5] };
-        if (ly == 0) memcpy(k, c, sizeof k);
-        else same = memcmp(k, c, sizeof k) == 0;
-      }
-      if (!same) continue;
-      int id = -1;
-      for (size_t j = 0; j < plans.size() / 4 && id < 0; j++)
-        if (memcmp(&plans[4 * j], k, sizeof k) == 0) id = (int)j;
-      if (id < 0 && plans.size() / 4 < EU4_MAX_PLANS) {
-        id = (int)(plans.size() / 4);
-        plans.insert(plans.end(), k, k + 4);
-      }
-      tp[(size_t)ty] = id;
-    }
-  }
+  if (can && sw.colplan)
+    eu_tile_row_plans(h_row, h_row_floats, EU_ROW_FLOATS, p.row_begin, p.row_end,
+                      [&](int y) { return eu_frame_row(y, p.band_shift, p.band_count, p.band_index); }, tp, plans);
   const int nplans = (int)(plans.size() / 4);
   if (hipStreamSynchronize(st) != hipSuccess) return -1;
   if (g4.tileplan.reserve(tp.size()) != hipSuccess) return -1;
@@ -545,12 +538,22 @@
   for (int v : tp) g4.planned_rows += v >= 0;
   auto paired = [&](int m) { return 2 * m + 1 < p.tiles_y && tp[(size_t)2 * m] >= 0 && tp[(size_t)2 * m] == tp[(size_t)2 * m + 1]; };
   {
-    std::vector<int> rows[8], all;
-    for (int r = 0; r < p.tiles_y; r++)
-      if (!paired(r >> 1)) rows[(r / EU5_UNIT_ROWS) & 7].push_back(r);
-    for (int x = 0; x < 8; x++) { g4.l2_off[x] = (int)all.size(); all.insert(all.end(), rows[x].begin(), rows[x].end()); }
-    g4.l2_off[8] = (int)all.size();
+    std::vector<int> all;
+    eu_second_loop_rows(tp, EU5_UNIT_ROWS, all, g4.l2_off);
     if (!upload(g4.l2_rows, all, 1)) return -1;
+    eu_polar_input pin;
+    pin.width = p.width; pin.tiles16 = tiles16; pin.row_begin = p.row_begin; pin.row_end = p.row_end;
+    pin.band_mode = p.band_count > 1;
+    pin.nrows = (int)all.size(); pin.rows = all.data();
+    pin.h_row = h_row; pin.h_row_floats = h_row_floats; pin.row_floats = EU_ROW_FLOATS;
+    pin.h_col = h_col; pin.h_col_floats = h_col_floats;
+    pin.mode = can ? sw.polar_share : 0; pin.unit_rows = EU5_UNIT_ROWS;
+    eu_polar_result pr;
+    eu_polar_build(pin, pr);
+    if (!upload(g4.l2p_ent, pr.entries, EU_POLAR_ENTRY_INTS)) return -1;
+    for (int x = 0; x < 9; x++) g4.l2p_off[x] = pr.off[x];
+    g4.l2p_ecols = pr.ecols; g4.l2p_bcols = pr.bcols;
+    g4.polar_follower_tiles = pr.follower_tiles;
   }
   g4.has_boxtab = false; g4.boxtab_tiles = 0;
   if (sw.boxtab && eu_staged_fast_profile(p)) {
@@ -618,6 +621,11 @@
   w.l1_magic = (1ull << 40) / (unsigned long long)w.l1_ecols + 1;
   w.xtab = g4.xtab.p;
   w.boxtab = g4.has_boxtab ? g4.boxtab.p : nullptr;
+  w.l2p_ent = g4.l2p_ent.p;
+  for (int x = 0; x < 9; x++) w.l2p_off[x] = g4.l2p_off[x];
+  w.l2p_ecols = g4.l2p_ecols; w.l2p_bcols = g4.l2p_bcols;
+  w.l2p_bpe = std::max(1, (w.l2p_ecols + w.l2p_bcols - 1) / w.l2p_bcols);
+  w.l2p_magic = (1ull << 40) / (unsigned long long)w.l2p_bpe + 1;
 }
 
 int launch4(const eu_render_params &p, const eu4_plan &w, hipStream_t st)
@@ -676,10 +684,10 @@
 }
 
 extern "C" int eu_launch_render4(const eu_render_params *pp, const eu_switches *sw, const float *h_row, size_t h_row_floats,
-                                 unsigned long long plan_gen, void *stream, int *launches)
+                                 const float *h_col, size_t h_col_floats, unsigned long long plan_gen, void *stream, int *launches)
 {
   eu_render_params p = *pp;
-  eu4_followers_last = 0;
+  eu4_followers_last = 0; eu4_polar_last = 0;
   eu4_boxtab_last = 0; eu4_boxtab_tiles_last = 0;
   *launches = 2;
   if (!eu_staged_covers(p) || !p.wl) return -2;
@@ -693,13 +701,14 @@
   if (p.src.prj == EU_SPHERICAL) {
     std::vector<unsigned char> key = eu4_plan_key(p, plan_gen, *sw);
     if (key != g4.key) {
-      if (eu4_build_plans(p, w.tiles16, *sw, h_row, h_row_floats, st)) return -1;
+      if (eu4_build_plans(p, w.tiles16, *sw, h_row, h_row_floats, h_col, h_col_floats, st)) return -1;
       g4.key.swap(key);
     }
     if (sw->r4 != 1 && !eu_staged_worth(p.src.degree, g4.planned_rows, p.tiles_y)) { *launches = 0; return 0; }
   }
   eu4_fill_plan(w);
   eu4_followers_plan = g4.follower_tiles;
+  eu4_polar_plan = g4.polar_follower_tiles;
   eu4_boxtab_tiles_last = w.boxtab ? g4.boxtab_tiles : 0;
 #ifdef EU5_STAMPS
   return launch4_stamped(p, w, st);
diff --git a/envutil_amd/csrc/eu_render5.h b/envutil_amd/csrc/eu_render5.h
--- a/envutil_amd/csrc/eu_render5.h
+++ b/envutil_amd/csrc/eu_render5.h
@@ -155,8 +155,12 @@
   eu_i2 ok;
 };
 
-template <int DEG>
-__device__ __forceinline__ void eu5_coords8(const eu_src_dev &s, const float *atab, const eu5_tab8 &T, eu5_co8 &c)
+struct eu5_ang8 {
+  eu_f2 lon, lat;
+  eu_i2 ok;
+};
+
+__device__ __forceinline__ void eu5_angles8(const float *atab, const eu5_tab8 &T, eu5_ang8 &a)
 {
   eu_i2 big0 = { 0, 0 }, big1 = { 0, 0 };
   const eu_f2 c0 = T.c0;
@@ -164,9 +168,14 @@
   const eu_i2 ok = { ~eu5_out_of_range3(rx.x, ry.x, rz.x), ~eu5_out_of_range3(rx.y, ry.y, rz.y) };
   const eu_f2 q2 = rx * rx + rz * rz;
   const eu_f2 qs = eu_sqrt2_safe(q2);
-  const eu_f2 lat = eu_atan2f_2_lean(ry, qs, atab, 1, big0);
-  const eu_f2 lon = eu_atan2f_2_lean(rx, rz, atab, 0, big1);
-  c.ok = ok & ~(big0 | big1);
+  a.lat = eu_atan2f_2_lean(ry, qs, atab, 1, big0);
+  a.lon = eu_atan2f_2_lean(rx, rz, atab, 0, big1);
+  a.ok = ok & ~(big0 | big1);
+}
+
+template <int DEG>
+__device__ __forceinline__ void eu5_spline_xy(const eu_src_dev &s, eu_f2 lon, eu_f2 lat, eu5_co8 &c)
+{
   eu_f2 i0 = { (float)((double)lon.x - s.tex_x0), (float)((double)lon.y - s.tex_x0) };
   if (s.cdiv_ok) i0 = eu_div2_const(i0, s.ext_w, s.rcp_ext_w);
   else i0 = eu_div2_rr(i0, s.ext_w, eu_rcp_refined(s.ext_w));
@@ -184,6 +193,15 @@
   i1 = i1 * s.total_h; i1 = i1 - .5f;
   const eu_f2 sy = i1 - s.win_y_off;
   c.ty = eu5_gate2(sy, s.gate1, s.lower1, s.upper1);
+}
+
+template <int DEG>
+__device__ __forceinline__ void eu5_coords8(const eu_src_dev &s, const float *atab, const eu5_tab8 &T, eu5_co8 &c)
+{
+  eu5_ang8 a;
+  eu5_angles8(atab, T, a);
+  c.ok = a.ok;
+  eu5_spline_xy<DEG>(s, a.lon, a.lat, c);
 }
 
 template <int DEG>
@@ -555,6 +573,7 @@
 typedef unsigned eu5_u4 __attribute__((ext_vector_type(4)));
 typedef int eu5_i4 __attribute__((ext_vector_type(4)));
 typedef const __attribute__((address_space(4))) eu5_i4 *eu5_crec;
+typedef const __attribute__((address_space(4))) int *eu5_cint;
 
 __device__ __forceinline__ int eu5_bt_pack(const eu5_box &b, int w3, int c)
 {
@@ -614,106 +633,158 @@
 
 template <int NCH, int DEG>
 __device__ __forceinline__ void eu5_tile_bt(const eu_render_params &p, const eu4_plan &w, const float *atab, float *wtile,
-                                            int tile_y, int x0, int lane, const eu5_tab8 &T, eu5_i4 R, eu5_crec rec,
-                                            bool have_n, int ty_n, int x0_n, eu5_tab8 &Tn)
+                                            int lane0, eu5_tab8 &T, eu5_i4 R, eu5_cint ent, int n, int m0, int slot0,
+                                            int tcol, bool have_n, int ty_n, int x0_n)
 {
   constexpr int order = DEG + 1;
   const eu_src_dev &s = p.src;
+  const eu5_crec bt = (eu5_crec)w.boxtab;
+  const unsigned lds_tile = (unsigned)(unsigned long long)(eu4_lds_void)wtile;
 #ifdef EU5_STAMPS
   unsigned long long st_[8] = { 0, 0, 0, 0, 0, 0, 0, 0 };
 #endif
   EU5_STAMP(0);
-  const int cls = R.w;
-  if (cls & EU5_BT_WORK) {
-    if (lane == 0) {
-      const int id = tile_y * w.tiles16 + x0 / EU4_TW;
-      const int sh = eu4_shard_of(id);
-      const int slot = atomicAdd(p.wl + EU4_WL_SHARD(sh), 1);
-      p.wl[EU4_WL_ENTRIES + (size_t)slot * EU4_SHARDS + sh] = id;
-    }
-    if (have_n) eu5_load8<true>(p, ty_n, x0_n, lane, Tn);
-    __builtin_amdgcn_s_waitcnt(EU5_WAIT_VM0);
-    return;
-  }
-  const int npass = cls & 7;
-  const unsigned lds_tile = (unsigned)(unsigned long long)(eu4_lds_void)wtile;
-  eu5_tab8 Tl = T;
-  asm volatile("" : "+v"(Tl.c0), "+v"(Tl.A0), "+v"(Tl.A1), "+v"(Tl.A2), "+v"(Tl.B0), "+v"(Tl.B1), "+v"(Tl.B2));
-  eu5_box bx = { R.x, R.y, R.x + (R.z & 0xffff), R.y + (R.z >> 16) };
-  bool some = npass > 0 && R.z >= 0;
-  if (some) eu5_stage<NCH, DEG>(s, bx, lds_tile, lane);
-  const int pr = lane & 3, rw = (lane >> 2) & 7, hf = lane >> 5;
-  const int y = p.row_begin + tile_y * EU4_TH + rw;
-  const bool yin = y < p.row_end;
-  const int xa = x0 + 8 * hf + 2 * pr, xb = xa + 1;
-  const bool va = yin && xa < p.width, vb = yin && xb < p.width;
-  eu_f2 rga = { 0.0f, 0.0f }, bxa = { 0.0f, 0.0f }, rgb = { 0.0f, 0.0f }, bxb = { 0.0f, 0.0f };
-  if (npass > 0) {
-    eu5_co8 c;
-    eu5_coords8<DEG>(s, atab, Tl, c);
-    eu5_split_y<DEG>(c);
-#ifdef EU5_STAMPS
-    asm volatile("" : : "v"(c.iya), "v"(c.iyb), "v"(c.ixa), "v"(c.ixb));
-#endif
-    EU5_STAMP(2);
-#ifdef EU5_STAMPS
-    st_[3] = st_[2];
-#endif
-    eu_f2 wx[order], wy[order];
-    if constexpr (DEG >= 2) {
-      eu_weights2<DEG>(s.wm, c.ty, wy);
-      eu_weights2<DEG>(s.wm, c.tx, wx);
-    }
-    const int grp = npass == 1 ? 0 : npass == 2 ? hf : (lane >> 4);
+  eu5_ang8 A;
+  A.lon = (eu_f2){ 0.0f, 0.0f }; A.lat = (eu_f2){ 0.0f, 0.0f };
+  if (n > 1 || !(R.w & EU5_BT_WORK)) {
+    int lane = lane0;
+    asm volatile("" : "+v"(lane));
+    eu5_tab8 Tl = T;
+    asm volatile("" : "+v"(Tl.c0), "+v"(Tl.A0), "+v"(Tl.A1), "+v"(Tl.A2), "+v"(Tl.B0), "+v"(Tl.B1), "+v"(Tl.B2));
+    if (!(R.w & EU5_BT_WORK) && (R.w & 7) > 0 && R.z >= 0) {
+      const eu5_box bx = { R.x, R.y, R.x + (R.z & 0xffff), R.y + (R.z >> 16) };
+      eu5_stage<NCH, DEG>(s, bx, lds_tile, lane);
+    }
+    eu5_angles8(atab, Tl, A);
+  }
+  int mk = m0, sk = slot0;
+  eu5_i4 Rk = R;
+  eu_f2 rga, bxa, rgb, bxb;
+  unsigned oa, ob;
+  int srow;
+  auto put = [&]() {
+    float *const base = p.out + (long long)(srow * EU4_TH) * p.out_stride;
+    const __amdgpu_buffer_rsrc_t rs = __builtin_amdgcn_make_buffer_rsrc(base, 0, 0x80000000u, 0x00027000);
+    if constexpr (NCH == 3) {
+      __builtin_amdgcn_raw_buffer_store_b96((eu5_u3){ __float_as_uint(rga.x), __float_as_uint(rga.y), __float_as_uint(bxa.x) }, rs, (int)oa, 0, 0);
+      __builtin_amdgcn_raw_buffer_store_b96((eu5_u3){ __float_as_uint(rgb.x), __float_as_uint(rgb.y), __float_as_uint(bxb.x) }, rs, (int)ob, 0, 0);
+    } else {
+      __builtin_amdgcn_raw_buffer_store_b128((eu5_u4){ __float_as_uint(rga.x), __float_as_uint(rga.y), __float_as_uint(bxa.x), __float_as_uint(bxa.y) }, rs, (int)oa, 0, 0);
+      __builtin_amdgcn_raw_buffer_store_b128((eu5_u4){ __float_as_uint(rgb.x), __float_as_uint(rgb.y), __float_as_uint(bxb.x), __float_as_uint(bxb.y) }, rs, (int)ob, 0, 0);
+    }
+  };
 #pragma unroll 1
-    for (int pi = 0; pi < npass; pi++) {
-      eu5_i4 Rn = { 0, 0, -1, 0 };
-      if (pi + 1 < npass) Rn = rec[pi + 1];
-      if (some) {
-        if (pi > 0) eu5_stage<NCH, DEG>(s, bx, lds_tile, lane);
-        const int ibw = bx.mxx - bx.mnx + order;
-        const bool mine = grp == pi;
-        const int oa = (mine && va) ? ((c.iya - bx.mny) * ibw + (c.ixa - bx.mnx)) * 4 : 0;
-        const int ob = (mine && vb) ? ((c.iyb - bx.mny) * ibw + (c.ixb - bx.mnx)) * 4 : 0;
-        if (pi == 0) EU5_STAMP(4);
-        asm volatile("s_waitcnt vmcnt(0)" ::: "memory");
-        if (pi == 0) EU5_STAMP(5);
-        if (mine) eu5_taps<NCH, DEG>((eu_lptr)wtile, oa, ob, ibw * 4, wx, wy, c.tx, c.ty, rga, bxa, rgb, bxb);
-      }
-      bx = (eu5_box){ Rn.x, Rn.y, Rn.x + (Rn.z & 0xffff), Rn.y + (Rn.z >> 16) };
-      some = Rn.z >= 0;
-    }
-  }
-#ifdef EU5_STAMPS
-  asm volatile("" : : "v"(rga), "v"(bxa), "v"(rgb), "v"(bxb));
-#endif
-  EU5_STAMP(6);
-  float qa[4] = { rga.x, rga.y, bxa.x, bxa.y }, qb[4] = { rgb.x, rgb.y, bxb.x, bxb.y };
-  if (have_n) eu5_load8<true>(p, ty_n, x0_n, lane, Tn);
+  for (int k = 0;; k++) {
+    int lane = lane0;
+    asm volatile("" : "+v"(lane));
+#ifdef EU5_STAMPS
+    if (k > 0) { EU5_STAMP(0); st_[4] = 0; st_[5] = 0; }
+#endif
+    const bool last = k + 1 >= n;
+    int mk_n = 0, sk_n = 0;
+    if (!last) { mk_n = ent[2 * k + 4]; sk_n = ent[2 * k + 5]; }
+    eu5_i4 Rk_n = { 0, 0, -1, 0 };
+    const bool flip = (mk & EU_POLAR_FLIP) != 0, mir = (mk & EU_POLAR_MIRROR) != 0;
+    srow = mk & (EU_POLAR_FLIP - 1);
+    const int tc = mir ? w.tiles16 - 1 - tcol : tcol;
+    const eu5_crec rec = bt + (sk * w.tiles16 + tc) * EU5_BT_RECS;
+    auto next_record = [&]() {
+      if (!last) {
+        const int tc_n = (mk_n & EU_POLAR_MIRROR) ? w.tiles16 - 1 - tcol : tcol;
+        Rk_n = bt[(sk_n * w.tiles16 + tc_n) * EU5_BT_RECS];
+      }
+    };
+    const int pr = lane & 3, rw = (lane >> 2) & 7, hf = lane >> 5;
+    const int rwm = flip ? 7 - rw : rw;
+    const int xl = tcol * EU4_TW + 8 * hf + 2 * pr;
+    const int xa = mir ? p.width - 1 - xl : xl, xb = mir ? xa - 1 : xa + 1;
+    const bool yin = p.row_begin + srow * EU4_TH + rwm < p.row_end;
+    const bool va = yin && xa < p.width, vb = yin && xb < p.width;
+    rga = (eu_f2){ 0.0f, 0.0f }; bxa = (eu_f2){ 0.0f, 0.0f }; rgb = (eu_f2){ 0.0f, 0.0f }; bxb = (eu_f2){ 0.0f, 0.0f };
+    oa = 0xfffff000u; ob = 0xfffff000u;
+    const int cls = Rk.w;
+    if (cls & EU5_BT_WORK) {
+      if (lane == 0) {
+        const int id = srow * w.tiles16 + tc;
+        const int sh = eu4_shard_of(id);
+        const int slot = atomicAdd(p.wl + EU4_WL_SHARD(sh), 1);
+        p.wl[EU4_WL_ENTRIES + (size_t)slot * EU4_SHARDS + sh] = id;
+      }
+      next_record();
+    } else {
+      const int npass = cls & 7;
+      eu5_box bx = { Rk.x, Rk.y, Rk.x + (Rk.z & 0xffff), Rk.y + (Rk.z >> 16) };
+      bool some = npass > 0 && Rk.z >= 0;
+      if (some && k > 0) eu5_stage<NCH, DEG>(s, bx, lds_tile, lane);
+      next_record();
+      if (npass > 0) {
+        const unsigned sgx = mir ? 0x80000000u : 0u, sgy = flip ? 0x80000000u : 0u;
+        const eu_f2 lon = { __uint_as_float(__float_as_uint(A.lon.x) ^ sgx), __uint_as_float(__float_as_uint(A.lon.y) ^ sgx) };
+        const eu_f2 lat = { __uint_as_float(__float_as_uint(A.lat.x) ^ sgy), __uint_as_float(__float_as_uint(A.lat.y) ^ sgy) };
+        eu5_co8 c;
+        eu5_spline_xy<DEG>(s, lon, lat, c);
+        eu5_split_y<DEG>(c);
+#ifdef EU5_STAMPS
+        asm volatile("" : : "v"(c.iya), "v"(c.iyb), "v"(c.ixa), "v"(c.ixb));
+#endif
+        EU5_STAMP(2);
+#ifdef EU5_STAMPS
+        st_[3] = st_[2];
+#endif
+        eu_f2 wx[order], wy[order];
+        if constexpr (DEG >= 2) {
+          eu_weights2<DEG>(s.wm, c.ty, wy);
+          eu_weights2<DEG>(s.wm, c.tx, wx);
+        }
+        const int hfm = mir ? 1 - hf : hf;
+        const int grp = npass == 1 ? 0 : npass == 2 ? hfm : 2 * hfm + (rwm >> 2);
+#pragma unroll 1
+        for (int pi = 0; pi < npass; pi++) {
+          eu5_i4 Rn = { 0, 0, -1, 0 };
+          if (pi + 1 < npass) Rn = rec[pi + 1];
+          if (some) {
+            if (pi > 0) eu5_stage<NCH, DEG>(s, bx, lds_tile, lane);
+            const int ibw = bx.mxx - bx.mnx + order;
+            const bool mine = grp == pi;
+            const int fa = (mine && va) ? ((c.iya - bx.mny) * ibw + (c.ixa - bx.mnx)) * 4 : 0;
+            const int fb = (mine && vb) ? ((c.iyb - bx.mny) * ibw + (c.ixb - bx.mnx)) * 4 : 0;
+            if (pi == 0) EU5_STAMP(4);
+            asm volatile("s_waitcnt vmcnt(0)" ::: "memory");
+            if (pi == 0) EU5_STAMP(5);
+            if (mine) eu5_taps<NCH, DEG>((eu_lptr)wtile, fa, fb, ibw * 4, wx, wy, c.tx, c.ty, rga, bxa, rgb, bxb);
+          }
+          bx = (eu5_box){ Rn.x, Rn.y, Rn.x + (Rn.z & 0xffff), Rn.y + (Rn.z >> 16) };
+          some = Rn.z >= 0;
+        }
+      }
+      const unsigned orow = (unsigned)rwm * (unsigned)p.out_stride;
+      if (va) oa = (orow + (unsigned)(xa * NCH)) * 4u;
+      if (vb) ob = (orow + (unsigned)(xb * NCH)) * 4u;
+    }
+#ifdef EU5_STAMPS
+    asm volatile("" : : "v"(rga), "v"(bxa), "v"(rgb), "v"(bxb));
+    EU5_STAMP(6);
+    if (lane == 0 && w.stamps && !(cls & EU5_BT_WORK)) {
+      unsigned long long *o = w.stamps + ((size_t)srow * w.tiles16 + tc) * 8;
+      st_[1] = (unsigned long long)((cls & 7) + 1) | (k > 0 ? 16ull : 0ull);
+      st_[7] = __builtin_amdgcn_s_memtime();
+#pragma unroll
+      for (int q = 0; q < 8; q++) o[q] = st_[q];
+    }
+#endif
+    if (last) break;
+    put();
+    mk = mk_n; sk = sk_n; Rk = Rk_n;
+  }
+  {
+    int lane = lane0;
+    asm volatile("" : "+v"(lane));
+    if (have_n) eu5_load8<true>(p, ty_n, x0_n, lane, T);
+  }
   __builtin_amdgcn_sched_barrier(0);
-  {
-    float *const base = p.out + (long long)(tile_y * EU4_TH) * p.out_stride + (long long)x0 * NCH;
-    const __amdgpu_buffer_rsrc_t rs = __builtin_amdgcn_make_buffer_rsrc(base, 0, 0x80000000u, 0x00027000);
-    const unsigned off = ((unsigned)rw * (unsigned)p.out_stride + (unsigned)((8 * hf + 2 * pr) * NCH)) * 4u;
-    const unsigned oa = va ? off : 0xfffff000u, ob = vb ? oa + NCH * 4u : 0xfffff000u;
-    if constexpr (NCH == 3) {
-      __builtin_amdgcn_raw_buffer_store_b96((eu5_u3){ __float_as_uint(qa[0]), __float_as_uint(qa[1]), __float_as_uint(qa[2]) }, rs, (int)oa, 0, 0);
-      __builtin_amdgcn_raw_buffer_store_b96((eu5_u3){ __float_as_uint(qb[0]), __float_as_uint(qb[1]), __float_as_uint(qb[2]) }, rs, (int)ob, 0, 0);
-    } else {
-      __builtin_amdgcn_raw_buffer_store_b128((eu5_u4){ __float_as_uint(qa[0]), __float_as_uint(qa[1]), __float_as_uint(qa[2]), __float_as_uint(qa[3]) }, rs, (int)oa, 0, 0);
-      __builtin_amdgcn_raw_buffer_store_b128((eu5_u4){ __float_as_uint(qb[0]), __float_as_uint(qb[1]), __float_as_uint(qb[2]), __float_as_uint(qb[3]) }, rs, (int)ob, 0, 0);
-    }
-  }
-  EU5_STAMP(7);
-#ifdef EU5_STAMPS
-  if (lane == 0 && w.stamps) {
-    unsigned long long *o = w.stamps + ((size_t)tile_y * w.tiles16 + x0 / EU4_TW) * 8;
-    st_[1] = (unsigned long long)(npass + 1);
-#pragma unroll
-    for (int k = 0; k < 8; k++) o[k] = st_[k];
-  }
-#endif
-}
+  put();
+}
+
 
 struct eu5_tab16 {
   eu4_f4 a0, a1, b0, b1;
@@ -735,8 +806,6 @@
   T.A1A = rtA[1]; T.B1A = rtA[4]; T.A1B = rtB[1]; T.B1B = rtB[4];
   T.c0 = (eu_f2){ p.col[xac], p.col[xbc] };
 }
-
-typedef const __attribute__((address_space(4))) int *eu5_cint;
 
 __device__ __forceinline__ void eu5_load_cols(const float *ct, int xa, int xb, eu5_tab16 &T)
 {
@@ -1019,8 +1088,6 @@
   it.start(t0, K);
   if constexpr (PAIRS) {
     int *const queue = p.wl + EU4_WL_DYN(xcd);
-    const int nbatch = (w.l2_off[xcd + 1] - w.l2_off[xcd]) * w.l2_half;
-    const eu5_cint rows2 = (eu5_cint)w.l2_rows + w.l2_off[xcd];
     auto take = [&]() -> int {
       int v = 0;
       if (lane0 == 0) v = atomicAdd(queue, 1);
@@ -1029,44 +1096,45 @@
     if constexpr (BOXTAB) {
       static_assert(FAST && PRJ == EU_SPHERICAL, "the box table is that of the FAST lat/lon second loop");
       const eu5_crec bt = (eu5_crec)w.boxtab;
-      auto decode = [&](int j, int &ty, int &tcol, int &ti) -> bool {
-        if (j >= nbatch) return false;
-        const int r = (int)(((unsigned long long)(unsigned)j * w.l2_magic) >> 40);
-        ty = rows2[r]; tcol = 2 * (j - r * w.l2_half);
-        ti = ((w.l2_off[xcd] + r) * w.tiles16 + tcol) * EU5_BT_RECS;
+      const eu5_cint ents = (eu5_cint)w.l2p_ent + EU_POLAR_ENTRY_INTS * w.l2p_off[xcd];
+      const int npos = (w.l2p_off[xcd + 1] - w.l2p_off[xcd]) * w.l2p_bpe;
+      auto decode = [&](int j, eu5_cint &e, int &n, int &m, int &sl, int &tcol, int &lim) -> bool {
+        if (j >= npos) return false;
+        const int r = (int)(((unsigned long long)(unsigned)j * w.l2p_magic) >> 40);
+        e = ents + EU_POLAR_ENTRY_INTS * r;
+        n = e[0]; m = e[2] & (EU_POLAR_FLIP - 1); sl = e[3];
+        tcol = e[1] + (j - r * w.l2p_bpe) * w.l2p_bcols;
+        lim = e[1] + w.l2p_ecols;
         return true;
       };
-      int ty_a = 0, col_a = 0, ti_a = 0, ty_n = 0, col_n = 0, ti_n = 0;
-      bool have = decode(__builtin_amdgcn_readfirstlane(take()), ty_a, col_a, ti_a);
-      eu5_tab8 Ta, Tb;
-      eu5_i4 Ra = { 0, 0, -1, 0 }, Rb = { 0, 0, -1, 0 };
-      if (have) { Ra = bt[ti_a]; eu5_load8<FAST>(p, ty_a, col_a * EU4_TW, lane0, Ta); }
+      eu5_cint e_a = ents, e_n = ents;
+      int n_a = 0, m_a = 0, sl_a = 0, col_a = 0, lim_a = 0, n_n = 0, m_n = 0, sl_n = 0, col_n = 0, lim_n = 0;
+      bool have = decode(__builtin_amdgcn_readfirstlane(take()), e_a, n_a, m_a, sl_a, col_a, lim_a);
+      int jn_lane = take();
+      bool second = have && w.l2p_bcols == 2 && col_a + 1 < lim_a;
+      eu5_tab8 Ta;
+      eu5_i4 Ra = { 0, 0, -1, 0 };
+      if (have) { Ra = bt[(sl_a * w.tiles16 + col_a) * EU5_BT_RECS]; eu5_load8<FAST>(p, m_a, col_a * EU4_TW, lane0, Ta); }
       __builtin_amdgcn_s_waitcnt(EU5_WAIT_VM0);
 #pragma unroll 1
       while (have) {
-        const int jn_lane = take();
-        const bool second = col_a + 1 < w.tiles16;
-        if (second) Rb = bt[ti_a + EU5_BT_RECS];
-        {
-          int lane = lane0;
-          asm volatile("" : "+v"(lane));
-          eu5_tile_bt<NCH, DEG>(p, w, atab, tile, ty_a, col_a * EU4_TW, lane, Ta, Ra, bt + ti_a, second, ty_a,
-                                (col_a + 1) * EU4_TW, Tb);
+        bool have_n = true;
+        if (second) {
+          e_n = e_a; n_n = n_a; m_n = m_a; sl_n = sl_a; col_n = col_a + 1; lim_n = lim_a;
+          second = false;
+        } else {
+          have_n = decode(__builtin_amdgcn_readfirstlane(jn_lane), e_n, n_n, m_n, sl_n, col_n, lim_n);
+          jn_lane = take();
+          second = have_n && w.l2p_bcols == 2 && col_n + 1 < lim_n;
         }
-        const bool have_n = decode(__builtin_amdgcn_readfirstlane(jn_lane), ty_n, col_n, ti_n);
-        if (have_n) Ra = bt[ti_n];
-        if (second) {
-          int lane = lane0;
-          asm volatile("" : "+v"(lane));
-          eu5_tile_bt<NCH, DEG>(p, w, atab, tile, ty_a, (col_a + 1) * EU4_TW, lane, Tb, Rb, bt + ti_a + EU5_BT_RECS, have_n,
-                                ty_n, col_n * EU4_TW, Ta);
-        } else if (have_n) {
-          eu5_load8<FAST>(p, ty_n, col_n * EU4_TW, lane0, Ta);
-          __builtin_amdgcn_s_waitcnt(EU5_WAIT_VM0);
-        }
-        ty_a = ty_n; col_a = col_n; ti_a = ti_n; have = have_n;
+        eu5_i4 Rn = { 0, 0, -1, 0 };
+        if (have_n) Rn = bt[(sl_n * w.tiles16 + col_n) * EU5_BT_RECS];
+        eu5_tile_bt<NCH, DEG>(p, w, atab, tile, lane0, Ta, Ra, e_a, n_a, m_a, sl_a, col_a, have_n, m_n, col_n * EU4_TW);
+        e_a = e_n; n_a = n_n; m_a = m_n; sl_a = sl_n; col_a = col_n; lim_a = lim_n; Ra = Rn; have = have_n;
       }
     } else {
+      const int nbatch = (w.l2_off[xcd + 1] - w.l2_off[xcd]) * w.l2_half;
+      const eu5_cint rows2 = (eu5_cint)w.l2_rows + w.l2_off[xcd];
       auto decode = [&](int j, int &ty, int &tcol) -> bool {
         if (j >= nbatch) return false;
         const int r = (int)(((unsigned long long)(unsigned)j * w.l2_magic) >> 40);
diff --git a/envutil_amd/csrc/eu_select.h b/envutil_amd/csrc/eu_select.h
--- a/envutil_amd/csrc/eu_select.h
+++ b/envutil_amd/csrc/eu_select.h
@@ -16,6 +16,7 @@
   int rej;
   int colplan;
   int share;
+  int polar_share;
   int direct;
   int iir_stream;
   int boxtab;
@@ -44,6 +45,8 @@
   s.colplan = first("EU_HIP_COLPLAN") != '0';
   const char sh = first("EU_HIP_SHARE");
   s.share = sh == '0' ? 0 : sh == 'm' ? EU_SHARE_MIRRORS : sh == 'f' ? EU_SHARE_FACES : EU_SHARE_FACES | EU_SHARE_MIRRORS;
+  const char ps = first("EU_HIP_POLAR_SHARE");
+  s.polar_share = ps == '0' ? 0 : ps == 't' ? EU_POLAR_TWINS : ps == 'm' ? EU_POLAR_MIRRORS : EU_POLAR_TWINS | EU_POLAR_MIRRORS;
   s.direct = first("EU_HIP_DIRECT") == '1';
   const char *iir = getenv("EU_HIP_IIR_STREAM");
   s.iir_stream = iir ? atoi(iir) : 7;
diff --git a/envutil_amd/csrc/eu_share_groups.h b/envutil_amd/csrc/eu_share_groups.h
--- a/envutil_amd/csrc/eu_share_groups.h
+++ b/envutil_amd/csrc/eu_share_groups.h
@@ -10,6 +10,8 @@
 #define EU_SHARE_MIRROR (1 << 30)
 #define EU_SHARE_FACES 1
 #define EU_SHARE_MIRRORS 2
+#define EU_POLAR_TWINS 1
+#define EU_POLAR_MIRRORS 2
 
 struct eu_share_input {
   int width, tiles16;
diff --git a/include/eu_hip.h b/include/eu_hip.h
--- a/include/eu_hip.h
+++ b/include/eu_hip.h
@@ -77,6 +77,8 @@
 unsigned long long eu_hip_launch_count(void);
 
 unsigned long long eu_hip_share_follower_tiles(void);
+
+unsigned long long eu_hip_polar_follower_tiles(void);
 
 unsigned long long eu_hip_listed_tiles(void);
 
```
